# Paleogenomics/pss-bam

Hardware: AMD Instinct MI355X
Metric: aligned reads/s (whole node) + HBM GB/s fraction, 200M x 150bp BAM (higher is better)
Workload: dtype u64

## Files before the change

include/pssbam_hip.h:

```cpp
#ifndef PSSBAM_HIP_H
#define PSSBAM_HIP_H

#include <stddef.h>
#include <stdint.h>

#ifdef __cplusplus
extern "C" {
#endif

#define PSSBAM_ABI_VERSION 1
#define PSSBAM_MAX_KLEN 15
#define PSSBAM_MAX_READ_GROUPS 4096
#define PSSBAM_MAX_LENGTH_BINS 64
#define PSSBAM_MAX_CONTIG_SETS 4096
#define PSSBAM_MAX_HIST_LENGTH 65535
#define PSSBAM_MAX_BASE_QUALITY 93
#define PSSBAM_MAX_REGIONS (1 << 26)
#define PSSBAM_SITE_NONE 0
#define PSSBAM_SITE_CPG 1
#define PSSBAM_MAX_END_DEPTH 8

#define PSSBAM_OK 0
#define PSSBAM_EINVAL (-1)
#define PSSBAM_ENODEV (-2)
#define PSSBAM_EHIP (-3)
#define PSSBAM_ENOMEM (-4)
#define PSSBAM_ESTATE (-5)
#define PSSBAM_EFORMAT (-6)
#define PSSBAM_EBUSY (-7)

#define PSSBAM_TALLY_PSS 1u
#define PSSBAM_TALLY_KMER 2u

#define PSSBAM_KERNEL_AUTO 0
#define PSSBAM_KERNEL_SIMPLE 1
#define PSSBAM_KERNEL_TILED 2

typedef struct pssbam_pss_opts {
    int32_t region_len;
    uint64_t min_read_len;
    uint64_t max_read_len;
    int32_t min_mq;
    const char *up_ctx;
    const char *down_ctx;
    int32_t merged_only;
} pssbam_pss_opts;

typedef struct pssbam_kmer_opts {
    int32_t klen;
    int32_t min_mq;
    uint64_t min_read_len;
    uint64_t max_read_len;
    int32_t merged_only;
} pssbam_kmer_opts;

typedef struct pssbam_config {
    uint32_t abi_version;
    uint32_t tally_mask;
    pssbam_pss_opts pss;
    pssbam_kmer_opts kmer;
    const char *read_group;
    int32_t device;
    int32_t kernel;
} pssbam_config;

typedef struct pssbam_engine pssbam_engine;
struct genome;

enum {
    PSSBAM_ST_RECORDS = 0,
    PSSBAM_ST_RG_DROPPED = 1,
    PSSBAM_ST_PARSE_SKIP = 2,
    PSSBAM_ST_NO_CONTIG = 3,
    PSSBAM_ST_PSS_OK = 4,
    PSSBAM_ST_PSS_FILTERED = 5,
    PSSBAM_ST_KMER_OK = 6,
    PSSBAM_ST_KMER_FILTERED = 7,
    PSSBAM_ST_KMER_FAIL = 8,
    PSSBAM_ST_SLOW_PATH = 9,
    PSSBAM_ST_N = 16
};

const char *pssbam_last_error(void);
int pssbam_device_count(void);
int pssbam_warmup(int device);

int pssbam_engine_create(const pssbam_config *cfg, pssbam_engine **out);
void pssbam_engine_destroy(pssbam_engine *e);

int pssbam_engine_set_stream(pssbam_engine *e, void *hip_stream);

int pssbam_engine_set_genome(pssbam_engine *e, const struct genome *g);
int pssbam_engine_set_genome_async(pssbam_engine *e, const struct genome *g);
int pssbam_engine_genome_wait(pssbam_engine *e);

int pssbam_engine_set_genome_arrays(pssbam_engine *e, size_t n, const char *const *ids,
                                    const uint8_t *const *seqs, const uint64_t *lens,
                                    int seqs_on_device);

int pssbam_engine_set_references(pssbam_engine *e, int32_t n_ref, const char *const *names);

int pssbam_engine_submit(pssbam_engine *e, const void *records, uint64_t nbytes,
                         const uint32_t *offsets, uint32_t n_records);

int pssbam_engine_submit_async(pssbam_engine *e, const void *records, uint64_t nbytes,
                               const uint32_t *offsets, uint32_t n_records, uint64_t *ticket);
int pssbam_engine_wait_copied(pssbam_engine *e, uint64_t ticket);
int pssbam_engine_copy_done(pssbam_engine *e, uint64_t ticket);

int pssbam_engine_submit_device(pssbam_engine *e, const void *d_records, uint64_t nbytes,
                                const uint32_t *d_offsets, uint32_t n_records);

int pssbam_engine_sync(pssbam_engine *e);

int pssbam_engine_finish(pssbam_engine *e, unsigned long *fwd, unsigned long *rev, uint64_t *k5,
                         uint64_t *k3, uint64_t stats[PSSBAM_ST_N]);
int pssbam_engine_reset(pssbam_engine *e);

int pssbam_engine_set_read_groups(pssbam_engine *e, int32_t n, const char *const *ids);
int pssbam_engine_finish_groups(pssbam_engine *e, int32_t group, unsigned long *fwd, unsigned long *rev);

int pssbam_engine_finish_kmer_groups(pssbam_engine *e, int32_t group, uint64_t *k5, uint64_t *k3);

int pssbam_engine_set_length_bins(pssbam_engine *e, int32_t n_edges, const uint32_t *edges);

int pssbam_engine_set_contig_sets(pssbam_engine *e, int32_t n_sets, int64_t n_names, const char *const *names,
                                  const int32_t *set_of);

int pssbam_engine_set_min_base_quality(pssbam_engine *e, int32_t q);

int pssbam_engine_set_regions(pssbam_engine *e, int32_t n_names, const char *const *names, int64_t n_regions,
                              const int32_t *name_of, const uint32_t *starts, const uint32_t *ends);

int pssbam_engine_set_length_histogram(pssbam_engine *e, int32_t max_len);

int pssbam_engine_finish_length_histogram(pssbam_engine *e, uint64_t *fwd, uint64_t *rev);

int pssbam_engine_set_site_context(pssbam_engine *e, int32_t mode);

int pssbam_engine_finish_site_context(pssbam_engine *e, unsigned long *fwd_in, unsigned long *rev_in);

int pssbam_engine_set_end_condition(pssbam_engine *e, int32_t depth, int32_t cell5, int32_t cell3);

int pssbam_engine_finish_end_condition(pssbam_engine *e, unsigned long *fwd_c, unsigned long *rev_c, uint64_t reads[4]);

int pssbam_engine_counters_device(pssbam_engine *e, void **d_counters, size_t *n_u64);

int pssbam_engine_bind_counters(pssbam_engine *e, void *d_counters, size_t n_u64);

int pssbam_engine_genome_kmer_count(pssbam_engine *e, int klen, uint64_t *counts);

int pssbam_reduce_counters(pssbam_engine *const *engines, int n, int root);

int pssbam_host_register(void *ptr, size_t bytes);
int pssbam_host_unregister(void *ptr);

int pssbam_engine_timer_begin(pssbam_engine *e);
int pssbam_engine_timer_end(pssbam_engine *e, float *ms);
int pssbam_engine_kernel_time(pssbam_engine *e, double *total_ms, uint64_t *n_launches, int reset);

int pssbam_engine_phase_times(pssbam_engine *e, double *h2d_ms, uint64_t *h2d_bytes, double *kernel_ms,
                              uint64_t *n_launches);

typedef struct pssbam_bgzf_block {
    uint64_t in_off;
    uint32_t in_len;
    uint32_t isize;
    uint64_t out_off;
    uint32_t crc;
    uint32_t status;
} pssbam_bgzf_block;

int64_t pssbam_bgzf_scan(const void *bytes, uint64_t nbytes, pssbam_bgzf_block *blocks, uint64_t max_blocks,
                         uint64_t *consumed, uint64_t *inflated_bytes);

int pssbam_bgzf_inflate_device(void *hip_stream, const void *d_comp, uint64_t comp_bytes, pssbam_bgzf_block *d_blocks,
                               uint32_t n_blocks, void *d_out, int check_crc);

int pssbam_engine_submit_bgzf(pssbam_engine *e, const void *comp, uint64_t comp_bytes, const pssbam_bgzf_block *blocks,
                              uint32_t n_blocks, uint32_t first_record_offset, uint64_t *ticket);
int pssbam_engine_wait_bgzf_copied(pssbam_engine *e, uint64_t ticket);
int pssbam_engine_feed_open(pssbam_engine *e, int32_t n_ref, uint64_t genome_bytes_hint);
int pssbam_engine_feed_break(pssbam_engine *e);
int pssbam_engine_feed_handoff(pssbam_engine *from, pssbam_engine *to);
#define PSSBAM_FEED_BAD_BLOCK 1u
#define PSSBAM_FEED_RAGGED 2u
#define PSSBAM_FEED_BAD_RECORD 4u
#define PSSBAM_FEED_TRUNCATED 8u
int pssbam_engine_feed_status(pssbam_engine *e, uint32_t *flags, double *inflate_ms, uint64_t *inflated_bytes);
int pssbam_engine_hint_records(pssbam_engine *e, const void *records, uint64_t nbytes);
int pssbam_feed_reserve(int device);
int pssbam_feed_release(int device);

int pssbam_bgzf_inflate_host(int device, const void *bgzf, uint64_t nbytes, void *out, uint64_t out_cap, uint64_t *out_len,
                             uint32_t *n_blocks, uint32_t *first_bad_block, uint32_t *first_bad_status, double *kernel_ms,
                             int check_crc, int repeats);

int64_t pssbam_index_records(const void *bytes, uint64_t nbytes, uint32_t *offsets,
                             uint64_t max_records, uint64_t *consumed);

#ifdef __cplusplus
}
#endif
#endif
```

pss-bam_amd/__init__.py:

```python
from __future__ import annotations

import ctypes as C
import subprocess
from dataclasses import dataclass
from pathlib import Path

import numpy as np

PKG_DIR = Path(__file__).resolve().parent
ROOT = PKG_DIR.parent
LIB_HIP = PKG_DIR / "libpssbam_hip.so"
LIB_HOST = PKG_DIR / "libpssbam_host.so"
LIB_SYNTH = PKG_DIR / "libpssbam_synth.so"

TALLY_PSS, TALLY_KMER = 1, 2
KERNEL_AUTO, KERNEL_SIMPLE, KERNEL_TILED = 0, 1, 2
ST_NAMES = ["records", "rg_dropped", "parse_skip", "no_contig", "pss_ok", "pss_filtered", "kmer_ok",
            "kmer_filtered", "kmer_fail", "slow_path"]
ST_N = 16

HIP_SYMBOLS = [
    "pssbam_last_error", "pssbam_device_count", "pssbam_warmup", "pssbam_engine_create", "pssbam_engine_destroy",
    "pssbam_engine_set_stream", "pssbam_engine_set_genome", "pssbam_engine_set_genome_arrays",
    "pssbam_engine_set_references", "pssbam_engine_submit", "pssbam_engine_submit_async", "pssbam_engine_wait_copied",
    "pssbam_engine_copy_done", "pssbam_engine_phase_times", "pssbam_engine_submit_device", "pssbam_engine_sync",
    "pssbam_engine_finish", "pssbam_engine_reset", "pssbam_engine_counters_device", "pssbam_engine_bind_counters",
    "pssbam_reduce_counters", "pssbam_engine_genome_kmer_count", "pssbam_host_register", "pssbam_host_unregister", "pssbam_engine_timer_begin",
    "pssbam_engine_timer_end", "pssbam_engine_kernel_time", "pssbam_index_records", "pssbam_bgzf_scan",
    "pssbam_bgzf_inflate_device", "pssbam_bgzf_inflate_host", "pssbam_engine_submit_bgzf", "pssbam_engine_wait_bgzf_copied",
    "pssbam_engine_feed_status", "pssbam_engine_feed_break", "pssbam_engine_feed_handoff", "pssbam_feed_reserve", "pssbam_engine_hint_records",
    "pssbam_engine_set_genome_async", "pssbam_engine_genome_wait", "pssbam_engine_feed_open", "pssbam_feed_release",
    "pssbam_engine_set_read_groups", "pssbam_engine_finish_groups", "pssbam_engine_set_length_bins",
    "pssbam_engine_set_contig_sets", "pssbam_engine_finish_kmer_groups", "pssbam_engine_set_min_base_quality",
    "pssbam_engine_set_regions", "pssbam_engine_set_length_histogram", "pssbam_engine_finish_length_histogram",
    "pssbam_engine_set_site_context", "pssbam_engine_finish_site_context",
    "pssbam_engine_set_end_condition", "pssbam_engine_finish_end_condition",
]
MAX_READ_GROUPS = 4096
MAX_LENGTH_BINS = 64
MAX_CONTIG_SETS = 4096
MAX_BASE_QUALITY = 93
MAX_HIST_LENGTH = 65535
MAX_REGIONS = 1 << 26
SITE_NONE, SITE_CPG = 0, 1
SITE_MODES = {None: SITE_NONE, "none": SITE_NONE, "cpg": SITE_CPG}
MAX_END_DEPTH = 8
END_PRESETS = {"ss": (13, 13), "ds": (13, 2)}
EBUSY = -7


def build(verbose: bool = False) -> None:
    subprocess.run(["make", "-C", str(PKG_DIR), "all"], check=True,
                   stdout=None if verbose else subprocess.DEVNULL)


class PssbamError(RuntimeError):
    pass


class _PssOpts(C.Structure):
    _fields_ = [("region_len", C.c_int32), ("min_read_len", C.c_uint64), ("max_read_len", C.c_uint64),
                ("min_mq", C.c_int32), ("up_ctx", C.c_char_p), ("down_ctx", C.c_char_p),
                ("merged_only", C.c_int32)]


class _KmerOpts(C.Structure):
    _fields_ = [("klen", C.c_int32), ("min_mq", C.c_int32), ("min_read_len", C.c_uint64),
                ("max_read_len", C.c_uint64), ("merged_only", C.c_int32)]


class _Config(C.Structure):
    _fields_ = [("abi_version", C.c_uint32), ("tally_mask", C.c_uint32), ("pss", _PssOpts), ("kmer", _KmerOpts),
                ("read_group", C.c_char_p), ("device", C.c_int32), ("kernel", C.c_int32)]


_hip = None


def hip_lib() -> C.CDLL:
    global _hip
    if _hip is not None:
        return _hip
    if not LIB_HIP.exists():
        raise PssbamError(f"{LIB_HIP} is missing: run __graft_entry__.build() (hipcc --offload-arch=gfx950)")
    L = C.CDLL(str(LIB_HIP))
    L.pssbam_last_error.restype = C.c_char_p
    L.pssbam_engine_create.argtypes = [C.POINTER(_Config), C.POINTER(C.c_void_p)]
    L.pssbam_engine_destroy.argtypes = [C.c_void_p]
    L.pssbam_engine_destroy.restype = None
    L.pssbam_engine_set_stream.argtypes = [C.c_void_p, C.c_void_p]
    L.pssbam_engine_set_genome.argtypes = [C.c_void_p, C.c_void_p]
    L.pssbam_engine_set_genome_arrays.argtypes = [C.c_void_p, C.c_size_t, C.POINTER(C.c_char_p),
                                                  C.POINTER(C.c_void_p), C.POINTER(C.c_uint64), C.c_int]
    L.pssbam_engine_set_references.argtypes = [C.c_void_p, C.c_int32, C.POINTER(C.c_char_p)]
    L.pssbam_engine_submit.argtypes = [C.c_void_p, C.c_void_p, C.c_uint64, C.c_void_p, C.c_uint32]
    L.pssbam_engine_submit_async.argtypes = [C.c_void_p, C.c_void_p, C.c_uint64, C.c_void_p, C.c_uint32, C.POINTER(C.c_uint64)]
    L.pssbam_engine_wait_copied.argtypes = [C.c_void_p, C.c_uint64]
    L.pssbam_engine_copy_done.argtypes = [C.c_void_p, C.c_uint64]
    L.pssbam_engine_phase_times.argtypes = [C.c_void_p, C.POINTER(C.c_double), C.POINTER(C.c_uint64), C.POINTER(C.c_double),
                                            C.POINTER(C.c_uint64)]
    L.pssbam_engine_submit_device.argtypes = [C.c_void_p, C.c_void_p, C.c_uint64, C.c_void_p, C.c_uint32]
    L.pssbam_engine_sync.argtypes = [C.c_void_p]
    L.pssbam_engine_finish.argtypes = [C.c_void_p, C.c_void_p, C.c_void_p, C.c_void_p, C.c_void_p, C.c_void_p]
    L.pssbam_engine_reset.argtypes = [C.c_void_p]
    L.pssbam_engine_set_read_groups.argtypes = [C.c_void_p, C.c_int32, C.POINTER(C.c_char_p)]
    L.pssbam_engine_finish_groups.argtypes = [C.c_void_p, C.c_int32, C.c_void_p, C.c_void_p]
    L.pssbam_engine_finish_kmer_groups.argtypes = [C.c_void_p, C.c_int32, C.c_void_p, C.c_void_p]
    L.pssbam_engine_set_length_bins.argtypes = [C.c_void_p, C.c_int32, C.POINTER(C.c_uint32)]
    L.pssbam_engine_set_contig_sets.argtypes = [C.c_void_p, C.c_int32, C.c_int64, C.POINTER(C.c_char_p), C.POINTER(C.c_int32)]
    L.pssbam_engine_set_min_base_quality.argtypes = [C.c_void_p, C.c_int32]
    L.pssbam_engine_set_length_histogram.argtypes = [C.c_void_p, C.c_int32]
    L.pssbam_engine_finish_length_histogram.argtypes = [C.c_void_p, C.c_void_p, C.c_void_p]
    L.pssbam_engine_set_site_context.argtypes = [C.c_void_p, C.c_int32]
    L.pssbam_engine_finish_site_context.argtypes = [C.c_void_p, C.c_void_p, C.c_void_p]
    L.pssbam_engine_set_end_condition.argtypes = [C.c_void_p, C.c_int32, C.c_int32, C.c_int32]
    L.pssbam_engine_finish_end_condition.argtypes = [C.c_void_p, C.c_void_p, C.c_void_p, C.c_void_p]
    L.pssbam_engine_set_regions.argtypes = [C.c_void_p, C.c_int32, C.POINTER(C.c_char_p), C.c_int64, C.c_void_p, C.c_void_p, C.c_void_p]
    L.pssbam_engine_counters_device.argtypes = [C.c_void_p, C.POINTER(C.c_void_p), C.POINTER(C.c_size_t)]
    L.pssbam_engine_bind_counters.argtypes = [C.c_void_p, C.c_void_p, C.c_size_t]
    L.pssbam_engine_genome_kmer_count.argtypes = [C.c_void_p, C.c_int, C.c_void_p]
    L.pssbam_engine_timer_begin.argtypes = [C.c_void_p]
    L.pssbam_engine_timer_end.argtypes = [C.c_void_p, C.POINTER(C.c_float)]
    L.pssbam_engine_kernel_time.argtypes = [C.c_void_p, C.POINTER(C.c_double), C.POINTER(C.c_uint64), C.c_int]
    L.pssbam_index_records.restype = C.c_int64
    L.pssbam_index_records.argtypes = [C.c_void_p, C.c_uint64, C.c_void_p, C.c_uint64, C.POINTER(C.c_uint64)]
    _hip = L
    return L


def _chk(rc: int) -> None:
    if rc != 0:
        raise PssbamError(f"pssbam error {rc}: {hip_lib().pssbam_last_error().decode()}")


def bgzf_inflate(bgzf: np.ndarray, check_crc: bool = True, repeats: int = 1, want_output: bool = True) -> dict:
    L = hip_lib()
    L.pssbam_bgzf_inflate_host.argtypes = [C.c_int, C.c_void_p, C.c_uint64, C.c_void_p, C.c_uint64, C.POINTER(C.c_uint64),
                                           C.POINTER(C.c_uint32), C.POINTER(C.c_uint32), C.POINTER(C.c_uint32),
                                           C.POINTER(C.c_double), C.c_int, C.c_int]
    L.pssbam_bgzf_scan.restype = C.c_int64
    L.pssbam_bgzf_scan.argtypes = [C.c_void_p, C.c_uint64, C.c_void_p, C.c_uint64, C.POINTER(C.c_uint64), C.POINTER(C.c_uint64)]
    bgzf = np.ascontiguousarray(bgzf, dtype=np.uint8)
    consumed, total = C.c_uint64(), C.c_uint64()
    n = L.pssbam_bgzf_scan(bgzf.ctypes.data, bgzf.size, None, 0, C.byref(consumed), C.byref(total))
    if n < 0:
        _chk(int(n))
    out = np.empty(int(total.value) if want_output else 0, dtype=np.uint8)
    out_len, nb, bad_b, bad_s, ms = C.c_uint64(), C.c_uint32(), C.c_uint32(), C.c_uint32(), C.c_double()
    _chk(L.pssbam_bgzf_inflate_host(-1, bgzf.ctypes.data, bgzf.size, out.ctypes.data if want_output else None, out.size,
                                    C.byref(out_len), C.byref(nb), C.byref(bad_b), C.byref(bad_s), C.byref(ms),
                                    int(check_crc), repeats))
    return {"data": out, "inflated_bytes": int(out_len.value), "n_blocks": int(nb.value),
            "bad_block": None if bad_b.value == 0xFFFFFFFF else int(bad_b.value), "bad_status": int(bad_s.value),
            "kernel_ms": float(ms.value)}


def index_records(buf: np.ndarray) -> np.ndarray:
    L = hip_lib()
    n = L.pssbam_index_records(buf.ctypes.data, buf.size, None, 1 << 62, None)
    if n < 0:
        _chk(int(n))
    offs = np.empty(n + 1, dtype=np.uint32)
    consumed = C.c_uint64()
    n2 = L.pssbam_index_records(buf.ctypes.data, buf.size, offs.ctypes.data, n, C.byref(consumed))
    assert n2 == n
    return offs


@dataclass
class Tables:
    fwd: np.ndarray | None
    rev: np.ndarray | None
    k5: np.ndarray | None
    k3: np.ndarray | None
    stats: dict


class Engine:

    def __init__(self, pss: dict | None = None, kmer: dict | None = None, read_group: str | None = None,
                 kernel: int = KERNEL_AUTO, device: int = -1, read_groups: list[str] | None = None,
                 length_bins: list[int] | None = None, contig_sets=None, min_base_qual: int = 0,
                 length_hist: int = 0, site_context: str | None = None, end_condition: tuple[int, int, int] | None = None):
        L = hip_lib()
        cfg = _Config()
        cfg.abi_version = 1
        cfg.tally_mask = (TALLY_PSS if pss is not None else 0) | (TALLY_KMER if kmer is not None else 0)
        self._keep = []
        if pss is not None:
            up, dn = pss.get("up_ctx", "ACGT").encode(), pss.get("down_ctx", "ACGT").encode()
            self._keep += [up, dn]
            cfg.pss = _PssOpts(pss.get("region_len", 15), pss.get("min_read_len", 0),
                               pss.get("max_read_len", 250000000), pss.get("min_mq", 0), up, dn,
                               int(pss.get("merged_only", False)))
            self.region_len = cfg.pss.region_len
            self._len_range = (cfg.pss.min_read_len, cfg.pss.max_read_len)
        if kmer is not None:
            cfg.kmer = _KmerOpts(kmer.get("klen", 8), kmer.get("min_mq", 0), kmer.get("min_read_len", 0),
                                 kmer.get("max_read_len", 250000000), int(kmer.get("merged_only", False)))
            self.klen = cfg.kmer.klen
            if pss is None:
                self._len_range = (cfg.kmer.min_read_len, cfg.kmer.max_read_len)
        self.has_pss, self.has_kmer = pss is not None, kmer is not None
        if read_group is not None:
            rg = read_group.encode()
            self._keep.append(rg)
            cfg.read_group = rg
        cfg.device = device
        cfg.kernel = kernel
        h = C.c_void_p()
        _chk(L.pssbam_engine_create(C.byref(cfg), C.byref(h)))
        self._h = h
        self._L = L
        self.read_groups: list[str] = []
        self.length_bins: list[tuple[int, int]] = []
        self.contig_sets: list[str] = []
        self._min_base_qual = 0
        self._length_hist = 0
        self._site_context = SITE_NONE
        if min_base_qual:
            self.set_min_base_quality(min_base_qual)
        if length_hist:
            self.set_length_histogram(length_hist)
        if site_context is not None:
            self.set_site_context(site_context)
        self._end_condition = (0, 0, 0)
        if end_condition is not None:
            self.set_end_condition(*end_condition)
        if read_groups is not None:
            self.set_read_groups(read_groups)
        if length_bins is not None:
            self.set_length_bins(length_bins)
        if contig_sets is not None:
            self.set_contig_sets(contig_sets)

    def set_min_base_quality(self, q: int):
        _chk(self._L.pssbam_engine_set_min_base_quality(self._h, int(q)))
        self._min_base_qual = int(q)

    @property
    def min_base_qual(self) -> int:
        return self._min_base_qual

    def set_length_histogram(self, max_len: int):
        _chk(self._L.pssbam_engine_set_length_histogram(self._h, int(max_len)))
        self._length_hist = int(max_len)

    @property
    def length_hist(self) -> int:
        return self._length_hist

    def finish_length_hist(self) -> tuple[np.ndarray, np.ndarray]:
        fwd = np.zeros(self._length_hist + 2, dtype=np.uint64)
        rev = np.zeros_like(fwd)
        _chk(self._L.pssbam_engine_finish_length_histogram(self._h, fwd.ctypes.data, rev.ctypes.data))
        return fwd, rev

    def set_site_context(self, mode):
        if isinstance(mode, str) or mode is None:
            if mode not in SITE_MODES:
                raise ValueError(f"unknown site context {mode!r}")
            mode = SITE_MODES[mode]
        _chk(self._L.pssbam_engine_set_site_context(self._h, int(mode)))
        self._site_context = int(mode)

    @property
    def site_context(self) -> str | None:
        return "cpg" if self._site_context == SITE_CPG else None

    def finish_site_context(self) -> tuple[np.ndarray, np.ndarray]:
        fwd = np.zeros((self.region_len + 2, 16), dtype=np.uint64)
        rev = np.zeros_like(fwd)
        _chk(self._L.pssbam_engine_finish_site_context(self._h, fwd.ctypes.data, rev.ctypes.data))
        return fwd, rev

    def set_end_condition(self, depth: int, cell5: int = 13, cell3: int = 13):
        _chk(self._L.pssbam_engine_set_end_condition(self._h, int(depth), int(cell5), int(cell3)))
        self._end_condition = (int(depth), int(cell5), int(cell3)) if depth else (0, 0, 0)

    @property
    def end_condition(self) -> tuple[int, int, int] | None:
        return self._end_condition if self._end_condition[0] else None

    def finish_end_condition(self) -> tuple[np.ndarray, np.ndarray, np.ndarray]:
        fwd = np.zeros((self.region_len + 2, 16), dtype=np.uint64)
        rev = np.zeros_like(fwd)
        reads = np.zeros(4, dtype=np.uint64)
        _chk(self._L.pssbam_engine_finish_end_condition(self._h, fwd.ctypes.data, rev.ctypes.data, reads.ctypes.data))
        return fwd, rev, reads

    def set_regions(self, names, name_of, starts, ends):
        raw = [nm.encode() if isinstance(nm, str) else bytes(nm) for nm in names]
        arr = (C.c_char_p * max(len(raw), 1))(*raw)
        name_of = np.ascontiguousarray(name_of, dtype=np.int32)
        starts = np.ascontiguousarray(starts, dtype=np.uint32)
        ends = np.ascontiguousarray(ends, dtype=np.uint32)
        if not (name_of.size == starts.size == ends.size):
            raise ValueError("name_of, starts and ends must have one entry per interval")
        _chk(self._L.pssbam_engine_set_regions(self._h, len(raw), arr, name_of.size, name_of.ctypes.data, starts.ctypes.data,
                                               ends.ctypes.data))

    def set_contig_sets(self, sets):
        pairs = [(nm, lab) for lab, nms in sets.items() for nm in nms] if isinstance(sets, dict) else list(sets)
        labels: list[str] = []
        index: dict[str, int] = {}
        for _, lab in pairs:
            if lab not in index:
                index[lab] = len(labels)
                labels.append(lab)
        names = (C.c_char_p * max(len(pairs), 1))(*[nm.encode() if isinstance(nm, str) else bytes(nm) for nm, _ in pairs])
        set_of = (C.c_int32 * max(len(pairs), 1))(*[index[lab] for _, lab in pairs])
        _chk(self._L.pssbam_engine_set_contig_sets(self._h, len(labels), len(pairs), names, set_of))
        self.contig_sets = labels

    def finish_sets(self) -> dict:
        return self._finish_planes(enumerate(self.contig_sets))

    def set_length_bins(self, edges: list[int]):
        edges = [int(x) for x in edges]
        arr = (C.c_uint32 * max(len(edges), 1))(*[x & 0xFFFFFFFF for x in edges])
        _chk(self._L.pssbam_engine_set_length_bins(self._h, len(edges), arr))
        lo, hi = self._len_range
        starts, ends = [lo] + edges, [x - 1 for x in edges] + [hi]
        self.length_bins = list(zip(starts, ends))

    def set_read_groups(self, ids: list[str]):
        raw = [i.encode() if isinstance(i, str) else bytes(i) for i in ids]
        arr = (C.c_char_p * max(len(raw), 1))(*raw)
        _chk(self._L.pssbam_engine_set_read_groups(self._h, len(raw), arr))
        self.read_groups = [i.decode() if isinstance(i, bytes) else i for i in ids]

    def finish_groups(self) -> dict:
        return self._finish_planes([(-1, None)] + list(enumerate(self.read_groups)))

    def finish_bins(self) -> dict:
        return self._finish_planes(enumerate(self.length_bins))

    def _finish_planes(self, planes) -> dict:
        out = {}
        for g, key in planes:
            if not self.has_pss:
                k5 = np.zeros(4 ** self.klen, dtype=np.uint64)
                k3 = np.zeros_like(k5)
                _chk(self._L.pssbam_engine_finish_kmer_groups(self._h, g, k5.ctypes.data, k3.ctypes.data))
                if key not in out:
                    out[key] = Tables(None, None, k5, k3, {})
                continue
            fwd = np.zeros((self.region_len + 2, 16), dtype=np.uint64)
            rev = np.zeros_like(fwd)
            _chk(self._L.pssbam_engine_finish_groups(self._h, g, fwd.ctypes.data, rev.ctypes.data))
            if key not in out:
                out[key] = Tables(fwd, rev, None, None, {})
        return out

    def close(self):
        if getattr(self, "_h", None):
            self._L.pssbam_engine_destroy(self._h)
            self._h = None

    __del__ = close

    def set_stream(self, hip_stream: int):
        _chk(self._L.pssbam_engine_set_stream(self._h, C.c_void_p(hip_stream)))

    def set_genome_arrays(self, contigs: list[tuple[str, np.ndarray]]):
        n = len(contigs)
        arrs = [np.ascontiguousarray(a, dtype=np.uint8) for _, a in contigs]
        ids = (C.c_char_p * n)(*[c[0].encode() for c in contigs])
        seqs = (C.c_void_p * n)(*[a.ctypes.data for a in arrs])
        lens = (C.c_uint64 * n)(*[a.size for a in arrs])
        _chk(self._L.pssbam_engine_set_genome_arrays(self._h, n, ids, seqs, lens, 0))

    def set_genome_device(self, contigs: list[tuple[str, int, int]]):
        n = len(contigs)
        ids = (C.c_char_p * n)(*[c[0].encode() for c in contigs])
        seqs = (C.c_void_p * n)(*[c[1] for c in contigs])
        lens = (C.c_uint64 * n)(*[c[2] for c in contigs])
        _chk(self._L.pssbam_engine_set_genome_arrays(self._h, n, ids, seqs, lens, 1))

    def set_genome_struct(self, genome_ptr: int):
        _chk(self._L.pssbam_engine_set_genome(self._h, C.c_void_p(genome_ptr)))

    def set_references(self, names: list[str]):
        n = len(names)
        arr = (C.c_char_p * max(n, 1))(*[s.encode() for s in names])
        _chk(self._L.pssbam_engine_set_references(self._h, n, arr))

    def submit(self, records: np.ndarray, offsets: np.ndarray | None = None):
        records = np.ascontiguousarray(records, dtype=np.uint8)
        if offsets is None:
            offsets = index_records(records)
            if int(offsets[-1]) != records.size:
                raise PssbamError("record block ends in a partial record")
        offsets = np.ascontiguousarray(offsets, dtype=np.uint32)
        _chk(self._L.pssbam_engine_submit(self._h, records.ctypes.data, records.size, offsets.ctypes.data,
                                          offsets.size - 1))

    def submit_async(self, records: np.ndarray, offsets: np.ndarray) -> int:
        t = C.c_uint64()
        _chk(self._L.pssbam_engine_submit_async(self._h, records.ctypes.data, records.size, offsets.ctypes.data,
                                                offsets.size - 1, C.byref(t)))
        return int(t.value)

    def wait_copied(self, ticket: int):
        _chk(self._L.pssbam_engine_wait_copied(self._h, ticket))

    def copy_done(self, ticket: int) -> bool:
        rc = self._L.pssbam_engine_copy_done(self._h, ticket)
        if rc < 0:
            _chk(rc)
        return bool(rc)

    def phase_times(self) -> dict:
        a, b, c, d = C.c_double(), C.c_uint64(), C.c_double(), C.c_uint64()
        _chk(self._L.pssbam_engine_phase_times(self._h, C.byref(a), C.byref(b), C.byref(c), C.byref(d)))
        return {"h2d_ms": a.value, "h2d_bytes": b.value, "kernel_ms": c.value, "launches": d.value}

    def feed_open(self, n_ref: int, genome_bytes_hint: int = 0):
        self._L.pssbam_engine_feed_open.argtypes = [C.c_void_p, C.c_int32, C.c_uint64]
        _chk(self._L.pssbam_engine_feed_open(self._h, n_ref, genome_bytes_hint))

    def submit_bgzf(self, bgzf: np.ndarray, header_bytes: int = 0, max_batch_inflated: int = 1 << 30, on_busy=None) -> int:
        class _Blk(C.Structure):
            _fields_ = [("in_off", C.c_uint64), ("in_len", C.c_uint32), ("isize", C.c_uint32), ("out_off", C.c_uint64),
                        ("crc", C.c_uint32), ("status", C.c_uint32)]
        L = self._L
        L.pssbam_bgzf_scan.restype = C.c_int64
        L.pssbam_bgzf_scan.argtypes = [C.c_void_p, C.c_uint64, C.c_void_p, C.c_uint64, C.POINTER(C.c_uint64), C.POINTER(C.c_uint64)]
        L.pssbam_engine_submit_bgzf.argtypes = [C.c_void_p, C.c_void_p, C.c_uint64, C.c_void_p, C.c_uint32, C.c_uint32,
                                                C.POINTER(C.c_uint64)]
        L.pssbam_engine_wait_bgzf_copied.argtypes = [C.c_void_p, C.c_uint64]
        bgzf = np.ascontiguousarray(bgzf, dtype=np.uint8)
        consumed = C.c_uint64()
        n = L.pssbam_bgzf_scan(bgzf.ctypes.data, bgzf.size, None, 0, C.byref(consumed), None)
        if n < 0:
            _chk(int(n))
        if consumed.value != bgzf.size:
            raise PssbamError("input ends inside a BGZF block")
        blocks = (_Blk * max(int(n), 1))()
        L.pssbam_bgzf_scan(bgzf.ctypes.data, bgzf.size, blocks, n, None, None)
        i, skip = 0, header_bytes
        while i < n and skip >= blocks[i].isize and (skip > 0 or blocks[i].isize == 0):
            skip -= blocks[i].isize
            i += 1
        while i < n:
            j, base_in, base_out = i, blocks[i].in_off & ~3, blocks[i].out_off
            while j < n and blocks[j].out_off + blocks[j].isize - base_out <= max_batch_inflated:
                j += 1
            j = max(j, i + 1)
            grp = (_Blk * (j - i))()
            for k in range(i, j):
                grp[k - i] = blocks[k]
                grp[k - i].in_off -= base_in
                grp[k - i].out_off -= base_out
            end_in = blocks[j - 1].in_off + blocks[j - 1].in_len
            t = C.c_uint64()
            rc = L.pssbam_engine_submit_bgzf(self._h, bgzf.ctypes.data + base_in, end_in - base_in, grp, j - i, skip, C.byref(t))
            if rc == EBUSY and on_busy is not None:
                on_busy()
                rc = L.pssbam_engine_submit_bgzf(self._h, bgzf.ctypes.data + base_in, end_in - base_in, grp, j - i, skip, C.byref(t))
            _chk(rc)
            _chk(L.pssbam_engine_wait_bgzf_copied(self._h, t.value))
            skip = 0
            i = j
        return int(n)

    def feed_break(self):
        self._L.pssbam_engine_feed_break.argtypes = [C.c_void_p]
        _chk(self._L.pssbam_engine_feed_break(self._h))

    def feed_handoff(self, to: "Engine"):
        self._L.pssbam_engine_feed_handoff.argtypes = [C.c_void_p, C.c_void_p]
        _chk(self._L.pssbam_engine_feed_handoff(self._h, to._h))

    def feed_status(self) -> dict:
        L = self._L
        L.pssbam_engine_feed_status.argtypes = [C.c_void_p, C.POINTER(C.c_uint32), C.POINTER(C.c_double), C.POINTER(C.c_uint64)]
        f, ms, nb = C.c_uint32(), C.c_double(), C.c_uint64()
        _chk(L.pssbam_engine_feed_status(self._h, C.byref(f), C.byref(ms), C.byref(nb)))
        return {"flags": int(f.value), "inflate_ms": float(ms.value), "inflated_bytes": int(nb.value)}

    def submit_device(self, d_records: int, nbytes: int, d_offsets: int, n_records: int):
        _chk(self._L.pssbam_engine_submit_device(self._h, C.c_void_p(d_records), nbytes, C.c_void_p(d_offsets),
                                                 n_records))

    def sync(self):
        _chk(self._L.pssbam_engine_sync(self._h))

    def reset(self):
        _chk(self._L.pssbam_engine_reset(self._h))

    def finish(self) -> Tables:
        fwd = rev = k5 = k3 = None
        if self.has_pss:
            fwd = np.zeros((self.region_len + 2, 16), dtype=np.uint64)
            rev = np.zeros_like(fwd)
        if self.has_kmer:
            k5 = np.zeros(4 ** self.klen, dtype=np.uint64)
            k3 = np.zeros_like(k5)
        st = np.zeros(ST_N, dtype=np.uint64)
        p = lambda a: a.ctypes.data if a is not None else None
        _chk(self._L.pssbam_engine_finish(self._h, p(fwd), p(rev), p(k5), p(k3), st.ctypes.data))
        return Tables(fwd, rev, k5, k3, {n: int(st[i]) for i, n in enumerate(ST_NAMES)})

    def counters_device(self) -> tuple[int, int]:
        ptr, n = C.c_void_p(), C.c_size_t()
        _chk(self._L.pssbam_engine_counters_device(self._h, C.byref(ptr), C.byref(n)))
        return int(ptr.value), int(n.value)

    def bind_counters(self, d_ptr: int | None, n_u64: int = 0):
        _chk(self._L.pssbam_engine_bind_counters(self._h, C.c_void_p(d_ptr) if d_ptr else None, n_u64))

    def counter_layout(self) -> dict:
        rows = (self.region_len + 2) if self.has_pss else 0
        nb = 4 ** self.klen if self.has_kmer else 0
        lay = {"fwd": 0, "rev": rows * 16, "k5": 2 * rows * 16, "k3": 2 * rows * 16 + nb,
               "stats": 2 * rows * 16 + 2 * nb, "rows": rows, "bins": nb}
        base = lay["stats"] + ST_N
        if not self.has_pss:
            for name, tag, keys in (("groups", "id", self.read_groups), ("length_bins", "bin", self.length_bins),
                                    ("contig_sets", "label", self.contig_sets)):
                lay[name] = [{tag: key, "k5": base + k * 2 * nb, "k3": base + k * 2 * nb + nb} for k, key in enumerate(keys)]
            lay["n_u64"] = base + (len(self.read_groups) + len(self.length_bins) + len(self.contig_sets)) * 2 * nb
            return lay
        lay["groups"] = [{"id": g, "fwd": base + k * 2 * rows * 16, "rev": base + k * 2 * rows * 16 + rows * 16}
                         for k, g in enumerate(self.read_groups)]
        lay["length_bins"] = [{"bin": b, "fwd": base + k * 2 * rows * 16, "rev": base + k * 2 * rows * 16 + rows * 16}
                              for k, b in enumerate(self.length_bins)]
        lay["contig_sets"] = [{"label": s, "fwd": base + k * 2 * rows * 16, "rev": base + k * 2 * rows * 16 + rows * 16}
                              for k, s in enumerate(self.contig_sets)]
        lay["n_u64"] = base + (len(self.read_groups) + len(self.length_bins) + len(self.contig_sets)) * 2 * rows * 16
        if self._length_hist:
# ... 28 lines not shown
```

pss-bam_amd/csrc/engine.hip:

```cpp
#include "../../include/pssbam_hip.h"
#include "../../include/fasta-genome-io.h"

#include <hip/hip_runtime.h>

#include <algorithm>
#include <condition_variable>
#include <cstdarg>
#include <cstdio>
#include <cstdlib>
#include <cstring>
#include <ctime>
#include <map>
#include <string>
#include <thread>
#include <tuple>
#include <type_traits>
#include <unordered_map>
#include <atomic>
#include <memory>
#include <mutex>
#include <vector>

#include "tally_kernels.h"

// ... 85 lines not shown
    uint64_t flush_seq = 0;
};

struct DeferredTally {
    int slot;
    uint64_t sub_base, sub_len, offs_at;
    uint32_t n_bound, k;
    uint64_t sample_off;
    bool last_of_slot;
};

namespace {
struct PinEntry { size_t len; int refs; };
std::map<const void *, PinEntry> g_pins;
std::mutex g_pins_mu;
bool pin_acquire(const void *p, size_t len) {
    std::lock_guard<std::mutex> lk(g_pins_mu);
    auto it = g_pins.find(p);
    if (it != g_pins.end()) { it->second.refs++; return true; }
    if (hipHostRegister((void *)p, len, hipHostRegisterPortable) != hipSuccess) { (void)hipGetLastError(); return false; }
    g_pins[p] = PinEntry{len, 1};
    return true;
}
void pin_release(const void *p) {
    std::lock_guard<std::mutex> lk(g_pins_mu);
    auto it = g_pins.find(p);
    if (it == g_pins.end()) return;
    if (--it->second.refs == 0) { (void)hipHostUnregister((void *)p); g_pins.erase(it); }
}
}

struct KernelPrep { uint32_t lds = 0; int occ = 0; };

struct pssbam_engine {
    pssbam_config cfg{};
    std::string up_ctx, down_ctx, rg;
    bool has_rg = false;
    int device = 0;
    int n_cu = 0;
    hipStream_t stream = nullptr, copy_stream = nullptr, copy_stream2 = nullptr;
    hipStream_t inflate_stream[2] = {nullptr, nullptr};
    hipEvent_t feed_base_ev = nullptr;
    hipStream_t genome_stream = nullptr;
    std::thread late_thread;
    std::atomic<int> late_ready{0};
    std::mutex late_mu;
    hipStream_t late_copy1 = nullptr, late_copy2 = nullptr, late_genome = nullptr;
    bool late_adopted = false;
    hipEvent_t genome_ready = nullptr;
    bool genome_wait_pending = false;
    std::vector<const void *> genome_pins;
    std::vector<void *> retired;
    hipEvent_t copied2 = nullptr;
    bool own_stream = false;

    uint8_t *d_genome = nullptr;
    uint32_t *d_genome4 = nullptr;
    uint32_t acgt_ctx = 0;
    uint64_t genome_bytes = 0;
    std::vector<uint64_t> contig_start;
    std::vector<uint32_t> contig_len;
    std::vector<std::string> contig_ids;
    int32_t star_contig = -1;
    uint4 *d_ref_info = nullptr;
    uint4 *h_ref_info = nullptr;
    size_t h_ref_cap = 0;
    int32_t n_ref = 0;
    bool have_refs = false;
    uint8_t *d_rg = nullptr;
    PlaneSel planes = PLANES_NONE;
    uint32_t n_planes = 0, off_groups = 0, plane_words = 0;
    uint64_t kplane_words = 0;
    uint8_t *d_grp_ids = nullptr;
    uint32_t *d_grp_offs = nullptr, *d_grp_hash = nullptr;
    uint32_t grp_hash_mask = 0;
    std::vector<uint32_t> len_edges;
    std::unordered_map<std::string, uint32_t> ctg_plane;
    std::vector<std::string> ref_names;
    bool tallied = false;
    uint32_t min_bq = 0;
    uint32_t hist_max = 0, off_hist = 0;
    uint32_t site_mode = 0, off_site = 0;
    uint32_t end_depth = 0, end_cell5 = 0, end_cell3 = 0, off_end = 0;
    int env_hist_lds_bins = -1;
    std::unordered_map<std::string, std::vector<uint2>> regions;
    bool has_regions = false;
    uint32_t region_shift = 10;
    std::vector<uint4> ref_info_host;
    uint4 *d_region_info = nullptr;
    uint32_t *d_region_grid = nullptr;
    uint2 *d_region_iv = nullptr;
    unsigned long long *d_counters = nullptr;
    unsigned long long *d_counters_own = nullptr;
    size_t n_counters = 0;
    uint32_t rows = 0, off_rev = 0, off_k5 = 0, off_k3 = 0, off_stats = 0;
    uint64_t n_bins = 0;
    Slot slots[2];
    int next_slot = 0;
    uint64_t ticket_seq = 0;
    double h2d_ms = 0.0;
    uint64_t h2d_bytes = 0;
    std::vector<FeedAcc *> feed;
    int cur_feed = -1, spare_feed = -1;
    uint64_t flush_seq = 0;
    bool feed_opened = false;
    int32_t feed_n_ref = 0;
    uint64_t feed_mem_budget = 0;
    std::vector<DeferredTally> deferred;
    uint8_t *d_carry = nullptr;
    uint8_t *h_handoff = nullptr;
    hipEvent_t handoff_ev = nullptr;
    uint64_t feed_out_target = FEED_OUT_TARGET, feed_comp_cap = FEED_COMP_CAP;
    double feed_t_alloc = 0, feed_t_wait_busy = 0, feed_t_flush = 0;
    double feed_t0 = 0, feed_t_first_flush = -1;
    uint64_t feed_slots_allocated = 0, feed_deferred_launches = 0, feed_early_flushes = 0;
    uint64_t feed_blocks_launched = 0, feed_lanes_launched = 0;
    uint64_t feed_idle_min_blocks = 8192;
    uint64_t feed_block_target = 0;
    std::vector<std::pair<uint64_t, hipEvent_t>> feed_copies;
    std::vector<hipEvent_t> feed_event_pool;
    uint32_t *d_feed_flags = nullptr;
    uint64_t *d_feed_tail = nullptr;
    bool feed_fresh = true;
    uint32_t feed_skip = 0;
    double inflate_ms = 0.0;
    uint64_t inflated_bytes = 0;
    std::vector<std::pair<hipEvent_t, hipEvent_t>> inflate_events;
    hipEvent_t t_begin = nullptr, t_end = nullptr;
    std::vector<std::pair<hipEvent_t, hipEvent_t>> launch_events;
    std::vector<hipEvent_t> event_pool;
    double kernel_ms = 0.0;
    uint64_t kernel_launches = 0;
    int env_tile_reads = 0, env_grid_mult = 0, env_simple_blocks = 0, env_grid_wgs = 0, env_pieces = 0;
    int env_group_slots = 0;
    bool warned_ablate = false;
    bool compact_plan_once = false;
    std::unordered_map<const void *, KernelPrep> prep;
    bool use_compact = true;
    uint32_t *d_scratch = nullptr;
    size_t scratch_slots = 0;
    uint32_t dev_pieces = 0;
    uint64_t dev_pieces_avg = 0;
};

static void ctx_mask(const char *set, uint32_t (&m)[8]) {
    memset(m, 0, sizeof m);
    for (const unsigned char *p = (const unsigned char *)set;; p++) {
        const uint32_t st = enc_byte(*p);
        m[st >> 5] |= 1u << (st & 31);
        if (!*p) break;
    }
}

static int env_int(const char *name) {
    const char *v = getenv(name);
    return v ? atoi(v) : 0;
}

static void late_streams(pssbam_engine *e, bool wait) {
    std::lock_guard<std::mutex> lk(e->late_mu);
    if (e->late_adopted) return;
    if (!wait && !e->late_ready.load(std::memory_order_acquire)) return;
    if (e->late_thread.joinable()) e->late_thread.join();
    e->copy_stream = e->late_copy1;
    e->copy_stream2 = e->late_copy2;
    e->genome_stream = e->late_genome;
    e->late_adopted = true;
}

extern "C" int pssbam_engine_create(const pssbam_config *cfg, pssbam_engine **out) {
    if (!cfg || !out) return fail(PSSBAM_EINVAL, "null argument");
    *out = nullptr;
    if (cfg->abi_version != PSSBAM_ABI_VERSION)
        return fail(PSSBAM_EINVAL, "abi_version %u != %u", cfg->abi_version, PSSBAM_ABI_VERSION);
    if (!(cfg->tally_mask & (PSSBAM_TALLY_PSS | PSSBAM_TALLY_KMER)) ||
        (cfg->tally_mask & ~(PSSBAM_TALLY_PSS | PSSBAM_TALLY_KMER)))
        return fail(PSSBAM_EINVAL, "tally_mask must be a non-empty subset of PSS|KMER");
    if ((cfg->tally_mask & PSSBAM_TALLY_PSS)) {
        if (cfg->pss.region_len < 0 || cfg->pss.region_len > 1000000)
            return fail(PSSBAM_EINVAL, "region_len %d out of range", cfg->pss.region_len);
        if (!cfg->pss.up_ctx || !cfg->pss.down_ctx) return fail(PSSBAM_EINVAL, "up_ctx/down_ctx must be set");
    }
    if ((cfg->tally_mask & PSSBAM_TALLY_KMER) && (cfg->kmer.klen < 1 || cfg->kmer.klen > PSSBAM_MAX_KLEN))
        return fail(PSSBAM_EINVAL, "klen %d outside the device range 1..%d", cfg->kmer.klen, PSSBAM_MAX_KLEN);

    int n_dev = 0;
    if (hipGetDeviceCount(&n_dev) != hipSuccess || n_dev == 0)
        return fail(PSSBAM_ENODEV, "no HIP device available (this engine has no CPU path)");
    int dev = cfg->device;
    if (dev < 0) HIP_TRY(hipGetDevice(&dev));
    if (dev >= n_dev) return fail(PSSBAM_ENODEV, "device %d does not exist (%d present)", dev, n_dev);
    if (!device_is_gfx950(dev) && !getenv("PSSBAM_ALLOW_OTHER_ARCH"))
        return fail(PSSBAM_ENODEV, "device %d is not gfx950", dev);
    HIP_TRY(hipSetDevice(dev));

    pssbam_engine *e = new pssbam_engine();
    std::unique_ptr<pssbam_engine, void (*)(pssbam_engine *)> guard(e, pssbam_engine_destroy);
    e->cfg = *cfg;
    e->device = dev;
    if (cfg->tally_mask & PSSBAM_TALLY_PSS) {
        e->up_ctx = cfg->pss.up_ctx;
        e->down_ctx = cfg->pss.down_ctx;
    }
    if (cfg->read_group) {
        e->rg = cfg->read_group;
        e->has_rg = true;
    }
    e->cfg.pss.up_ctx = e->cfg.pss.down_ctx = e->cfg.read_group = nullptr;
    const bool tstat = getenv("PSSBAM_STATS") != nullptr;
    const double tc0 = tstat ? feed_now() : 0.0;
    hipDeviceProp_t pr;
    HIP_TRY(hipGetDeviceProperties(&pr, dev));
    e->n_cu = pr.multiProcessorCount;
    const double tc1 = tstat ? feed_now() : 0.0;
    HIP_TRY(hipStreamCreateWithFlags(&e->stream, hipStreamNonBlocking));
    if (getenv("PSSBAM_STREAMS_UP_FRONT")) {
        HIP_TRY(hipStreamCreateWithFlags(&e->copy_stream, hipStreamNonBlocking));
        HIP_TRY(hipStreamCreateWithFlags(&e->copy_stream2, hipStreamNonBlocking));
        HIP_TRY(hipStreamCreateWithFlags(&e->genome_stream, hipStreamNonBlocking));
        e->late_adopted = true;
    } else {
        e->late_thread = std::thread([e, dev]() {
            if (hipSetDevice(dev) == hipSuccess) {
                if (hipStreamCreateWithFlags(&e->late_copy1, hipStreamNonBlocking) != hipSuccess) e->late_copy1 = nullptr;
                if (hipStreamCreateWithFlags(&e->late_copy2, hipStreamNonBlocking) != hipSuccess) e->late_copy2 = nullptr;
                if (hipStreamCreateWithFlags(&e->late_genome, hipStreamNonBlocking) != hipSuccess) e->late_genome = nullptr;
            }
            (void)hipGetLastError();
            e->late_ready.store(1, std::memory_order_release);
        });
    }
    HIP_TRY(hipEventCreateWithFlags(&e->genome_ready, hipEventDisableTiming));
    HIP_TRY(hipEventCreateWithFlags(&e->copied2, hipEventDisableTiming));
    e->own_stream = true;
    HIP_TRY(hipEventCreate(&e->t_begin));
    HIP_TRY(hipEventCreate(&e->t_end));
    const double tc2 = tstat ? feed_now() : 0.0;

    e->rows = (cfg->tally_mask & PSSBAM_TALLY_PSS) ? (uint32_t)cfg->pss.region_len + 2u : 0u;
    e->n_bins = (cfg->tally_mask & PSSBAM_TALLY_KMER) ? (1ull << (2 * cfg->kmer.klen)) : 0ull;
    e->off_rev = e->rows * 16u;
    e->off_k5 = 2u * e->rows * 16u;
    e->off_k3 = (uint32_t)(e->off_k5 + e->n_bins);
    e->off_stats = (uint32_t)(e->off_k3 + e->n_bins);
    e->n_counters = (size_t)e->off_stats + PSSBAM_ST_N;
    e->plane_words = 2u * e->rows * 16u;
    e->off_groups = (uint32_t)e->n_counters;
    e->kplane_words = cfg->tally_mask == PSSBAM_TALLY_KMER ? 2ull * e->n_bins : 0ull;
    HIP_TRY(hipMalloc(&e->d_counters_own, e->n_counters * sizeof(unsigned long long)));
    e->d_counters = e->d_counters_own;
    HIP_TRY(hipMemsetAsync(e->d_counters, 0, e->n_counters * sizeof(unsigned long long), e->stream));
    if (e->has_rg) {
        HIP_TRY(hipMalloc(&e->d_rg, e->rg.size() + 16));
        HIP_TRY(hipMemcpy(e->d_rg, e->rg.data(), e->rg.size(), hipMemcpyHostToDevice));
    }
    for (Slot &s : e->slots) {
        HIP_TRY(hipEventCreate(&s.copy_begin));
        HIP_TRY(hipEventCreate(&s.copied));
        HIP_TRY(hipEventCreateWithFlags(&s.consumed, hipEventDisableTiming));
    }
    e->scratch_slots = (size_t)e->n_cu * 8;
    HIP_TRY(hipMalloc(&e->d_scratch, e->scratch_slots * SCRATCH_WORDS * sizeof(uint32_t)));
    e->env_tile_reads = env_int("PSSBAM_TILE_READS");
    e->env_grid_mult = env_int("PSSBAM_GRID_MULT");
    e->env_simple_blocks = env_int("PSSBAM_SIMPLE_BLOCKS");
    e->env_grid_wgs = env_int("PSSBAM_GRID_WGS");
    e->env_pieces = env_int("PSSBAM_PIECES");
    e->env_group_slots = env_int("PSSBAM_GROUP_SLOTS");
    if (getenv("PSSBAM_HIST_LDS_BINS")) e->env_hist_lds_bins = std::max(env_int("PSSBAM_HIST_LDS_BINS"), 0);
    if (const int g = env_int("PSSBAM_REGION_GRID_SHIFT")) e->region_shift = (uint32_t)std::min(std::max(g, 2), 20);
    if (getenv("PSSBAM_COMPACT")) e->use_compact = env_int("PSSBAM_COMPACT") != 0;
    if (getenv("PSSBAM_COMPACT_PLAN_ONCE")) e->compact_plan_once = env_int("PSSBAM_COMPACT_PLAN_ONCE") != 0;
    if (tstat)
        fprintf(stderr, "[pssbam] engine on device %d: device properties %.3f, its stream + events %.3f, counters + scratch (first allocations, first "
                        "enqueue) %.3f s\n", dev, tc1 - tc0, tc2 - tc1, feed_now() - tc2);
    *out = guard.release();
    return PSSBAM_OK;
}

extern "C" void pssbam_engine_destroy(pssbam_engine *e) {
    if (!e) return;
    (void)hipSetDevice(e->device);
    late_streams(e, true);
    for (hipStream_t is : e->inflate_stream)
        if (is) (void)hipStreamSynchronize(is);
    if (e->stream) (void)hipStreamSynchronize(e->stream);
    if (e->copy_stream) (void)hipStreamSynchronize(e->copy_stream);
    if (e->copy_stream2) (void)hipStreamSynchronize(e->copy_stream2);
    for (Slot &s : e->slots) {
        if (s.d_recs) (void)hipFree(s.d_recs);
        if (s.d_offs) (void)hipFree(s.d_offs);
        if (s.copied) (void)hipEventDestroy(s.copied);
        if (s.copy_begin) (void)hipEventDestroy(s.copy_begin);
        if (s.consumed) (void)hipEventDestroy(s.consumed);
    }
    if (e->genome_stream) (void)hipStreamSynchronize(e->genome_stream);
    for (const void *p : e->genome_pins) pin_release(p);
    e->genome_pins.clear();
    for (FeedAcc *sp : e->feed) {
        FeedAcc &s = *sp;
        void *ptrs[] = {s.d_comp, s.d_blocks, s.d_a, s.d_e, s.d_last, s.d_nexta, s.d_n, s.d_counts, s.d_base, s.d_out, s.d_offs, s.d_nrecs, s.d_chain};
        for (void *q : ptrs)
            if (q) (void)hipFree(q);
        if (s.h_blocks) (void)hipHostFree(s.h_blocks);
        if (s.consumed) (void)hipEventDestroy(s.consumed);
        if (s.copies_done) (void)hipEventDestroy(s.copies_done);
        if (s.copies_done2) (void)hipEventDestroy(s.copies_done2);
        if (s.inflated) (void)hipEventDestroy(s.inflated);
        if (s.inflate_done) (void)hipEventDestroy(s.inflate_done);
        delete sp;
    }
    e->feed.clear();
    if (e->d_carry) (void)hipFree(e->d_carry);
    if (e->h_handoff) (void)hipHostFree(e->h_handoff);
    if (e->handoff_ev) (void)hipEventDestroy(e->handoff_ev);
    for (void *q : e->retired) (void)hipFree(q);
    if (e->d_feed_tail) (void)hipFree(e->d_feed_tail);
    for (auto &p : e->feed_copies) (void)hipEventDestroy(p.second);
    for (hipEvent_t ev : e->feed_event_pool) (void)hipEventDestroy(ev);
    if (e->d_feed_flags) (void)hipFree(e->d_feed_flags);
    for (auto &p : e->inflate_events) { (void)hipEventDestroy(p.first); (void)hipEventDestroy(p.second); }
    for (auto &p : e->launch_events) { (void)hipEventDestroy(p.first); (void)hipEventDestroy(p.second); }
    for (hipEvent_t ev : e->event_pool) (void)hipEventDestroy(ev);
    if (e->t_begin) (void)hipEventDestroy(e->t_begin);
    if (e->t_end) (void)hipEventDestroy(e->t_end);
    if (e->d_scratch) (void)hipFree(e->d_scratch);
    if (e->d_genome) (void)hipFree(e->d_genome);
    if (e->d_genome4) (void)hipFree(e->d_genome4);
    if (e->d_ref_info) (void)hipFree(e->d_ref_info);
    if (e->h_ref_info) (void)hipHostFree(e->h_ref_info);
    if (e->d_rg) (void)hipFree(e->d_rg);
    for (void *q : {(void *)e->d_region_info, (void *)e->d_region_grid, (void *)e->d_region_iv})
        if (q) (void)hipFree(q);
    if (e->d_grp_ids) (void)hipFree(e->d_grp_ids);
    if (e->d_grp_offs) (void)hipFree(e->d_grp_offs);
    if (e->d_grp_hash) (void)hipFree(e->d_grp_hash);
    if (e->d_counters_own) (void)hipFree(e->d_counters_own);
    if (e->own_stream && e->stream) (void)hipStreamDestroy(e->stream);
    if (e->copy_stream) (void)hipStreamDestroy(e->copy_stream);
    if (e->copy_stream2) (void)hipStreamDestroy(e->copy_stream2);
    for (hipStream_t is : e->inflate_stream)
        if (is) (void)hipStreamDestroy(is);
    if (e->feed_base_ev) (void)hipEventDestroy(e->feed_base_ev);
    if (e->genome_stream) (void)hipStreamDestroy(e->genome_stream);
    if (e->genome_ready) (void)hipEventDestroy(e->genome_ready);
    if (e->copied2) (void)hipEventDestroy(e->copied2);
    delete e;
}

extern "C" int pssbam_engine_set_stream(pssbam_engine *e, void *hip_stream) {
    if (!e) return fail(PSSBAM_EINVAL, "null engine");
    HIP_TRY(hipSetDevice(e->device));
    HIP_TRY(hipStreamSynchronize(e->stream));
    if (e->own_stream) HIP_TRY(hipStreamDestroy(e->stream));
    e->stream = (hipStream_t)hip_stream;
    e->own_stream = false;
    return PSSBAM_OK;
}

static constexpr uint64_t CONTIG_ALIGN = 256, CONTIG_PAD = 256;

static hipEvent_t take_event(pssbam_engine *e);
static int feed_resume(pssbam_engine *e);

static int genome_settle(pssbam_engine *e) {
    if (e->genome_pins.empty()) return PSSBAM_OK;
    HIP_TRY(hipSetDevice(e->device));
    HIP_TRY(hipEventSynchronize(e->genome_ready));
    for (const void *p : e->genome_pins) pin_release(p);
    e->genome_pins.clear();
    return PSSBAM_OK;
}

static int genome_upload(pssbam_engine *e, size_t n, const char *const *ids, const uint8_t *const *seqs, const uint64_t *lens,
                         int seqs_on_device) {
    if (!e || (n && (!ids || !seqs || !lens))) return fail(PSSBAM_EINVAL, "null argument");
    HIP_TRY(hipSetDevice(e->device));
    int rc = genome_settle(e);
    if (rc) return rc;
    std::vector<size_t> order(n);
    for (size_t i = 0; i < n; i++) order[i] = i;
    std::stable_sort(order.begin(), order.end(), [&](size_t a, size_t b) { return strcmp(ids[a], ids[b]) < 0; });
    std::vector<uint64_t> start(n + 1, 0);
    std::vector<uint32_t> len(n + 1, 0);
    uint64_t total = CONTIG_PAD;
    for (size_t k = 0; k < n; k++) {
        if (lens[order[k]] > 0xFFFFFF00ull)
            return fail(PSSBAM_EINVAL, "contig %s has %llu bases; the engine addresses contigs below 4 Gi bases", ids[order[k]],
                        (unsigned long long)lens[order[k]]);
        start[k] = total;
        len[k] = (uint32_t)lens[order[k]];
        total += ((uint64_t)len[k] + CONTIG_PAD + CONTIG_ALIGN - 1) / CONTIG_ALIGN * CONTIG_ALIGN;
    }
    if (e->d_genome) {
        HIP_TRY(hipStreamSynchronize(e->stream));
        HIP_TRY(hipFree(e->d_genome));
        e->d_genome = nullptr;
        if (e->d_genome4) { HIP_TRY(hipFree(e->d_genome4)); e->d_genome4 = nullptr; }
    }
    HIP_TRY(hipMalloc(&e->d_genome, total));
    late_streams(e, true);
    if (!e->genome_stream) HIP_TRY(hipStreamCreateWithFlags(&e->genome_stream, hipStreamNonBlocking));
    hipStream_t gs = e->genome_stream;
    if (seqs_on_device) {
        hipEvent_t ev = take_event(e);
        if (!ev) return fail(PSSBAM_EHIP, "hipEventCreate failed");
        HIP_TRY(hipEventRecord(ev, e->stream));
        HIP_TRY(hipStreamWaitEvent(gs, ev, 0));
        e->event_pool.push_back(ev);
    }
    HIP_TRY(hipMemsetAsync(e->d_genome, 0, total, gs));
    const bool try_lock = !seqs_on_device && !getenv("PSSBAM_NO_PIN");
    for (size_t k = 0; k < n; k++) {
        if (!len[k]) continue;
        const void *src = seqs[order[k]];
        if (try_lock && len[k] >= (32u << 20) && pin_acquire(src, len[k])) e->genome_pins.push_back(src);
        HIP_TRY(hipMemcpyAsync(e->d_genome + start[k], src, len[k],
                               seqs_on_device ? hipMemcpyDeviceToDevice : hipMemcpyHostToDevice, gs));
    }
    hipLaunchKernelGGL(encode_genome_kernel, dim3(4096), dim3(256), 0, gs, e->d_genome, total / 16);
    HIP_TRY(hipGetLastError());
    {
        CtxSets sets;
        ctx_mask(e->up_ctx.c_str(), sets.up);
        ctx_mask(e->down_ctx.c_str(), sets.down);
        e->acgt_ctx = 0;
        for (uint32_t v = 0; v < 4; v++)
            e->acgt_ctx |= (((sets.up[0] >> v) & 1u) << (2 * v)) | (((sets.down[0] >> v) & 1u) << (2 * v + 1));
        const uint64_t n_out = total / 8, slack = 16;
        HIP_TRY(hipMalloc(&e->d_genome4, (n_out + slack) * sizeof(uint32_t)));
        HIP_TRY(hipMemsetAsync(e->d_genome4 + n_out, 0x44, slack * sizeof(uint32_t), gs));
        hipLaunchKernelGGL(pack_genome4_kernel, dim3(4096), dim3(256), 0, gs, e->d_genome, e->d_genome4, n_out, sets);
        HIP_TRY(hipGetLastError());
    }
    HIP_TRY(hipEventRecord(e->genome_ready, gs));
    e->genome_wait_pending = true;
    e->contig_start.assign(start.begin(), start.begin() + n);
    e->contig_len.assign(len.begin(), len.begin() + n);
    e->genome_bytes = total;
    e->contig_ids.clear();
    for (size_t k = 0; k < n; k++) e->contig_ids.emplace_back(ids[order[k]]);
    e->star_contig = -1;
    if (e->have_refs) e->have_refs = false;
    {
        auto it = std::lower_bound(e->contig_ids.begin(), e->contig_ids.end(), std::string("*"),
                                   [](const std::string &a, const std::string &b) { return strcmp(a.c_str(), b.c_str()) < 0; });
        if (it != e->contig_ids.end() && *it == "*") e->star_contig = (int32_t)(it - e->contig_ids.begin());
    }
    return PSSBAM_OK;
}

extern "C" int pssbam_engine_set_genome_arrays(pssbam_engine *e, size_t n, const char *const *ids,
                                               const uint8_t *const *seqs, const uint64_t *lens,
                                               int seqs_on_device) {
    int rc = genome_upload(e, n, ids, seqs, lens, seqs_on_device);
    if (rc) return rc;
    if (e->genome_stream) HIP_TRY(hipStreamSynchronize(e->genome_stream));
    return genome_settle(e);
}

static int genome_from_struct(pssbam_engine *e, const struct genome *g, bool wait) {
    if (!e || !g) return fail(PSSBAM_EINVAL, "null argument");
    std::vector<const char *> ids(g->n_seqs);
    std::vector<const uint8_t *> seqs(g->n_seqs);
    std::vector<uint64_t> lens(g->n_seqs);
    for (size_t i = 0; i < g->n_seqs; i++) {
        ids[i] = g->seqs[i]->id;
        seqs[i] = (const uint8_t *)g->seqs[i]->seq;
        lens[i] = g->seqs[i]->len;
    }
    return wait ? pssbam_engine_set_genome_arrays(e, g->n_seqs, ids.data(), seqs.data(), lens.data(), 0)
                : genome_upload(e, g->n_seqs, ids.data(), seqs.data(), lens.data(), 0);
}

extern "C" int pssbam_engine_set_genome(pssbam_engine *e, const struct genome *g) { return genome_from_struct(e, g, true); }

extern "C" int pssbam_engine_set_genome_async(pssbam_engine *e, const struct genome *g) { return genome_from_struct(e, g, false); }

extern "C" int pssbam_engine_genome_wait(pssbam_engine *e) {
    if (!e) return fail(PSSBAM_EINVAL, "null engine");
    HIP_TRY(hipSetDevice(e->device));
    if (e->genome_stream) HIP_TRY(hipStreamSynchronize(e->genome_stream));
    return genome_settle(e);
}

static int pack_regions(pssbam_engine *e, bool in_use) {
    if (!e->has_regions) return PSSBAM_OK;
    const size_t n_ent = (size_t)e->n_ref + 1;
    const uint32_t g = e->region_shift;
    std::vector<uint4> desc(n_ent, make_uint4(0, 0, 0, 0));
    uint64_t n_iv = 0, n_grid = 0;
    std::vector<const std::vector<uint2> *> src(n_ent, nullptr);
    for (size_t i = 0; i < n_ent; i++) {
        const uint4 ri = e->ref_info_host[i];
        if (!ri.w) continue;
        const auto it = e->regions.find(i < (size_t)e->n_ref ? e->ref_names[i] : std::string("*"));
        if (it == e->regions.end()) continue;
        uint64_t cnt = 0;
        for (const uint2 &v : it->second) cnt += v.x < ri.z ? 1u : 0u;
        if (!cnt) continue;
        src[i] = &it->second;
        desc[i] = make_uint4(0, (uint32_t)cnt, 0, 0);
        n_iv += cnt;
        n_grid += ((uint64_t)ri.z >> g) + 2;
    }
    if (n_iv >= (1ull << 32) || n_grid >= (1ull << 32)) return fail(PSSBAM_ENOMEM, "the region table has too many intervals or grid words for 32-bit indices");
    const uint64_t bytes = n_ent * sizeof(uint4) + (n_iv + 1) * sizeof(uint2) + (n_grid + 2) * sizeof(uint32_t);
    HIP_TRY(hipSetDevice(e->device));
    if (in_use && e->d_region_info) HIP_TRY(hipStreamSynchronize(e->stream));
    for (void **q : {(void **)&e->d_region_info, (void **)&e->d_region_grid, (void **)&e->d_region_iv})
        if (*q) { HIP_TRY(hipFree(*q)); *q = nullptr; }
    size_t free_b = 0, total_b = 0;
    HIP_TRY(hipMemGetInfo(&free_b, &total_b));
    if (bytes > (uint64_t)free_b)
        return fail(PSSBAM_ENOMEM, "the region table (%llu intervals, grid shift %u) needs %llu bytes; the device has %llu free",
                    (unsigned long long)n_iv, g, (unsigned long long)bytes, (unsigned long long)free_b);
    std::vector<uint2> iv((size_t)n_iv + 1, make_uint2(0, 0));
    std::vector<uint32_t> grid((size_t)n_grid + 2, 0u);
    uint64_t at_iv = 0, at_grid = 0;
    for (size_t i = 0; i < n_ent; i++) {
        if (!src[i]) continue;
        const uint32_t len = e->ref_info_host[i].z, cnt = desc[i].y;
        desc[i].x = (uint32_t)at_iv;
        desc[i].z = (uint32_t)at_grid;
        uint2 *out = iv.data() + at_iv;
        for (uint32_t k = 0; k < cnt; k++) out[k] = make_uint2((*src[i])[k].x, std::min((*src[i])[k].y, len));
        const uint64_t n_bins = ((uint64_t)len >> g) + 1;
        uint32_t j = 0;
        for (uint64_t b = 0; b < n_bins; b++) {
            while (j < cnt && (uint64_t)out[j].y <= (b << g)) j++;
            grid[at_grid + b] = j;
        }
        grid[at_grid + n_bins] = cnt;
        at_iv += cnt;
        at_grid += n_bins + 1;
    }
    HIP_TRY(hipMalloc(&e->d_region_info, n_ent * sizeof(uint4)));
    HIP_TRY(hipMalloc(&e->d_region_iv, iv.size() * sizeof(uint2)));
    HIP_TRY(hipMalloc(&e->d_region_grid, grid.size() * sizeof(uint32_t)));
    HIP_TRY(hipMemcpy(e->d_region_info, desc.data(), n_ent * sizeof(uint4), hipMemcpyHostToDevice));
    HIP_TRY(hipMemcpy(e->d_region_iv, iv.data(), iv.size() * sizeof(uint2), hipMemcpyHostToDevice));
    HIP_TRY(hipMemcpy(e->d_region_grid, grid.data(), grid.size() * sizeof(uint32_t), hipMemcpyHostToDevice));
    return PSSBAM_OK;
}

extern "C" int pssbam_engine_set_regions(pssbam_engine *e, int32_t n_names, const char *const *names, int64_t n_regions,
                                         const int32_t *name_of, const uint32_t *starts, const uint32_t *ends) {
    if (!e) return fail(PSSBAM_EINVAL, "null engine");
    if (n_names < 0 || n_regions < 0 || n_regions > PSSBAM_MAX_REGIONS) return fail(PSSBAM_EINVAL, "region count outside 0..%d", PSSBAM_MAX_REGIONS);
    if ((n_names && !names) || (n_regions && (!name_of || !starts || !ends))) return fail(PSSBAM_EINVAL, "null region list");
    if (e->tallied) return fail(PSSBAM_ESTATE, "records have been tallied already: set the regions after create or reset, before the first tally");
    std::unordered_map<std::string, std::vector<uint2>> map;
    for (int32_t k = 0; k < n_names; k++) {
        if (!names[k]) return fail(PSSBAM_EINVAL, "region contig name %d is NULL", k);
        if (n_regions) map[names[k]];
    }
    for (int64_t i = 0; i < n_regions; i++) {
        if (name_of[i] < 0 || name_of[i] >= n_names) return fail(PSSBAM_EINVAL, "region %lld: contig index %d outside 0..%d", (long long)i, name_of[i], n_names - 1);
        if (starts[i] > ends[i])
            return fail(PSSBAM_EINVAL, "region %lld on %s: start %u lies behind end %u", (long long)i, names[name_of[i]], starts[i], ends[i]);
        if (starts[i] < ends[i]) map[names[name_of[i]]].push_back(make_uint2(starts[i], ends[i]));
    }
    for (auto &kv : map) {
        std::vector<uint2> &v = kv.second;
        std::sort(v.begin(), v.end(), [](const uint2 &a, const uint2 &b) { return a.x != b.x ? a.x < b.x : a.y < b.y; });
        size_t n = 0;
        for (const uint2 &r : v) {
            if (n && r.x <= v[n - 1].y) v[n - 1].y = std::max(v[n - 1].y, r.y);
            else v[n++] = r;
        }
        v.resize(n);
    }
    HIP_TRY(hipSetDevice(e->device));
    e->regions.swap(map);
    e->has_regions = n_regions > 0;
    if (!e->has_regions) {
        if (e->d_region_info) HIP_TRY(hipStreamSynchronize(e->stream));
        for (void **q : {(void **)&e->d_region_info, (void **)&e->d_region_grid, (void **)&e->d_region_iv})
            if (*q) { HIP_TRY(hipFree(*q)); *q = nullptr; }
        return PSSBAM_OK;
    }
    return e->have_refs ? pack_regions(e, true) : PSSBAM_OK;
}

extern "C" int pssbam_engine_set_references(pssbam_engine *e, int32_t n_ref, const char *const *names) {
    if (!e || n_ref < 0 || (n_ref && !names)) return fail(PSSBAM_EINVAL, "bad argument");
    if (!e->d_genome) return fail(PSSBAM_ESTATE, "set_genome must precede set_references");
    HIP_TRY(hipSetDevice(e->device));
    std::vector<uint4> info((size_t)n_ref + 1, make_uint4(0, 0, 0, 0));
    auto fill = [&](size_t slot, int32_t contig, const char *name) {
        if (contig < 0) return;
        const uint64_t gb = e->contig_start[(size_t)contig];
        uint32_t plane = 0;
        if (!e->ctg_plane.empty()) {
            const auto it = e->ctg_plane.find(name);
            if (it != e->ctg_plane.end()) plane = it->second;
        }
        info[slot] = make_uint4((uint32_t)gb, (uint32_t)(gb >> 32), e->contig_len[(size_t)contig], 1u | plane << 1);
    };
    for (int32_t i = 0; i < n_ref; i++) {
        size_t lo = 0, hi = e->contig_ids.size();
        while (lo < hi) {
            const size_t mid = (lo + hi) / 2;
            const int c = strcmp(names[i], e->contig_ids[mid].c_str());
            if (c == 0) { fill((size_t)i, (int32_t)mid, names[i]); break; }
            if (c < 0) hi = mid; else lo = mid + 1;
        }
    }
    fill((size_t)n_ref, e->star_contig, "*");
    e->ref_names.assign(names, names + n_ref);
    if (e->feed_opened && !e->deferred.empty() && n_ref != e->feed_n_ref)
        return fail(PSSBAM_ESTATE, "pssbam_engine_feed_open announced %d references, set_references brings %d", e->feed_n_ref, n_ref);
    if (e->d_ref_info) {
        if (e->have_refs) HIP_TRY(hipStreamSynchronize(e->stream));
        HIP_TRY(hipFree(e->d_ref_info));
        e->d_ref_info = nullptr;
    }
    HIP_TRY(hipMalloc(&e->d_ref_info, ((size_t)n_ref + 1) * sizeof(uint4)));
    if (e->h_ref_cap < (size_t)n_ref + 1) {
        if (e->h_ref_info) (void)hipHostFree(e->h_ref_info);
        e->h_ref_info = nullptr;
        e->h_ref_cap = (size_t)n_ref + 1 + 64;
        HIP_TRY(hipHostMalloc((void **)&e->h_ref_info, e->h_ref_cap * sizeof(uint4), hipHostMallocDefault));
    } else if (e->have_refs) HIP_TRY(hipStreamSynchronize(e->stream));
    memcpy(e->h_ref_info, info.data(), ((size_t)n_ref + 1) * sizeof(uint4));
    hipLaunchKernelGGL(copy_table_kernel, dim3(1), dim3(256), 0, e->stream, e->d_ref_info, (const uint4 *)e->h_ref_info, (uint32_t)n_ref + 1u);
    HIP_TRY(hipGetLastError());
    const bool replaced = e->have_refs;
    e->n_ref = n_ref;
    e->have_refs = true;
    e->ref_info_host.swap(info);
    if (const int rc = pack_regions(e, replaced)) return rc;
    return feed_resume(e);
}

static hipEvent_t take_event(pssbam_engine *e) {
// ... 1055 lines not shown
```

pss-bam_amd/csrc/tally_kernels.h:

```cpp
#pragma once

#include "record_decode.h"

namespace pssbam {

constexpr int TILED_THREADS = 256;
constexpr int TILED_WAVES = TILED_THREADS / 64;
constexpr int TILED_ROWS = 32;
constexpr int KMER_LDS_MAX_K = 4;
constexpr uint32_t STAGE_SLACK = 64;
constexpr uint32_t CODE_NONE = 32;
constexpr uint32_t TABLE_WORDS = 64 * 32;
constexpr uint32_t SCRATCH_KMER = 1024, SCRATCH_DELTA = 1536, SCRATCH_WORDS = 1552;
constexpr uint32_t SITE_WORDS = 16 * 32, SITE_SCRATCH_WORDS = SCRATCH_WORDS + SITE_WORDS;
constexpr uint32_t CODE_SITE = 64;
constexpr uint32_t END_SCRATCH_WORDS = SCRATCH_WORDS + 32 * 32;
constexpr uint32_t CODE_END = 64;
__host__ __device__ inline uint32_t end_lds_bytes(uint32_t rows) { return (32u * rows + 4u) * 4u; }
constexpr uint32_t REF_LDS_ENTRIES = 64;

struct LdsTableRowMajor {
    uint32_t *t;
    uint32_t rows;
    __device__ __forceinline__ void add(uint32_t table, uint32_t row, uint32_t cell) const {
// ... 1413 lines not shown
    __shared__ int32_t lds_delta[ST_USED];
    if (threadIdx.x < ST_USED) lds_delta[threadIdx.x] = 0;
    __syncthreads();
    const uint32_t stride = gridDim.x * blockDim.x;
    for (uint32_t r = blockIdx.x * blockDim.x + threadIdx.x; r < P.n_recs; r += stride) {
        const uint32_t o0 = P.offs[r], o1 = P.offs[r + 1];
        GlobalBytes src{P.recs + o0};
        const RecHdr h = decode_hdr(src, o1 - o0);
        const Plan pl = make_plan<false, true>(P, src, h);
        bool kfail = false;
        if (pl.fk5 || pl.fk3) kfail = tally_kmer_record_plane<false>(P, G, pl, record_plane<PLANES, true>(src, h, pl, G), nullptr);
        book_events(false, true, record_events(false, true, pl, kfail), lds_delta);
    }
    __syncthreads();
    flush_events(false, true, P, lds_delta);
}

constexpr uint32_t GKC_SPAN = 256;
template <bool LDS_BINS>
__global__ void __launch_bounds__(256) genome_kmer_kernel(const uint8_t *genome, uint64_t n, int K,
                                                          unsigned long long *bins) {
    __shared__ uint32_t lds_bins[LDS_BINS ? 4096 : 1];
    const uint32_t nb = 1u << (2 * K), mask = nb - 1u;
    if (LDS_BINS) {
        for (uint32_t i = threadIdx.x; i < nb; i += blockDim.x) lds_bins[i] = 0u;
        __syncthreads();
    }
    const uint64_t n_spans = (n + GKC_SPAN - 1) / GKC_SPAN;
    for (uint64_t sp = (uint64_t)blockIdx.x * blockDim.x + threadIdx.x; sp < n_spans; sp += (uint64_t)gridDim.x * blockDim.x) {
        const uint64_t p0 = sp * GKC_SPAN, p1 = min(n, p0 + GKC_SPAN);
        uint32_t code = 0u, run = 0u;
        for (uint64_t p = p0 >= (uint64_t)(K - 1) ? p0 - (uint64_t)(K - 1) : 0; p < p0; p++) {
            const uint32_t c = genome[p];
            run = c < 4u ? run + 1u : 0u;
            code = ((code << 2) | (c & 3u)) & mask;
        }
        for (uint64_t p = p0; p < p1; p += 4) {
            const uint32_t w = *(const uint32_t *)(genome + p);
#pragma unroll
            for (int b = 0; b < 4; b++) {
                if (p + b < p1) {
                    const uint32_t c = (w >> (8 * b)) & 0xFFu;
                    run = c < 4u ? run + 1u : 0u;
                    code = ((code << 2) | (c & 3u)) & mask;
                    if (run >= (uint32_t)K) {
                        if (LDS_BINS) atomicAdd(&lds_bins[code], 1u);
                        else atomicAdd(&bins[code], 1ull);
                    }
                }
            }
        }
    }
    if (LDS_BINS) {
        __syncthreads();
        for (uint32_t i = threadIdx.x; i < nb; i += blockDim.x)
            if (lds_bins[i]) atomicAdd(&bins[i], (unsigned long long)lds_bins[i]);
    }
}

constexpr uint32_t GKC4_SPAN = 256;
__global__ void __launch_bounds__(512) genome_kmer_packed_kernel(const uint32_t *g4, uint64_t n_pos, int K, uint32_t bin_lo,
                                                                 uint32_t n_bins, uint32_t rep_log2,
                                                                 unsigned long long *bins) {
    extern __shared__ uint32_t lds_hist[];
    const uint32_t rep = 1u << rep_log2;
    for (uint32_t i = threadIdx.x; i < (n_bins << rep_log2); i += blockDim.x) lds_hist[i] = 0u;
    __syncthreads();
    const uint32_t mask = (1u << (2 * K)) - 1u;
    const uint32_t copy = threadIdx.x & (rep - 1u);
    const uint64_t n_spans = (n_pos + GKC4_SPAN - 1) / GKC4_SPAN;
    for (uint64_t sp = (uint64_t)blockIdx.x * blockDim.x + threadIdx.x; sp < n_spans; sp += (uint64_t)gridDim.x * blockDim.x) {
        const uint64_t p0 = sp * GKC4_SPAN;
        const uint4 *src = (const uint4 *)(g4 + p0 / 8);
        uint32_t code = 0u, run = 0u;
        if (p0) {
            const uint32_t w = g4[p0 / 8 - 1];
#pragma unroll
            for (int b = 1; b < 8; b++) {
                const uint32_t c = (w >> (4 * b)) & 15u;
                run = c < 4u ? run + 1u : 0u;
                code = (code << 2) | (c & 3u);
            }
            run = min(run, (uint32_t)(K - 1));
        }
#pragma unroll 2
        for (int q = 0; q < (int)(GKC4_SPAN / 32); q++) {
            if (p0 + 32ull * q >= n_pos) break;
            const uint4 v = src[q];
            const uint32_t w4[4] = {v.x, v.y, v.z, v.w};
#pragma unroll
            for (int d = 0; d < 4; d++) {
#pragma unroll
                for (int b = 0; b < 8; b++) {
                    const uint32_t c = (w4[d] >> (4 * b)) & 15u;
                    run = c < 4u ? run + 1u : 0u;
                    code = ((code << 2) | (c & 3u)) & mask;
                    const uint32_t slot = code - bin_lo;
                    if (run >= (uint32_t)K && slot < n_bins && p0 + 32ull * q + 8u * d + b < n_pos)
                        atomicAdd(&lds_hist[(slot << rep_log2) + copy], 1u);
                }
            }
        }
    }
    __syncthreads();
    for (uint32_t i = threadIdx.x; i < n_bins; i += blockDim.x) {
        uint32_t sum = 0u;
        for (uint32_t r = 0; r < rep; r++) sum += lds_hist[(i << rep_log2) + r];
        if (sum) atomicAdd(&bins[bin_lo + i], (unsigned long long)sum);
    }
}

__global__ void copy_table_kernel(uint4 *dst, const uint4 *src, uint32_t n) {
    for (uint32_t i = threadIdx.x; i < n; i += blockDim.x) dst[i] = src[i];
}

__global__ void encode_genome_kernel(uint8_t *p, uint64_t n16) {
    const uint64_t stride = (uint64_t)gridDim.x * blockDim.x;
    uint4 *q = (uint4 *)p;
    for (uint64_t i = (uint64_t)blockIdx.x * blockDim.x + threadIdx.x; i < n16; i += stride) {
        uint4 v = q[i];
        uint32_t w[4] = {v.x, v.y, v.z, v.w};
#pragma unroll
        for (int k = 0; k < 4; k++) {
            uint32_t o = 0;
#pragma unroll
            for (int b = 0; b < 4; b++) {
                uint32_t c = (w[k] >> (8 * b)) & 0xFFu;
                if (c >= 'a' && c <= 'z') c -= 32u;
                o |= enc_byte(c) << (8 * b);
            }
            w[k] = o;
        }
        q[i] = make_uint4(w[0], w[1], w[2], w[3]);
    }
}

struct CtxSets { uint32_t up[8], down[8]; };
__global__ void pack_genome4_kernel(const uint8_t *g, uint32_t *out, uint64_t n_out, CtxSets sets) {
    const uint64_t stride = (uint64_t)gridDim.x * blockDim.x;
    const uint2 *src = (const uint2 *)g;
    for (uint64_t i = (uint64_t)blockIdx.x * blockDim.x + threadIdx.x; i < n_out; i += stride) {
        const uint2 v = src[i];
        uint32_t o = 0u;
#pragma unroll
        for (int b = 0; b < 8; b++) {
            const uint32_t c = ((b < 4 ? v.x : v.y) >> (8 * (b & 3))) & 0xFFu;
            const uint32_t nib = c < 4u ? c : 4u + (in_set(sets.up, c) ? 1u : 0u) + (in_set(sets.down, c) ? 2u : 0u);
            o |= nib << (4 * b);
        }
        out[i] = o;
    }
}

}
```

pss-bam_amd/host/fragkon_main.c:

```c
#include <ctype.h>
#include <stdio.h>
#include <stdlib.h>
#include <string.h>
#include <unistd.h>

#include "contig_sets.h"
#include "fasta-genome-io.h"
#include "frontend.h"
#include "length_bins.h"
#include "read_groups.h"
#include "regions.h"
#include "report.h"
#include "sam-parse.h"

int main(int argc, char *argv[])
{
    frontend_detach_start();
    int klen = 8, min_mq = 0, merged_only = 0, option;
    unsigned long min_read_len = 0, max_read_len = 250000000;
    char *fasta_fn = NULL, *bam_fn = NULL, *out_prefix = NULL;
    int by_group = 0;
    const char *len_edges = NULL, *ctg_map = NULL, *bed_fn = NULL;

    while ((option = getopt(argc, argv, ":F:B:k:l:L:q:mGS:C:o:T:")) != -1) {
        switch (option) {
        case 'F': fasta_fn = strdup(optarg); break;
        case 'B': bam_fn = strdup(optarg); break;
        case 'k': klen = atoi(optarg); break;
        case 'l': min_read_len = strtoul(optarg, NULL, 10); break;
        case 'L': max_read_len = strtoul(optarg, NULL, 10); break;
        case 'q': min_mq = atoi(optarg); break;
        case 'm': merged_only = 1; break;
        case 'G': by_group = 1; break;
        case 'S': len_edges = optarg; break;
        case 'C': ctg_map = optarg; break;
        case 'T': bed_fn = optarg; break;
        case 'o': out_prefix = strdup(optarg); break;
        case ':':
            fprintf(stderr, "Please enter required argument for option -%c.\n", optopt);
            exit(0);
        case '?':
            if (isprint(optopt)) fprintf(stderr, "Unknown option -%c.\n", optopt);
            else fprintf(stderr, "Unknown option character \\x%x.\n", optopt);
            break;
        default:
            fprintf(stderr, "Error parsing command-line options.\n");
            exit(0);
        }
    }
    for (int i = optind; i < argc; i++) fprintf(stderr, "Non-option argument %s\n", argv[i]);

    if (!fasta_fn || !bam_fn) {
        fputs("fragkon: Program for describing kmer-based genomic sequence\n"
              "contexts around the fragmentation points of aligned reads.\n"
              "-F <reference FASTA (required)>\n"
              "-B <input BAM (required)>\n"
              "-k <kmer length (default: 8)>\n"
              "-l <minimum length of read to report (default: 0)>\n"
              "-L <maximum length of read to report (default: 250000000)>\n"
              "-q <map quality filter of read to report (default: 0)>\n"
              "-m <only consider merged reads>\n",
              stderr);
        exit(1);
    }
    const int n_selectors = by_group + (len_edges != NULL) + (ctg_map != NULL);
    if (n_selectors > 1) {
        fprintf(stderr, "-G (tables per read group), -S (tables per length bin) and -C (tables per contig set) exclude each other.\n");
        exit(1);
    }
    if (n_selectors && !out_prefix) {
        fprintf(stderr, "-%c needs -o <output filename prefix> for the per-%s tables (<prefix>.<tag>.fragkon.txt).\n",
                by_group ? 'G' : len_edges ? 'S' : 'C', by_group ? "read-group" : len_edges ? "length-bin" : "contig-set");
        exit(1);
    }
    uint32_t edges[PSSBAM_MAX_LENGTH_BINS - 1];
    int n_edges = 0;
    if (len_edges) {
        char err[200];
        if ((n_edges = pss_parse_length_edges(len_edges, min_read_len, max_read_len, edges, err, sizeof err)) < 0) {
            fprintf(stderr, "%s\n", err);
            exit(1);
        }
    }
    pss_regions bed;
    memset(&bed, 0, sizeof bed);
    if (bed_fn) {
        char err[300];
        if (pss_read_bed(bed_fn, &bed, err, sizeof err)) {
            fprintf(stderr, "%s (%s)\n", err, bed_fn);
            exit(1);
        }
    }
    frontend_contig_map sets;
    memset(&sets, 0, sizeof sets);
    if (ctg_map) {
        FILE *mf = fopen(ctg_map, "rb");
        char *text = NULL;
        size_t len = 0, cap = 0;
        int read_ok = mf != NULL;
        while (read_ok) {
            if (len == cap) {
                char *t = (char *)realloc(text, cap = cap ? 2 * cap : 65536);
                if (!t) { read_ok = 0; break; }
                text = t;
            }
            const size_t got = fread(text + len, 1, cap - len, mf);
            len += got;
            if (got == 0) { read_ok = !ferror(mf); break; }
        }
        if (mf) fclose(mf);
        if (!read_ok) {
            fprintf(stderr, "-C: unable to read the map file %s.\n", ctg_map);
            exit(1);
        }
        char err[600];
        sets.n_names = pss_parse_contig_sets(text, len, &sets.names, &sets.set_of, &sets.labels, &sets.n_labels, err, sizeof err);
        free(text);
        if (sets.n_names < 0) {
            fprintf(stderr, "%s (%s)\n", err, ctg_map);
            exit(1);
        }
    }
    if (klen < 1 || klen > PSSBAM_MAX_KLEN) {
        fprintf(stderr, "k-mer length %d is outside the range this build tallies on the GPU (1..%d).\n", klen, PSSBAM_MAX_KLEN);
        exit(1);
    }

    fputs("# Entered command: ", stderr);
    for (int i = 0; i < argc; i++) fprintf(stderr, "%s ", argv[i]);
    fputc('\n', stderr);
    fprintf(stderr, "Input kmer length = %d.\n", klen);
    if (klen & 1)
        fprintf(stderr, "    *** k is odd - counting %d bases outside %d bases inside of alignment.\n", klen / 2,
                klen / 2 + 1);
    fprintf(stderr, "Reading genome sequence from: %s\n", fasta_fn);
    pssbam_config cfg;
    memset(&cfg, 0, sizeof cfg);
    cfg.abi_version = PSSBAM_ABI_VERSION;
    cfg.tally_mask = PSSBAM_TALLY_KMER;
    cfg.kmer.klen = klen;
    cfg.kmer.min_mq = min_mq;
    cfg.kmer.min_read_len = min_read_len;
    cfg.kmer.max_read_len = max_read_len;
    cfg.kmer.merged_only = merged_only;
    cfg.device = 0;
    cfg.kernel = PSSBAM_KERNEL_AUTO;

    frontend_group_by_rg = by_group;
    frontend_n_length_edges = n_edges;
    memcpy(frontend_length_edges, edges, (size_t)n_edges * sizeof *edges);
    if (ctg_map) frontend_contig_sets = &sets;
    if (bed_fn) frontend_regions = &bed;
    frontend_warmup_start(&cfg, bam_fn, fasta_fn);
    Genome *genome = init_genome(fasta_fn);
    if (!genome) {
        fprintf(stderr, "Error: Unable to load genome from %s.\n", fasta_fn);
        exit(1);
    }
    fprintf(stderr, "Finished loading genome.\nCounting kmer contexts for: %s\n", bam_fn);

    run_result res;
    frontend_fast_exit = getenv("PSSBAM_CLEAN_EXIT") == NULL;
    if (run_tally(&cfg, genome, bam_fn, env_gpu_count(), &res)) exit(1);
    fragkon_write_table(stdout, fasta_fn, bam_fn, klen, res.k5, res.k3);
    fflush(stdout);
    if (by_group && res.n_planes == 0)
        fprintf(stderr, "Warning: -G: the header of %s has no @RG line; only the table of all reads was written.\n", bam_fn);
    for (int k = 0; k < res.n_planes; k++) {
        const size_t bins = (size_t)1 << (2 * klen);
        unsigned long lo = 0, hi = 0;
        if (len_edges) pss_length_bin_bounds(edges, n_edges, k, min_read_len, max_read_len, &lo, &hi);
        const char *id = by_group ? res.group_ids[k] : ctg_map ? sets.labels[k] : NULL;
        const size_t tag_len = id ? pss_rg_file_tag(id, NULL, 0) : pss_length_bin_tag(lo, hi, NULL, 0);
        char *tag = (char *)malloc(tag_len + 1);
        if (!tag) { fprintf(stderr, "Error: out of memory\n"); exit(1); }
        if (id) pss_rg_file_tag(id, tag, tag_len + 1);
        else pss_length_bin_tag(lo, hi, tag, tag_len + 1);
        if (fragkon_write_plane(fasta_fn, bam_fn, out_prefix, tag, klen, res.plane_k5 + k * bins, res.plane_k3 + k * bins)) exit(1);
        free(tag);
    }
    if (getenv("PSSBAM_STATS")) {
        fprintf(stderr, "[pssbam] records=%llu kmer_ok=%llu kmer_filtered=%llu kmer_fail=%llu gpus=%d\n",
                (unsigned long long)res.stats[PSSBAM_ST_RECORDS], (unsigned long long)res.stats[PSSBAM_ST_KMER_OK],
                (unsigned long long)res.stats[PSSBAM_ST_KMER_FILTERED], (unsigned long long)res.stats[PSSBAM_ST_KMER_FAIL],
                res.n_gpus);
    }
    if (frontend_fast_exit) {
        fprintf(stderr, "Done.\n");
        front_end_exit(0);
    }
    run_result_free(&res);
    destroy_genome(genome);
    if (ctg_map) pss_free_contig_sets(sets.names, sets.n_names, sets.set_of, sets.labels, sets.n_labels);
    free(fasta_fn);
    free(bam_fn);
    free(out_prefix);
    fprintf(stderr, "Done.\n");
    return 0;
}
```

pss-bam_amd/host/frontend.c:

```c
#include "frontend.h"
#include "read_groups.h"

#include <errno.h>
#include <fcntl.h>
#include <pthread.h>
#include <signal.h>
#include <stdint.h>
#include <stdio.h>
#include <stdlib.h>
#include <string.h>
#include <sys/stat.h>
#include <sys/types.h>
#include <sys/wait.h>
#include <time.h>
#include <unistd.h>

#include "bam_reader.h"
#include "device_feed.h"
#include "sam_reader.h"

int frontend_fast_exit = 0;
int frontend_group_by_rg = 0;
int frontend_n_length_edges = 0;
int frontend_min_base_quality = 0;
int frontend_length_hist = 0;
int frontend_site_context = PSSBAM_SITE_NONE;
int frontend_end_depth = 0, frontend_end_cell5 = 0, frontend_end_cell3 = 0;
const pss_regions *frontend_regions = NULL;
uint32_t frontend_length_edges[PSSBAM_MAX_LENGTH_BINS - 1];
const frontend_contig_map *frontend_contig_sets = NULL;

static int send_contig_sets(pssbam_engine *e, const frontend_contig_map *m)
{
    return m ? pssbam_engine_set_contig_sets(e, m->n_labels, m->n_names, (const char *const *)m->names, m->set_of) : 0;
}

static int send_regions(pssbam_engine *e, const pss_regions *r)
{
    return r ? pssbam_engine_set_regions(e, r->n_names, (const char *const *)r->names, r->n, r->name_of, r->starts, r->ends) : 0;
}

static bam_reader *early_rd = NULL;
static char early_path[4096];
static int early_registered = 0, early_light = 0;
static pthread_t warmup_thread;
static int warmup_running = 0;

static struct early_feed {
    int want;
    pssbam_config cfg;
    char *up, *down, *rg;
    uint64_t fasta_bytes;
    pssbam_engine *eng[64];
    char **rg_ids;
    int n_rg;
    int min_bq;
    int hist;
    int site;
    int end_depth, end_cell5, end_cell3;
    const pss_regions *regions;
    int n_edges;
    uint32_t edges[PSSBAM_MAX_LENGTH_BINS - 1];
    const frontend_contig_map *sets;
    int n_gpus, engines_ok, engines_done, fed, feed_rc, genome_set, failed;
    device_feed_stats dfs;
    char err[600];
    pthread_mutex_t mu;
    pthread_cond_t cv;
    int posted, abandon;
    double t0, t_hip, t_engines, t_posted, t_upload_dur, t_genome_set, t_genome_set_dur, t_feed_end;
} EF = {.mu = PTHREAD_MUTEX_INITIALIZER, .cv = PTHREAD_COND_INITIALIZER};

static int early_gate(void *ctx, int block)
{
    (void)ctx;
    pthread_mutex_lock(&EF.mu);
    while (!EF.posted && !EF.abandon && block) pthread_cond_wait(&EF.cv, &EF.mu);
    const int abandon = EF.abandon, posted = EF.posted;
    pthread_mutex_unlock(&EF.mu);
    if (abandon) return -1;
    if (!posted) return 0;
    if (!EF.genome_set) {
        const double t = frontend_now_s();
        const bam_header *h = bam_reader_header(early_rd);
        for (int g = 0; g < EF.n_gpus; g++)
            if (pssbam_engine_set_references(EF.eng[g], h->n_ref, (const char *const *)h->ref_name)) {
                snprintf(EF.err, sizeof EF.err, "GPU engine: %s", pssbam_last_error());
                EF.failed = 1;
                return -1;
            }
        EF.genome_set = 1;
        EF.t_genome_set = frontend_now_s() - EF.t0;
        EF.t_genome_set_dur = frontend_now_s() - t;
    }
    return 1;
}

static void early_engines_done(void)
{
    pthread_mutex_lock(&EF.mu);
    EF.engines_done = 1;
    pthread_cond_broadcast(&EF.cv);
    pthread_mutex_unlock(&EF.mu);
}

static int feed_run(int n_gpus);

static void *pin_main(void *arg)
{
    (void)arg;
    device_feed_prefetch_pin();
    return NULL;
}

static void *reserve_main(void *arg)
{
    (void)pssbam_feed_reserve((int)(intptr_t)arg);
    return NULL;
}

typedef struct {
    pssbam_config cfg;
    int32_t n_ref;
    pssbam_engine **out;
    int rc, started;
    char err[400];
} engine_make_job;

static void *engine_make_main(void *arg)
{
    engine_make_job *j = (engine_make_job *)arg;
    if (pssbam_engine_create(&j->cfg, j->out) || pssbam_engine_feed_open(*j->out, j->n_ref, EF.fasta_bytes) ||
        (EF.min_bq > 0 && pssbam_engine_set_min_base_quality(*j->out, EF.min_bq)) ||
        (EF.hist > 0 && pssbam_engine_set_length_histogram(*j->out, EF.hist)) ||
        (EF.site != PSSBAM_SITE_NONE && pssbam_engine_set_site_context(*j->out, EF.site)) ||
        (EF.end_depth > 0 && pssbam_engine_set_end_condition(*j->out, EF.end_depth, EF.end_cell5, EF.end_cell3)) || send_regions(*j->out, EF.regions) ||
        (EF.n_rg > 0 && pssbam_engine_set_read_groups(*j->out, EF.n_rg, (const char *const *)EF.rg_ids)) ||
        (EF.n_edges > 0 && pssbam_engine_set_length_bins(*j->out, EF.n_edges, EF.edges)) || send_contig_sets(*j->out, EF.sets)) {
        j->rc = 1;
        snprintf(j->err, sizeof j->err, "%s", pssbam_last_error());
    }
    return NULL;
}

static void early_feed_main(void)
{
    const int n = env_gpu_count();
    EF.t_hip = frontend_now_s() - EF.t0;
    const int have = pssbam_device_count();
    if (!getenv("PSSBAM_OVERSUBSCRIBE"))
        for (int g = 0; g < n && g < (have > 0 ? have : 1); g++) {
            pthread_t th;
            if (pthread_create(&th, NULL, reserve_main, (void *)(intptr_t)g) == 0) pthread_detach(th);
        }
    pthread_t pin_th;
    const int pin_started = pthread_create(&pin_th, NULL, pin_main, NULL) == 0;
    const bam_header *h = bam_reader_header(early_rd);
    if (frontend_group_by_rg && (EF.n_rg = pss_parse_read_groups(h->text, h->l_text, &EF.rg_ids)) < 0) EF.n_rg = 0;
    engine_make_job job[64];
    pthread_t th[64];
    for (int g = 0; g < n; g++) {
        job[g].cfg = EF.cfg;
        job[g].cfg.device = have > 0 ? g % have : g;
        job[g].n_ref = h->n_ref;
        job[g].out = &EF.eng[g];
        job[g].rc = 0;
        job[g].started = g > 0 && pthread_create(&th[g], NULL, engine_make_main, &job[g]) == 0;
    }
    for (int g = 0; g < n; g++)
        if (!job[g].started) (void)engine_make_main(&job[g]);
    for (int g = 0; g < n; g++)
        if (job[g].started) pthread_join(th[g], NULL);
    for (int g = 0; g < n; g++) {
        if (job[g].rc) {
            snprintf(EF.err, sizeof EF.err, "GPU engine %d: %s", g, job[g].err);
            EF.failed = 1;
            EF.n_gpus = n;
            early_engines_done();
            if (pin_started) pthread_join(pin_th, NULL);
            return;
        }
        EF.n_gpus = g + 1;
    }
    EF.engines_ok = 1;
    EF.t_engines = frontend_now_s() - EF.t0;
    early_engines_done();
    {
        const uint8_t *r0;
        const uint32_t *o0;
        size_t nb0;
        int slot0 = -1;
        if (bam_reader_next_hold(early_rd, &r0, &o0, &nb0, &slot0) > 0)
// ... 153 lines not shown
        close(2);
    }
    if (frontend_fast_exit) _exit(status);
    exit(status);
}

double frontend_process_age_s(void)
{
    FILE *f = fopen("/proc/self/stat", "r");
    if (!f) return -1.0;
    char buf[2048];
    const size_t n = fread(buf, 1, sizeof buf - 1, f);
    fclose(f);
    buf[n] = 0;
    const char *p = strrchr(buf, ')');
    if (!p) return -1.0;
    unsigned long long start = 0;
    int field = 2;
    for (p++; *p && field < 22; p++)
        if (*p == ' ') field++;
    if (field != 22 || sscanf(p, "%llu", &start) != 1) return -1.0;
    struct timespec ts;
    if (clock_gettime(CLOCK_BOOTTIME, &ts) != 0) return -1.0;
    return ts.tv_sec + ts.tv_nsec * 1e-9 - (double)start / (double)sysconf(_SC_CLK_TCK);
}

double frontend_now_s(void)
{
    struct timespec ts;
    clock_gettime(CLOCK_MONOTONIC, &ts);
    return ts.tv_sec + ts.tv_nsec * 1e-9;
}
#define now_s frontend_now_s

int env_gpu_count(void)
{
    const char *v = getenv("PSSBAM_NGPU");
    int want = v ? atoi(v) : 1, have = pssbam_device_count();
    if (want < 1) want = 1;
    if (have < 1) have = 1;
    if (getenv("PSSBAM_OVERSUBSCRIBE")) return want > 64 ? 64 : want;
    return want > have ? have : want;
}

void run_result_free(run_result *res)
{
    pss_free_read_groups(res->group_ids, res->group_ids ? res->n_planes : 0);
    free(res->plane_fwd);
    free(res->plane_rev);
    free(res->plane_k5);
    free(res->plane_k3);
    free(res->hist_fwd);
    free(res->hist_rev);
    free(res->site_fwd);
    free(res->site_rev);
    free(res->end_fwd);
    free(res->end_rev);
    free(res->fwd);
    free(res->rev);
    free(res->k5);
    free(res->k3);
    memset(res, 0, sizeof *res);
}

static int send_read_groups(pssbam_engine **eng, int n_gpus, const char *text, size_t len, run_result *res)
{
    if ((res->n_planes = pss_parse_read_groups(text, len, &res->group_ids)) < 0) {
        res->n_planes = 0;
        fprintf(stderr, "Error: out of memory\n");
        return -1;
    }
    for (int g = 0; g < n_gpus && res->n_planes > 0; g++)
        if (pssbam_engine_set_read_groups(eng[g], res->n_planes, (const char *const *)res->group_ids)) {
            fprintf(stderr, "Error: GPU engine %d: %s\n", g, pssbam_last_error());
            return -1;
        }
    return 0;
}

static int cmp_str_ptr(const void *a, const void *b) { return strcmp(*(const char *const *)a, *(const char *const *)b); }

static void warn_unreached_sets(const frontend_contig_map *m, const Genome *genome, int32_t n_ref, const char *const *ref_names,
                                const char *aln_path)
{
    const char **refs = (const char **)malloc(((size_t)n_ref + 1) * sizeof *refs);
    char *reached = (char *)calloc((size_t)m->n_labels, 1);
    if (!refs || !reached) {
        free(refs);
        free(reached);
        return;
    }
    for (int32_t i = 0; i < n_ref; i++) refs[i] = ref_names[i];
    qsort(refs, (size_t)n_ref, sizeof *refs, cmp_str_ptr);
    for (int k = 0; k < m->n_names; k++) {
        const char *nm = m->names[k];
        if (reached[m->set_of[k]]) continue;
        const int in_input = strcmp(nm, "*") == 0 || bsearch(&nm, refs, (size_t)n_ref, sizeof *refs, cmp_str_ptr) != NULL;
        size_t lo = 0, hi = genome ? genome->n_seqs : 0;
        int in_genome = 0;
        while (in_input && lo < hi && !in_genome) {
            const size_t mid = (lo + hi) / 2;
            const int c = strcmp(nm, genome->seqs[mid]->id);
            if (c == 0) in_genome = 1;
            else if (c < 0) hi = mid;
            else lo = mid + 1;
        }
        reached[m->set_of[k]] = (char)in_genome;
    }
    for (int s = 0; s < m->n_labels; s++)
        if (!reached[s])
            fprintf(stderr, "Warning: -C: no contig of label %s is both a reference of %s and in the FASTA; its tables are all zero.\n",
                    m->labels[s], aln_path);
    free(refs);
    free(reached);
}

int run_tally(const pssbam_config *cfg, Genome *genome, const char *aln_path, int n_gpus, run_result *res)
{
    pssbam_engine *eng[64] = {0};
    char err[512];
    int rc = -1, registered = 0;
    void *buf_base = NULL;
    size_t buf_bytes = 0;
    const double t0 = now_s();
    double t_mark = t0, t_open = 0, t_engine = 0, t_register = 0, t_read = 0, t_submit = 0, t_finish = 0;
    const int verbose = getenv("PSSBAM_STATS") != NULL;
    memset(res, 0, sizeof *res);
    if (n_gpus < 1) n_gpus = 1;
    if (n_gpus > 64) n_gpus = 64;

    const int is_bam = file_is_bam(aln_path);
    bam_reader *rd = NULL;
    sam_reader *sd = NULL;
    int32_t refs_sent = -1;
    if (is_bam < 0) {
        fprintf(stderr, "Error: Unable to open %s.\n", aln_path);
        return -1;
    }
    device_feed_stats dfs;
    memset(&dfs, 0, sizeof dfs);
    int fed_on_device = 0, adopted = 0, light = 0;
    int device_feed = is_bam && device_feed_enabled() && cfg->kernel != PSSBAM_KERNEL_SIMPLE;
    if (warmup_running) {
        const int mine = EF.want && is_bam && strcmp(early_path, aln_path) == 0 && same_config(cfg, &EF.cfg) && same_length_bins() && device_feed;
        if (EF.want) {
            int upload_ok = 0;
            if (mine) {
                pthread_mutex_lock(&EF.mu);
                while (!EF.engines_done) pthread_cond_wait(&EF.cv, &EF.mu);
                pthread_mutex_unlock(&EF.mu);
                upload_ok = EF.engines_ok;
                const double tu = now_s();
                for (int g = 0; g < EF.n_gpus && upload_ok; g++)
                    if (pssbam_engine_set_genome_async(EF.eng[g], genome)) {
                        snprintf(EF.err, sizeof EF.err, "GPU engine %d: %s", g, pssbam_last_error());
                        upload_ok = 0;
                    }
                EF.t_upload_dur = now_s() - tu;
            }
            pthread_mutex_lock(&EF.mu);
            if (mine && upload_ok) EF.posted = 1;
            else EF.abandon = 1;
            EF.t_posted = now_s() - EF.t0;
            pthread_cond_broadcast(&EF.cv);
            pthread_mutex_unlock(&EF.mu);
        }
        pthread_join(warmup_thread, NULL);
        warmup_running = 0;
        if (EF.want && mine && EF.engines_ok && !EF.failed && EF.posted) {
            adopted = 1;
            n_gpus = EF.n_gpus;
            for (int g = 0; g < n_gpus; g++) eng[g] = EF.eng[g];
        } else if (EF.want) {
            for (int g = 0; g < EF.n_gpus; g++)
                if (EF.eng[g]) pssbam_engine_destroy(EF.eng[g]);
            if (EF.failed && verbose) fprintf(stderr, "[pssbam] early feed not usable (%s): regular start\n", EF.err);
        }
        EF.want = 0;
    }
    if (is_bam && early_rd && strcmp(early_path, aln_path) == 0) {
        rd = early_rd;
        early_rd = NULL;
        light = early_light;
        if (early_registered) {
            bam_reader_buffer(rd, &buf_base, &buf_bytes);
            registered = 1;
        }
    } else if (is_bam && device_feed) {
        rd = bam_reader_open_slots(aln_path, 2, (size_t)8 << 20, 3, err, sizeof err);
        light = 1;
    } else if (is_bam) rd = bam_reader_open_slots(aln_path, 0, 0, feed_slots(n_gpus), err, sizeof err);
    else sd = sam_reader_open(aln_path, 0, err, sizeof err);
    if (is_bam && !rd && light) {
        light = 0;
        device_feed = 0;
        rd = bam_reader_open_slots(aln_path, 0, 0, feed_slots(n_gpus), err, sizeof err);
    }
    if (rd && light && !device_feed) {
        bam_reader_close(rd);
        light = 0;
        rd = bam_reader_open_slots(aln_path, 0, 0, feed_slots(n_gpus), err, sizeof err);
    }
    if (!rd && !sd) {
        fprintf(stderr, "Error: Unable to open %s: %s\n", aln_path, err);
        goto done;
    }
    t_open = now_s() - t_mark; t_mark = now_s();
    if (adopted) {
        if (EF.feed_rc || EF.failed) {
            if (EF.err[0]) fprintf(stderr, "Error: %s\n", EF.err);
            goto done;
        }
        if (!EF.genome_set) {
            const bam_header *h = bam_reader_header(rd);
            for (int g = 0; g < n_gpus; g++)
                if (pssbam_engine_set_references(eng[g], h->n_ref, (const char *const *)h->ref_name)) {
                    fprintf(stderr, "Error: GPU engine %d: %s\n", g, pssbam_last_error());
                    goto done;
                }
        }
        refs_sent = bam_reader_header(rd)->n_ref;
        dfs = EF.dfs;
        if (frontend_group_by_rg) {
            res->n_planes = EF.n_rg;
            res->group_ids = EF.rg_ids;
            EF.rg_ids = NULL;
            EF.n_rg = 0;
        }
        if (verbose)
            fprintf(stderr, "[pssbam] early feed (helper thread, seconds after start-up began): HIP runtime up %.3f, engines %.3f, genome upload "
                            "enqueued %.3f (took this thread %.3f), references set + put-off tallies launched %.3f (took %.3f), feed drained %.3f\n",
                    EF.t_hip, EF.t_engines, EF.t_posted, EF.t_upload_dur, EF.t_genome_set, EF.t_genome_set_dur, EF.t_feed_end);
    } else {
        for (int g = 0; g < n_gpus; g++) {
            pssbam_config c = *cfg;
            const int have = pssbam_device_count();
            c.device = have > 0 ? g % have : g;
            if (pssbam_engine_create(&c, &eng[g]) ||
                (frontend_min_base_quality > 0 && pssbam_engine_set_min_base_quality(eng[g], frontend_min_base_quality)) ||
                (frontend_length_hist > 0 && pssbam_engine_set_length_histogram(eng[g], frontend_length_hist)) ||
                (frontend_site_context != PSSBAM_SITE_NONE && pssbam_engine_set_site_context(eng[g], frontend_site_context)) ||
                (frontend_end_depth > 0 && pssbam_engine_set_end_condition(eng[g], frontend_end_depth, frontend_end_cell5, frontend_end_cell3)) ||
                send_regions(eng[g], frontend_regions) ||
                (frontend_n_length_edges > 0 && pssbam_engine_set_length_bins(eng[g], frontend_n_length_edges, frontend_length_edges)) ||
                send_contig_sets(eng[g], frontend_contig_sets)) {
                fprintf(stderr, "Error: GPU engine %d: %s\n", g, pssbam_last_error());
                goto done;
            }
        }
        for (int g = 0; g < n_gpus; g++)
            if (pssbam_engine_set_genome_async(eng[g], genome)) {
                fprintf(stderr, "Error: GPU engine %d: %s\n", g, pssbam_last_error());
                goto done;
            }
        if (frontend_group_by_rg && rd && send_read_groups(eng, n_gpus, bam_reader_header(rd)->text, bam_reader_header(rd)->l_text, res))
            goto done;
    }
    int groups_sent = !frontend_group_by_rg || rd != NULL;
    t_engine = now_s() - t_mark; t_mark = now_s();
    if (device_feed && rd && !adopted) {
        const bam_header *h = bam_reader_header(rd);
        for (int g = 0; g < n_gpus; g++)
            if (pssbam_engine_set_references(eng[g], h->n_ref, (const char *const *)h->ref_name)) {
                fprintf(stderr, "Error: GPU engine %d: %s\n", g, pssbam_last_error());
                goto done;
            }
        refs_sent = h->n_ref;
        {
            const uint8_t *r0;
            const uint32_t *o0;
            size_t nb0;
            int slot0 = -1;
            if (bam_reader_next_hold(rd, &r0, &o0, &nb0, &slot0) > 0)
                for (int g = 0; g < n_gpus; g++) (void)pssbam_engine_hint_records(eng[g], r0, nb0);
            if (slot0 >= 0) bam_reader_release(rd, slot0);
        }
        if (run_device_feed(eng, n_gpus, aln_path, bam_reader_header_bytes(rd), feed_run(n_gpus), verbose, &dfs, NULL)) goto done;
    }
    if (device_feed && rd) {
        if (dfs.fallback) {
            if (verbose) fprintf(stderr, "[pssbam] device feed not usable for this file: falling back to the host reader\n");
            for (int g = 0; g < n_gpus; g++)
                if (pssbam_engine_reset(eng[g])) { fprintf(stderr, "Error: GPU engine %d: %s\n", g, pssbam_last_error()); goto done; }
            bam_reader_close(rd);
            rd = bam_reader_open_slots(aln_path, 0, 0, feed_slots(n_gpus), err, sizeof err);
            light = 0;
            if (!rd) { fprintf(stderr, "Error: Unable to open %s: %s\n", aln_path, err); goto done; }
        } else fed_on_device = 1;
        t_submit = now_s() - t_mark; t_mark = now_s();
    }
    if (rd && !fed_on_device && !registered && !getenv("PSSBAM_NO_PIN")) {
        bam_reader_buffer(rd, &buf_base, &buf_bytes);
        registered = pssbam_host_register(buf_base, buf_bytes) == 0;
    }
    t_register = now_s() - t_mark;

    struct { int slot, g; uint64_t ticket; double t_issue, t_done; } fifo[64];
    int fifo_head = 0, fifo_len = 0;
    const int run = feed_run(n_gpus);
    const int max_inflight = rd ? (bam_reader_slots(rd) - 2 < 1 ? 1 : bam_reader_slots(rd) - 2 > 62 ? 62 : bam_reader_slots(rd) - 2) : 0;
    double overlap_s = 0.0, win_lo[64], win_hi[64];
    for (int g = 0; g < 64; g++) win_lo[g] = win_hi[g] = -1.0;
    uint64_t n_batches = 0;
#define RETIRE_OLDEST()                                                                                        \
    do {                                                                                                       \
        const int k = fifo_head;                                                                               \
        if (pssbam_engine_wait_copied(eng[fifo[k].g], fifo[k].ticket)) {                                       \
            fprintf(stderr, "Error: GPU engine: %s\n", pssbam_last_error());                                   \
            goto done;                                                                                         \
        }                                                                                                      \
        if (fifo[k].t_done < 0) fifo[k].t_done = now_s();                                                      \
        bam_reader_release(rd, fifo[k].slot);                                                                  \
        if (verbose && n_gpus > 1) {                                                                           \
                                \
            for (int o = 0; o < n_gpus; o++) {                                                                 \
                if (o == fifo[k].g || win_hi[o] < 0) continue;                                                 \
                const double lo = fifo[k].t_issue > win_lo[o] ? fifo[k].t_issue : win_lo[o];                   \
                const double hi = fifo[k].t_done < win_hi[o] ? fifo[k].t_done : win_hi[o];                     \
                if (hi > lo) overlap_s += hi - lo;                                                             \
            }                                                                                                  \
            if (n_batches <= 24)                                                                               \
                fprintf(stderr, "[pssbam] copy window: engine %d  %.4f .. %.4f s\n", fifo[k].g, fifo[k].t_issue - t0, \
                        fifo[k].t_done - t0);                                                                  \
            win_lo[fifo[k].g] = fifo[k].t_issue;                                                               \
            win_hi[fifo[k].g] = fifo[k].t_done;                                                                \
        }                                                                                                      \
        fifo_head = (fifo_head + 1) % 64;                                                                      \
        fifo_len--;                                                                                            \
    } while (0)

    for (int turn = 0; !fed_on_device; turn++) {
        const uint8_t *recs;
        const uint32_t *offs;
        size_t nbytes;
        int slot = -1;
        t_mark = now_s();
        int64_t n = rd ? bam_reader_next_hold(rd, &recs, &offs, &nbytes, &slot) : sam_reader_next(sd, &recs, &offs, &nbytes);
        t_read += now_s() - t_mark; t_mark = now_s();
        if (n < 0) {
            fprintf(stderr, "Error: %s: %s\n", aln_path, rd ? bam_reader_error(rd) : sam_reader_error(sd));
            goto done;
        }
        if (!groups_sent) {
            size_t hl = 0;
            const char *ht = sam_reader_header_text(sd, &hl);
            if (send_read_groups(eng, n_gpus, ht, hl, res)) goto done;
            groups_sent = 1;
        }
        if (n == 0) break;
        n_batches++;
        const int32_t n_ref = rd ? bam_reader_header(rd)->n_ref : sam_reader_n_ref(sd);
        if (n_ref != refs_sent) {
            const char *const *names = rd ? (const char *const *)bam_reader_header(rd)->ref_name : sam_reader_ref_names(sd);
            for (int g = 0; g < n_gpus; g++)
                if (pssbam_engine_set_references(eng[g], n_ref, names)) {
                    fprintf(stderr, "Error: GPU engine %d: %s\n", g, pssbam_last_error());
                    goto done;
                }
            refs_sent = n_ref;
        }
        const int g = (turn / run) % n_gpus;
        if (rd) {
            uint64_t ticket = 0;
            const double t_issue = now_s();
            if (pssbam_engine_submit_async(eng[g], recs, nbytes, offs, (uint32_t)n, &ticket)) {
                fprintf(stderr, "Error: GPU engine: %s\n", pssbam_last_error());
                goto done;
            }
            const int k = (fifo_head + fifo_len) % 64;
            fifo[k].slot = slot; fifo[k].g = g; fifo[k].ticket = ticket; fifo[k].t_issue = t_issue; fifo[k].t_done = -1.0;
            fifo_len++;
            if (verbose && n_gpus > 1)
                for (int i = 0; i < fifo_len; i++) {
                    const int q = (fifo_head + i) % 64;
                    if (fifo[q].t_done < 0 && pssbam_engine_copy_done(eng[fifo[q].g], fifo[q].ticket) == 1) fifo[q].t_done = now_s();
                }
            while (fifo_len > max_inflight) RETIRE_OLDEST();
        } else if (pssbam_engine_submit(eng[g], recs, nbytes, offs, (uint32_t)n)) {
            fprintf(stderr, "Error: GPU engine: %s\n", pssbam_last_error());
            goto done;
        }
        t_submit += now_s() - t_mark;
    }
    while (fifo_len > 0) RETIRE_OLDEST();
#undef RETIRE_OLDEST
    if (verbose && n_gpus > 1 && !fed_on_device)
        fprintf(stderr, "[pssbam] feed: %llu batches in runs of %d over %d engines, up to %d copies in flight; copy windows of "
                        "different engines overlapped for %.3f s\n", (unsigned long long)n_batches, run, n_gpus, max_inflight, overlap_s);
    t_mark = now_s();
    if (refs_sent < 0) {
        const int32_t n_ref = rd ? bam_reader_header(rd)->n_ref : sam_reader_n_ref(sd);
        const char *const *names = rd ? (const char *const *)bam_reader_header(rd)->ref_name : sam_reader_ref_names(sd);
        for (int g = 0; g < n_gpus; g++) (void)pssbam_engine_set_references(eng[g], n_ref, names);
    }
    if (pssbam_reduce_counters(eng, n_gpus, 0)) {
        fprintf(stderr, "Error: counter reduce: %s\n", pssbam_last_error());
        goto done;
    }
    if (cfg->tally_mask & PSSBAM_TALLY_PSS) {
        size_t cells = (size_t)(cfg->pss.region_len + 2) * 16;
        res->fwd = (unsigned long *)calloc(cells, sizeof(unsigned long));
        res->rev = (unsigned long *)calloc(cells, sizeof(unsigned long));
    }
    if (cfg->tally_mask & PSSBAM_TALLY_KMER) {
// ... 108 lines not shown
```

pss-bam_amd/host/frontend.h:

```cpp
#ifndef PSSBAM_FRONTEND_H
#define PSSBAM_FRONTEND_H

#include <stdint.h>

#include "fasta-genome-io.h"
#include "pssbam_hip.h"
#include "regions.h"

typedef struct run_result {
    unsigned long *fwd, *rev;
    uint64_t *k5, *k3;
    uint64_t stats[PSSBAM_ST_N];
    double inflate_s, total_s;
    int n_gpus;
    int n_planes;
    char **group_ids;
    unsigned long *plane_fwd, *plane_rev;
    uint64_t *plane_k5, *plane_k3;
    int hist_max;
    uint64_t *hist_fwd, *hist_rev;
    unsigned long *site_fwd, *site_rev;
    unsigned long *end_fwd, *end_rev;
    uint64_t end_reads[4];
} run_result;

extern int frontend_group_by_rg;

extern int frontend_min_base_quality;

extern int frontend_length_hist;

extern int frontend_site_context;

extern int frontend_end_depth, frontend_end_cell5, frontend_end_cell3;

extern const pss_regions *frontend_regions;

extern int frontend_n_length_edges;
extern uint32_t frontend_length_edges[PSSBAM_MAX_LENGTH_BINS - 1];

typedef struct frontend_contig_map {
    int n_names, n_labels;
    char **names, **labels;
    int32_t *set_of;
} frontend_contig_map;
extern const frontend_contig_map *frontend_contig_sets;

int run_tally(const pssbam_config *cfg, Genome *genome, const char *aln_path, int n_gpus, run_result *res);

void frontend_warmup_start(const pssbam_config *cfg, const char *aln_path, const char *fasta_path);

void frontend_detach_start(void);
int frontend_detached(void);

extern int frontend_fast_exit;
void front_end_exit(int status);
void run_result_free(run_result *res);
double frontend_now_s(void);
double frontend_process_age_s(void);
int env_gpu_count(void);
#endif
```

pss-bam_amd/host/genome_load.c:

```c
#include "fasta-genome-io.h"
#include "inflate_fast.h"

#include <errno.h>
#include <fcntl.h>
#include <pthread.h>
#include <stdatomic.h>
#include <sys/mman.h>
#include <sys/stat.h>
#include <unistd.h>

static char *contig_alloc(size_t bytes)
{
    const size_t huge = (size_t)2 << 20;
    if (bytes >= 4 * huge) {
        const size_t rounded = (bytes + huge - 1) & ~(huge - 1);
        void *p = NULL;
        if (posix_memalign(&p, huge, rounded) == 0) {
#ifdef MADV_HUGEPAGE
            (void)madvise(p, rounded, MADV_HUGEPAGE);
#endif
            return (char *)p;
        }
    }
    return (char *)malloc(bytes);
}

enum { C_BASE = 0, C_SPACE = 1, C_GT = 2 };
static unsigned char g_class[256];
static unsigned char g_upper[256];
static int g_tables_ready = 0;

static void init_tables(void)
{
    if (g_tables_ready) return;
    for (int c = 0; c < 256; c++) {
        g_class[c] = isspace(c) ? C_SPACE : (c == '>' ? C_GT : C_BASE);
        g_upper[c] = (unsigned char)toupper(c);
    }
    g_tables_ready = 1;
}

int is_gz(const char *fn)
{
    size_t n = strlen(fn);
    if (n < 3) return 0;
    return fn[n - 3] == '.' && fn[n - 2] == 'g' && fn[n - 1] == 'z';
}

FILE *fileOpen(const char *name, char access_mode[])
{
    FILE *f = fopen(name, access_mode);
    if (f == NULL) {
        fprintf(stderr, "%s\n", name);
        perror("Cannot open file");
    }
    return f;
}

int chr_cmp(const void *v1, const void *v2)
{
    const Seq *a = *(Seq *const *)v1, *b = *(Seq *const *)v2;
    return strcmp(a->id, b->id);
}

Seq *find_seq(Genome *genome, const char id[])
{
    Seq **hit;
    strncpy(genome->dummy->id, id, MAX_ID_LEN);
    genome->dummy->id[MAX_ID_LEN] = '\0';
    if (strlen(id) > MAX_ID_LEN) return NULL;
    hit = (Seq **)bsearch(&genome->dummy, genome->seqs, genome->n_seqs, sizeof(Seq *), chr_cmp);
    return hit ? *hit : NULL;
}


typedef struct {
    int gz;
    gzFile zf;
    int fd;
} blk_src;

static long blk_read(blk_src *s, unsigned char *buf, size_t cap)
{
    if (s->gz) return (long)gzread(s->zf, buf, (unsigned)cap);
    for (;;) {
        ssize_t n = read(s->fd, buf, cap);
        if (n < 0 && errno == EINTR) continue;
        return (long)n;
    }
}

typedef struct {
    Seq *cur;
    size_t cap;
    int state;
    size_t id_len;
    int bad;
} parse_state;

static void finish_contig(Genome *g, parse_state *ps)
{
    Seq *s = ps->cur;
    if (!s) return;
    s->seq[s->len] = '\0';
    if (ps->cap > s->len + 1) {
        char *shr = (char *)realloc(s->seq, s->len + 1);
        if (shr) s->seq = shr;
    }
    if (g->n_seqs < MAX_GENOME_SEQS) g->seqs[g->n_seqs++] = s;
    else destroy_seq(s);
    ps->cur = NULL;
}

static int begin_contig(parse_state *ps)
{
    Seq *s = (Seq *)malloc(sizeof(Seq));
    if (!s) return -1;
    ps->cap = 1 << 16;
    s->seq = (char *)malloc(ps->cap);
    if (!s->seq) { free(s); return -1; }
    s->len = 0;
    s->id[0] = '\0';
    ps->cur = s;
    ps->state = 1;
    ps->id_len = 0;
    return 0;
}

static int feed(Genome *g, parse_state *ps, const unsigned char *p, size_t n)
{
    size_t i = 0;
    while (i < n) {
        if (ps->state == 0) {
            Seq *s = ps->cur;
            if (!s) {
                if (p[i] != '>') { ps->bad = 1; return -1; }
                if (begin_contig(ps)) return -1;
                i++;
                continue;
            }
            while (i < n) {
                unsigned char c = p[i];
                unsigned char k = g_class[c];
                if (k == C_BASE) {
                    if (s->len + 2 > ps->cap) {
                        size_t want = ps->cap * 2;
                        char *nb;
                        if (want > (size_t)MAX_SEQ_LEN + 1) want = (size_t)MAX_SEQ_LEN + 1;
                        nb = (char *)realloc(s->seq, want);
                        if (!nb) return -1;
                        s->seq = nb;
                        ps->cap = want;
                    }
                    if (s->len == (size_t)MAX_SEQ_LEN) {
                        fprintf(stderr, "%s is truncated to %d\n", s->id, MAX_SEQ_LEN);
                        ps->state = 3;
                        break;
                    }
                    s->seq[s->len++] = (char)g_upper[c];
                    i++;
                } else if (k == C_SPACE) {
                    i++;
                } else {
                    break;
                }
            }
            if (i < n && ps->state == 0) {
                finish_contig(g, ps);
                if (begin_contig(ps)) return -1;
                i++;
            }
        } else if (ps->state == 1) {
            while (i < n && !g_class[p[i]]) {
                if (ps->id_len < MAX_ID_LEN) ps->cur->id[ps->id_len++] = (char)p[i];
                else ps->bad = 1;
                i++;
            }
            if (i < n) {
                if (p[i] == '>' ) {
                    if (ps->id_len < MAX_ID_LEN) ps->cur->id[ps->id_len++] = '>';
                    i++;
                    continue;
                }
                ps->cur->id[ps->id_len] = '\0';
                ps->state = 2;
            }
        } else if (ps->state == 2) {
            const unsigned char *nl = (const unsigned char *)memchr(p + i, '\n', n - i);
            if (!nl) { i = n; break; }
            i = (size_t)(nl - p) + 1;
            ps->state = 0;
        } else {
            const unsigned char *gt = (const unsigned char *)memchr(p + i, '>', n - i);
            if (!gt) { i = n; break; }
            i = (size_t)(gt - p);
            ps->state = 0;
        }
    }
    return 0;
}


typedef struct {
    size_t hdr;
    size_t body_a, body_b;
    size_t n_bases;
    char *dst;
    char id[MAX_ID_LEN + 1];
} fa_seg;

typedef struct {
    const unsigned char *data;
    size_t a, b;
    fa_seg *seg;
    size_t n_seg, cap_seg;
    int bad, open_header;
} fa_piece;

typedef struct {
    fa_piece *pc;
    size_t n_pc;
    size_t next;
    pthread_mutex_t mu;
    int pass;
} fa_job;

static fa_seg *piece_add_seg(fa_piece *pc)
{
    if (pc->n_seg == pc->cap_seg) {
        size_t cap = pc->cap_seg ? pc->cap_seg * 2 : 8;
        fa_seg *ns = (fa_seg *)realloc(pc->seg, cap * sizeof(fa_seg));
        if (!ns) return NULL;
        pc->seg = ns;
        pc->cap_seg = cap;
    }
    fa_seg *sg = &pc->seg[pc->n_seg++];
    memset(sg, 0, sizeof *sg);
    return sg;
}

static void piece_scan(fa_piece *pc)
{
    const unsigned char *p = pc->data;
    size_t i = pc->a;
    fa_seg *sg = piece_add_seg(pc);
    if (!sg) { pc->bad = 1; return; }
    sg->hdr = (size_t)-1;
    sg->body_a = i;
    while (i < pc->b) {
        size_t n = 0;
        while (i < pc->b) {
            const unsigned char k = g_class[p[i]];
            if (k == C_GT) break;
            n += k == C_BASE;
            i++;
        }
        sg->n_bases = n;
        sg->body_b = i;
        if (i == pc->b) break;
        sg = piece_add_seg(pc);
        if (!sg) { pc->bad = 1; return; }
        sg->hdr = i++;
        size_t id_len = 0;
        while (i < pc->b && !isspace(p[i])) {
            if (id_len < MAX_ID_LEN) sg->id[id_len++] = (char)p[i];
            else pc->bad = 1;
            i++;
        }
        sg->id[id_len] = '\0';
        const unsigned char *nl = i < pc->b ? (const unsigned char *)memchr(p + i, '\n', pc->b - i) : NULL;
        if (!nl) { pc->open_header = 1; sg->body_a = sg->body_b = pc->b; return; }
        i = (size_t)(nl - p) + 1;
        sg->body_a = sg->body_b = i;
    }
}

static void piece_copy(const fa_piece *pc)
{
    for (size_t k = 0; k < pc->n_seg; k++) {
        const fa_seg *sg = &pc->seg[k];
        char *d = sg->dst;
        if (!d) continue;
        for (size_t i = sg->body_a; i < sg->body_b; i++) {
            const unsigned char c = pc->data[i];
            if (g_class[c] == C_BASE) *d++ = (char)g_upper[c];
        }
    }
}

static void *fa_worker(void *arg)
{
    fa_job *job = (fa_job *)arg;
    for (;;) {
        pthread_mutex_lock(&job->mu);
        const size_t k = job->next++;
        pthread_mutex_unlock(&job->mu);
        if (k >= job->n_pc) break;
        if (job->pass == 0) piece_scan(&job->pc[k]);
        else piece_copy(&job->pc[k]);
    }
    return NULL;
}

static void fa_run(fa_job *job, int pass, int n_threads)
{
    pthread_t th[64];
    int started = 0;
    job->pass = pass;
    job->next = 0;
    for (int t = 0; t < n_threads - 1 && t < 64; t++)
        if (pthread_create(&th[started], NULL, fa_worker, job) == 0) started++;
    fa_worker(job);
    for (int t = 0; t < started; t++) pthread_join(th[t], NULL);
}

static int fasta_threads(void)
{
    int n_threads = 16;
    const char *ev = getenv("PSSBAM_FASTA_THREADS");
    long ncpu = sysconf(_SC_NPROCESSORS_ONLN);
    if (ev) n_threads = atoi(ev);
    if (ncpu > 0 && n_threads > ncpu) n_threads = (int)ncpu;
    return n_threads;
}

static int parse_parallel(const unsigned char *data, size_t size, const char fn[], int n_threads, Genome **out);

static int load_parallel(const char fn[], Genome **out)
{
    const int n_threads = fasta_threads();
    if (n_threads < 2) return 0;

    int fd = open(fn, O_RDONLY);
    struct stat st;
    if (fd < 0) return 0;
    if (fstat(fd, &st) != 0 || !S_ISREG(st.st_mode) || st.st_size < (off_t)(1 << 20)) { close(fd); return 0; }
    const size_t size = (size_t)st.st_size;
    const unsigned char *data = (const unsigned char *)mmap(NULL, size, PROT_READ, MAP_PRIVATE, fd, 0);
    close(fd);
    if (data == (const unsigned char *)MAP_FAILED) return 0;
    (void)madvise((void *)data, size, MADV_SEQUENTIAL);
    const int rc = parse_parallel(data, size, fn, n_threads, out);
    munmap((void *)data, size);
    return rc;
}

static int parse_parallel(const unsigned char *data, size_t size, const char fn[], int n_threads, Genome **out)
{
    int applicable = 1, bad = 0;
    Genome *genome = NULL;
    fa_job job;
    memset(&job, 0, sizeof job);
    pthread_mutex_init(&job.mu, NULL);
    size_t want = size / (4u * (size_t)n_threads);
    if (want > (8u << 20)) want = 8u << 20;
    if (want < (64u << 10)) want = 64u << 10;
    job.pc = (fa_piece *)calloc(size / want + 2, sizeof(fa_piece));
    if (!job.pc) { applicable = 0; goto out; }
    for (size_t a = 0; a < size;) {
        size_t b = a + want;
        if (b >= size) b = size;
        else {
            const unsigned char *nl = (const unsigned char *)memchr(data + b, '\n', size - b);
            b = nl ? (size_t)(nl - data) + 1 : size;
        }
        job.pc[job.n_pc].data = data;
        job.pc[job.n_pc].a = a;
        job.pc[job.n_pc].b = b;
        job.n_pc++;
        a = b;
    }
    if (data[0] != '>') bad = 1;
    if (!bad) fa_run(&job, 0, n_threads);

    genome = (Genome *)calloc(1, sizeof(Genome));
    if (!genome) { applicable = 0; goto out; }
    genome->seqs = (Seq **)malloc(sizeof(Seq *) * MAX_GENOME_SEQS);
    genome->dummy = (Seq *)calloc(1, sizeof(Seq));
    if (!genome->seqs || !genome->dummy) { applicable = 0; goto out; }
    genome->n_seqs = 0;
    for (int round = 0; round < 2 && !bad && applicable; round++) {
        Seq *cur = NULL;
        size_t idx = 0, fill = 0;
        for (size_t k = 0; k < job.n_pc && !bad; k++) {
            fa_piece *pc = &job.pc[k];
            if (round == 0 && (pc->bad || (pc->open_header))) { bad = 1; break; }
            for (size_t q = 0; q < pc->n_seg; q++) {
                fa_seg *sg = &pc->seg[q];
                if (sg->hdr != (size_t)-1) {
                    if (round == 0) {
                        if (genome->n_seqs >= MAX_GENOME_SEQS) { applicable = 0; break; }
                        cur = (Seq *)calloc(1, sizeof(Seq));
                        if (!cur) { applicable = 0; break; }
                        strcpy(cur->id, sg->id);
                        genome->seqs[genome->n_seqs++] = cur;
                    } else {
                        cur = genome->seqs[idx++];
                        fill = 0;
                    }
                }
                if (!cur) continue;
                if (round == 0) cur->len += sg->n_bases;
                else { sg->dst = cur->seq + fill; fill += sg->n_bases; }
            }
            if (!applicable) break;
        }
        if (round == 0 && !bad && applicable) {
            for (size_t c = 0; c < genome->n_seqs; c++) {
                Seq *sq = genome->seqs[c];
                if (sq->len > (size_t)MAX_SEQ_LEN) { applicable = 0; break; }
                sq->seq = contig_alloc(sq->len + 1);
                if (!sq->seq) { applicable = 0; break; }
                sq->seq[sq->len] = '\0';
            }
        }
    }
    if (!bad && applicable) fa_run(&job, 1, n_threads);

out:
    for (size_t k = 0; k < job.n_pc; k++) free(job.pc[k].seg);
    free(job.pc);
    pthread_mutex_destroy(&job.mu);
    if (!applicable) {
        if (genome) destroy_genome(genome);
        return 0;
    }
    if (bad) {
        fprintf(stderr, "%s: malformed FASTA (must start with '>', header lines end in newline, ids <= %d)\n",
                fn, MAX_ID_LEN);
        destroy_genome(genome);
        *out = NULL;
        return 1;
    }
    qsort(genome->seqs, genome->n_seqs, sizeof(Seq *), chr_cmp);
    *out = genome;
    return 1;
}

typedef struct { size_t in_off; uint32_t in_len, isize, crc; size_t out_off; } fa_bgzf_block;

typedef struct {
    const unsigned char *data;
    unsigned char *text;
    const fa_bgzf_block *blk;
    size_t n_blk, next;
    pthread_mutex_t mu;
    atomic_int bad;
} fa_bgzf_job;

static void *fa_bgzf_worker(void *arg)
{
    fa_bgzf_job *job = (fa_bgzf_job *)arg;
    pss_inflater *st = (pss_inflater *)malloc(sizeof *st);
    if (!st) { atomic_store(&job->bad, 1); return NULL; }
    for (;;) {
        pthread_mutex_lock(&job->mu);
        const size_t k0 = job->next;
        job->next += 64;
        pthread_mutex_unlock(&job->mu);
        if (k0 >= job->n_blk || atomic_load(&job->bad)) break;
        for (size_t k = k0; k < k0 + 64 && k < job->n_blk; k++) {
            const fa_bgzf_block *b = &job->blk[k];
            if (!b->isize) continue;
            if (pss_inflate_raw(st, job->data + b->in_off, b->in_len, job->text + b->out_off, b->isize) != 0 ||
                pss_crc32(0, job->text + b->out_off, b->isize) != b->crc) { atomic_store(&job->bad, 1); break; }
        }
    }
    free(st);
    return NULL;
}

static int load_bgzf_parallel(const char fn[], Genome **out)
{
    const int n_threads = fasta_threads();
    if (n_threads < 2) return 0;
    int fd = open(fn, O_RDONLY);
    struct stat sb;
    if (fd < 0) return 0;
    if (fstat(fd, &sb) != 0 || !S_ISREG(sb.st_mode) || sb.st_size < 28) { close(fd); return 0; }
    const size_t size = (size_t)sb.st_size;
    const unsigned char *data = (const unsigned char *)mmap(NULL, size, PROT_READ, MAP_PRIVATE, fd, 0);
    close(fd);
    if (data == (const unsigned char *)MAP_FAILED) return 0;
    int rc = 0;
    fa_bgzf_block *blk = NULL;
    size_t n_blk = 0, cap = 0, total = 0, o = 0;
    unsigned char *text = NULL;
    while (o < size) {
        if (size - o < 18 || data[o] != 0x1f || data[o + 1] != 0x8b || data[o + 2] != 8 || !(data[o + 3] & 4)) goto done;
        const size_t xlen = (size_t)data[o + 10] | ((size_t)data[o + 11] << 8);
        if (size - o < 12 + xlen + 8) goto done;
        size_t bsize = 0, x = o + 12;
        while (x + 4 <= o + 12 + xlen) {
            const size_t sl = (size_t)data[x + 2] | ((size_t)data[x + 3] << 8);
            if (data[x] == 'B' && data[x + 1] == 'C' && sl == 2 && x + 6 <= o + 12 + xlen) bsize = ((size_t)data[x + 4] | ((size_t)data[x + 5] << 8)) + 1;
            x += 4 + sl;
        }
        if (!bsize || bsize < 12 + xlen + 8 || bsize > size - o || (data[o + 3] & ~4)) goto done;
        if (n_blk == cap) {
            cap = cap ? cap * 2 : 4096;
            fa_bgzf_block *nb = (fa_bgzf_block *)realloc(blk, cap * sizeof *nb);
            if (!nb) goto done;
            blk = nb;
        }
        fa_bgzf_block *b = &blk[n_blk++];
        b->in_off = o + 12 + xlen;
        b->in_len = (uint32_t)(bsize - 12 - xlen - 8);
        memcpy(&b->crc, data + o + bsize - 8, 4);
        memcpy(&b->isize, data + o + bsize - 4, 4);
        if (b->isize > 65536u) goto done;
        b->out_off = total;
        total += b->isize;
        o += bsize;
    }
    if (total < ((size_t)1 << 20)) goto done;
    text = (unsigned char *)contig_alloc(total + 1);
    if (!text) goto done;
    {
        fa_bgzf_job job;
        memset(&job, 0, sizeof job);
        job.data = data;
        job.text = text;
        job.blk = blk;
        job.n_blk = n_blk;
        pthread_mutex_init(&job.mu, NULL);
        pthread_t th[64];
        int started = 0;
        for (int t = 0; t < n_threads - 1 && t < 64; t++)
            if (pthread_create(&th[started], NULL, fa_bgzf_worker, &job) == 0) started++;
        fa_bgzf_worker(&job);
        for (int t = 0; t < started; t++) pthread_join(th[t], NULL);
        pthread_mutex_destroy(&job.mu);
        if (atomic_load(&job.bad)) {
            fprintf(stderr, "%s: damaged BGZF block (inflate / CRC-32 check failed)\n", fn);
            *out = NULL;
            rc = 1;
            goto done;
        }
    }
    rc = parse_parallel(text, total, fn, n_threads, out);
done:
    free(text);
    free(blk);
    munmap((void *)data, size);
    return rc;
}

static int load_gzip_whole(const char fn[], Genome **out)
{
    const int n_threads = fasta_threads();
    if (n_threads < 2) return 0;
    struct stat sb;
    if (stat(fn, &sb) != 0 || !S_ISREG(sb.st_mode) || sb.st_size < 18) return 0;
    uint32_t isize = 0;
    {
        FILE *f = fopen(fn, "rb");
        if (!f) return 0;
        if (fseeko(f, -4, SEEK_END) != 0 || fread(&isize, 1, 4, f) != 4) isize = 0;
        fclose(f);
    }
    if (isize >= (1u << 20)) {
        int fd = open(fn, O_RDONLY);
        const size_t size = (size_t)sb.st_size;
        const unsigned char *data = fd >= 0 ? (const unsigned char *)mmap(NULL, size, PROT_READ, MAP_PRIVATE, fd, 0) : (const unsigned char *)MAP_FAILED;
        if (fd >= 0) close(fd);
        if (data != (const unsigned char *)MAP_FAILED) {
            size_t o = 10;
            int ok = size > 18 && data[0] == 0x1f && data[1] == 0x8b && data[2] == 8 && !(data[3] & 0xE0);
            const unsigned flg = ok ? data[3] : 0;
            if (ok && (flg & 4)) { ok = o + 2 <= size; if (ok) o += 2 + ((size_t)data[o] | ((size_t)data[o + 1] << 8)); }
            for (int fld = 0; ok && fld < 2; fld++)
                if (flg & (fld ? 16u : 8u)) {
                    while (o < size && data[o]) o++;
                    o++;
                }
            if (ok && (flg & 2)) o += 2;
            ok = ok && o + 8 < size;
            unsigned char *text = ok ? (unsigned char *)contig_alloc((size_t)isize + 1) : NULL;
            pss_inflater *st = text ? (pss_inflater *)malloc(sizeof *st) : NULL;
            int rc = 0, done = 0;
            if (st) {
                uint32_t crc;
                memcpy(&crc, data + size - 8, 4);
                if (pss_inflate_raw(st, data + o, size - 8 - o, text, isize) == 0 && pss_crc32(0, text, isize) == crc) {
                    rc = parse_parallel(text, isize, fn, n_threads, out);
                    done = 1;
                }
            }
            free(st);
            free(text);
            munmap((void *)data, size);
            if (done) return rc;
        }
    }
    gzFile zf = gzopen(fn, "rb");
    if (!zf) return 0;
    gzbuffer(zf, 1u << 20);
    size_t cap = (size_t)isize + 1, len = 0;
    if (cap < 5 * (size_t)sb.st_size) cap = 5 * (size_t)sb.st_size;
    if (cap < ((size_t)64 << 20)) cap = (size_t)64 << 20;
    unsigned char *text = (unsigned char *)contig_alloc(cap);
    int rc = 0, bad = 0;
    if (!text) { gzclose(zf); return 0; }
    for (;;) {
        if (len == cap) {
            const size_t ncap = cap + cap / 2;
            unsigned char *nt = (unsigned char *)contig_alloc(ncap);
            if (!nt) { bad = 1; break; }
            memcpy(nt, text, len);
            free(text);
            text = nt;
            cap = ncap;
        }
        const size_t want = cap - len < ((size_t)256 << 20) ? cap - len : ((size_t)256 << 20);
        const int got = gzread(zf, text + len, (unsigned)want);
        if (got < 0) { bad = 1; break; }
        if (got == 0) break;
        len += (size_t)got;
    }
    gzclose(zf);
    if (!bad && len >= ((size_t)1 << 20)) rc = parse_parallel(text, len, fn, n_threads, out);
    free(text);
    return rc;
}

Genome *init_genome(const char fn[])
{
    Genome *genome;
    blk_src src;
    parse_state ps;
    unsigned char *buf;
    const size_t BLK = 4u << 20;
    long got;

    init_tables();
    if (fn == NULL) return NULL;
    memset(&src, 0, sizeof src);
    src.gz = is_gz(fn);
    if (!src.gz && load_parallel(fn, &genome)) return genome;
    if (src.gz && load_bgzf_parallel(fn, &genome)) return genome;
    if (src.gz && load_gzip_whole(fn, &genome)) return genome;
    if (src.gz) {
        src.zf = gzopen(fn, "rb");
        if (!src.zf) {
            fprintf(stderr, "%s\n", fn);
            perror("Cannot open file");
            return NULL;
        }
        gzbuffer(src.zf, 1u << 20);
    } else {
        src.fd = open(fn, O_RDONLY);
        if (src.fd < 0) {
            fprintf(stderr, "%s\n", fn);
            perror("Cannot open file");
            return NULL;
        }
#ifdef POSIX_FADV_SEQUENTIAL
        (void)posix_fadvise(src.fd, 0, 0, POSIX_FADV_SEQUENTIAL);
#endif
    }
    genome = (Genome *)malloc(sizeof(Genome));
    genome->seqs = (Seq **)malloc(sizeof(Seq *) * MAX_GENOME_SEQS);
    genome->dummy = (Seq *)calloc(1, sizeof(Seq));
    genome->n_seqs = 0;
    buf = (unsigned char *)malloc(BLK);
    memset(&ps, 0, sizeof ps);
    while ((got = blk_read(&src, buf, BLK)) > 0) {
        if (feed(genome, &ps, buf, (size_t)got)) break;
    }
    if (ps.cur && (ps.state == 1 || ps.state == 2)) {
        ps.cur->id[ps.id_len < MAX_ID_LEN ? ps.id_len : MAX_ID_LEN] = '\0';
        ps.bad = 1;
    }
    finish_contig(genome, &ps);
    free(buf);
    if (src.gz) gzclose(src.zf); else close(src.fd);
    if (ps.bad) {
        fprintf(stderr, "%s: malformed FASTA (must start with '>', header lines end in newline, ids <= %d)\n",
                fn, MAX_ID_LEN);
        destroy_genome(genome);
        return NULL;
    }
    qsort(genome->seqs, genome->n_seqs, sizeof(Seq *), chr_cmp);
    return genome;
}


Fa_Src *init_fasta_src(const char fn[])
{
    Fa_Src *fs;
    if (fn == NULL) return NULL;
    if (strlen(fn) > MAX_FN_LEN) return NULL;
    fs = (Fa_Src *)calloc(1, sizeof(Fa_Src));
    if (!fs) return NULL;
    strcpy(fs->fn, fn);
    fs->seq_buffer = (char *)malloc((size_t)MAX_SEQ_LEN + 1);
    if (!fs->seq_buffer) { free(fs); return NULL; }
    fs->seq_buffer[0] = '\0';
    fs->is_gz = is_gz(fn);
    if (fs->is_gz) {
        fs->fagz = gzopen(fs->fn, "r");
        if (fs->fagz == NULL) { free(fs->seq_buffer); free(fs); return NULL; }
    } else {
        fs->fafp = fileOpen(fs->fn, "r");
        if (fs->fafp == NULL) { free(fs->seq_buffer); free(fs); return NULL; }
    }
    return fs;
}

int close_fasta_src(Fa_Src *fs)
{
    if (!fs) return 0;
    if (fs->is_gz) gzclose(fs->fagz); else fclose(fs->fafp);
    free(fs->seq_buffer);
    free(fs);
    return 0;
}

typedef int (*getc_fn)(void *h);
typedef void (*ungetc_fn)(int c, void *h);

static int read_record(getc_fn get, ungetc_fn unget, void *h, Seq *seq, char *seq_buffer)
{
    size_t i = 0;
    int c = get(h);
    init_tables();
    if (c == EOF) return -1;
    if (c != '>') return -2;
    c = get(h);
    while (c != EOF && !isspace(c)) {
        if (i < MAX_ID_LEN) seq->id[i++] = (char)c;
        c = get(h);
    }
    seq->id[i] = '\0';
    while (c != EOF && c != '\n') c = get(h);
    i = 0;
    if (c != EOF) c = get(h);
    while (c != '>' && c != EOF && i < (size_t)MAX_SEQ_LEN) {
        if (!g_class[c & 0xFF]) seq_buffer[i++] = (char)g_upper[c & 0xFF];
        c = get(h);
    }
    seq_buffer[i] = '\0';
    if (i == (size_t)MAX_SEQ_LEN) {
        fprintf(stderr, "%s is truncated to %d\n", seq->id, MAX_SEQ_LEN);
        while (c != '>' && c != EOF) c = get(h);
    }
    if (c != EOF) unget(c, h);
    seq->seq = (char *)malloc(i + 1);
    if (!seq->seq) return -3;
    memcpy(seq->seq, seq_buffer, i + 1);
    seq->len = i;
    return 0;
}

static int f_get(void *h) { return getc_unlocked((FILE *)h); }
static void f_unget(int c, void *h) { ungetc(c, (FILE *)h); }
static int z_get(void *h) { return gzgetc((gzFile)h); }
static void z_unget(int c, void *h) { gzungetc(c, (gzFile)h); }

int read_fasta(FILE *fafp, Seq *seq, char *seq_buffer)
{
    return read_record(f_get, f_unget, fafp, seq, seq_buffer);
}

int gzread_fasta(gzFile gzfp, Seq *seq, char *seq_buffer)
{
    return read_record(z_get, z_unget, gzfp, seq, seq_buffer);
}

Seq *get_next_fa(Fa_Src *fa_source, Genome *genome)
{
    Seq *seq;
    int status;
    if (!fa_source || !genome || genome->n_seqs >= MAX_GENOME_SEQS) return NULL;
    seq = (Seq *)malloc(sizeof(Seq));
    if (!seq) return NULL;
    status = fa_source->is_gz ? gzread_fasta(fa_source->fagz, seq, fa_source->seq_buffer)
                              : read_fasta(fa_source->fafp, seq, fa_source->seq_buffer);
    if (status) {
        free(seq);
        return NULL;
    }
    fa_source->n++;
    genome->seqs[genome->n_seqs++] = seq;
    return seq;
}

int destroy_seq(Seq *seq)
{
    if (!seq) return 0;
    free(seq->seq);
    free(seq);
    return 0;
}

int destroy_genome(Genome *genome)
{
    if (!genome) return 0;
    for (size_t i = 0; i < genome->n_seqs; i++) destroy_seq(genome->seqs[i]);
    free(genome->seqs);
    free(genome->dummy);
    free(genome);
    return 0;
}
```

pss-bam_amd/host/gkc_main.c:

```c
#include <stdio.h>
#include <stdlib.h>
#include <string.h>
#include <limits.h>
#include <unistd.h>

#include "fasta-genome-io.h"
#include "pssbam_hip.h"
#include "report.h"

#define K_DEF (4)

static void help(void)
{
    printf("genome-kmer-count -f <fasta genome file>\n");
    printf("                  -k <kmer size; default = %u>\n", K_DEF);
    printf("This program reports the number of observed number\n");
    printf("of all possible kmers of the given length in the\n");
    printf("input genome.\n");
    exit(0);
}

int main(int argc, char *argv[])
{
    int ich, k = K_DEF;
    char fa_in[MAX_FN_LEN + 1] = {'\0'};
    while ((ich = getopt(argc, argv, "f:k:")) != -1) {
        switch (ich) {
        case 'f': strncpy(fa_in, optarg, MAX_FN_LEN); break;
        case 'k': k = atoi(optarg); break;
        default: help();
        }
    }
    if (strlen(fa_in) == 0) help();
    if (k < 1 || k > PSSBAM_MAX_KLEN) {
        fprintf(stderr, "k-mer length %d is outside the range this build counts on the GPU (1..%d).\n", k, PSSBAM_MAX_KLEN);
        return 1;
    }
    Genome *genome = init_genome(fa_in);
    if (!genome) return 1;
    printf("Parsed input genome. Found %lu sequences.\n", genome->n_seqs);

    pssbam_config cfg;
    memset(&cfg, 0, sizeof cfg);
    cfg.abi_version = PSSBAM_ABI_VERSION;
    cfg.tally_mask = PSSBAM_TALLY_KMER;
    cfg.kmer.klen = k;
    cfg.kmer.max_read_len = 250000000;
    cfg.device = 0;
    pssbam_engine *eng = NULL;
    const size_t bins = (size_t)1 << (2 * k);
    uint64_t *counts = (uint64_t *)calloc(bins, sizeof(uint64_t));
    if (pssbam_engine_create(&cfg, &eng) || pssbam_engine_set_genome(eng, genome) ||
        pssbam_engine_genome_kmer_count(eng, k, counts)) {
        fprintf(stderr, "Error: GPU engine: %s\n", pssbam_last_error());
        return 1;
    }
    gkc_write_table(stdout, k, counts);
    pssbam_engine_destroy(eng);
    destroy_genome(genome);
    free(counts);
    return 0;
}
```

pss-bam_amd/host/pss_main.c:

```c
#include <ctype.h>
#include <stdio.h>
#include <stdlib.h>
#include <string.h>
#include <unistd.h>

#include "base_quality.h"
#include "contig_sets.h"
#include "fasta-genome-io.h"
#include "frontend.h"
#include "length_bins.h"
#include "length_hist.h"
#include "read_groups.h"
#include "regions.h"
#include "report.h"

int main(int argc, char *argv[])
{
    const double age_main = frontend_process_age_s();
    frontend_detach_start();
    const double t_main = frontend_now_s();
    int region_len = 15, min_mq = 0, merged_only = 0, by_group = 0, option;
    unsigned long min_read_len = 0, max_read_len = 250000000;
    const char *up_ctx = "ACGT", *down_ctx = "ACGT";
    char *fasta_fn = NULL, *bam_fn = NULL, *out_prefix = NULL, *read_group = NULL;
// ... 61 lines not shown
        exit(1);
    }
    uint32_t edges[PSSBAM_MAX_LENGTH_BINS - 1];
    int n_edges = 0;
    if (len_edges) {
        if (by_group) {
            fprintf(stderr, "-S (tables per length bin) and -G (tables per read group) exclude each other.\n");
            exit(1);
        }
        char err[200];
        if ((n_edges = pss_parse_length_edges(len_edges, min_read_len, max_read_len, edges, err, sizeof err)) < 0) {
            fprintf(stderr, "%s\n", err);
            exit(1);
        }
    }
    int min_bq = 0;
    if (min_bq_arg) {
        char err[200];
        if ((min_bq = pss_parse_min_base_quality(min_bq_arg, err, sizeof err)) < 0) {
            fprintf(stderr, "%s\n", err);
            exit(1);
        }
    }
    int hist_max = 0;
    if (hist_arg) {
        if (by_group || len_edges || ctg_map) {
            fprintf(stderr, "-H (fragment-length histogram) and %s exclude each other.\n",
                    by_group ? "-G (tables per read group)" : len_edges ? "-S (tables per length bin)" : "-C (tables per contig set)");
            exit(1);
        }
        char err[200];
        if ((hist_max = pss_parse_length_hist(hist_arg, err, sizeof err)) < 0) {
            fprintf(stderr, "%s\n", err);
            exit(1);
        }
    }
    if (site_arg) {
        if (strcmp(site_arg, "cpg") != 0) {
            fprintf(stderr, "-X (tables per site context): unknown context \"%s\"; the one context is cpg.\n", site_arg);
            exit(1);
        }
        if (by_group || len_edges || ctg_map || hist_arg) {
            fprintf(stderr, "-X (tables per site context) and %s exclude each other.\n",
                    by_group ? "-G (tables per read group)" : len_edges ? "-S (tables per length bin)"
                    : ctg_map ? "-C (tables per contig set)" : "-H (fragment-length histogram)");
            exit(1);
        }
    }
    int end_depth = 0, end_cell5 = 0, end_cell3 = 0;
    if (end_arg) {
        char err[200];
        if (pss_parse_end_condition(end_arg, &end_depth, &end_cell5, &end_cell3, err, sizeof err)) {
            fprintf(stderr, "%s\n", err);
            exit(1);
        }
        if (by_group || len_edges || ctg_map || hist_arg || site_arg) {
            fprintf(stderr, "-E (tables conditional on the other end) and %s exclude each other.\n",
                    by_group ? "-G (tables per read group)" : len_edges ? "-S (tables per length bin)"
                    : ctg_map ? "-C (tables per contig set)" : hist_arg ? "-H (fragment-length histogram)" : "-X (tables per site context)");
            exit(1);
        }
        if (region_len > 30 || end_depth > region_len) {
            fprintf(stderr, "-E (tables conditional on the other end) needs its depth <= -r <= 30 (both ends' marks are taken from the one pass "
                            "over 32 table rows), not -r %d with depth %d.\n", region_len, end_depth);
            exit(1);
        }
    }
    pss_regions bed;
    memset(&bed, 0, sizeof bed);
    if (bed_fn) {
        char err[300];
        if (pss_read_bed(bed_fn, &bed, err, sizeof err)) {
            fprintf(stderr, "%s (%s)\n", err, bed_fn);
            exit(1);
        }
    }
    frontend_contig_map sets;
    memset(&sets, 0, sizeof sets);
    if (ctg_map) {
        if (by_group || len_edges) {
            fprintf(stderr, "-C (tables per contig set) and %s exclude each other.\n",
                    by_group ? "-G (tables per read group)" : "-S (tables per length bin)");
            exit(1);
        }
        FILE *mf = fopen(ctg_map, "rb");
        char *text = NULL;
        size_t len = 0, cap = 0;
        int read_ok = mf != NULL;
        while (read_ok) {
            if (len == cap) {
                char *t = (char *)realloc(text, cap = cap ? 2 * cap : 65536);
                if (!t) { read_ok = 0; break; }
                text = t;
            }
            const size_t got = fread(text + len, 1, cap - len, mf);
            len += got;
            if (got == 0) { read_ok = !ferror(mf); break; }
        }
        if (mf) fclose(mf);
        if (!read_ok) {
            fprintf(stderr, "-C: unable to read the map file %s.\n", ctg_map);
            exit(1);
        }
        char err[600];
        sets.n_names = pss_parse_contig_sets(text, len, &sets.names, &sets.set_of, &sets.labels, &sets.n_labels, err, sizeof err);
        free(text);
        if (sets.n_names < 0) {
            fprintf(stderr, "%s (%s)\n", err, ctg_map);
            exit(1);
        }
    }

    fprintf(stderr, "Full command: %s -F %s -B %s -o %s -r %d -l %lu -L %lu -q %d", argv[0], fasta_fn, bam_fn,
            out_prefix, region_len, min_read_len, max_read_len, min_mq);
    if (read_group) fprintf(stderr, " -R %s", read_group);
    fprintf(stderr, " -U %s -D %s%s%s", up_ctx, down_ctx, merged_only ? " -m" : "", by_group ? " -G" : "");
    if (len_edges) fprintf(stderr, " -S %s", len_edges);
    if (ctg_map) fprintf(stderr, " -C %s", ctg_map);
    if (min_bq_arg) fprintf(stderr, " -Q %d", min_bq);
    if (hist_arg) fprintf(stderr, " -H %d", hist_max);
    if (site_arg) fprintf(stderr, " -X %s", site_arg);
    if (end_arg) fprintf(stderr, " -E %s", end_arg);
    fputc('\n', stderr);

    pssbam_config cfg;
    memset(&cfg, 0, sizeof cfg);
    cfg.abi_version = PSSBAM_ABI_VERSION;
    cfg.tally_mask = PSSBAM_TALLY_PSS;
    cfg.pss.region_len = region_len;
    cfg.pss.min_read_len = min_read_len;
    cfg.pss.max_read_len = max_read_len;
    cfg.pss.min_mq = min_mq;
    cfg.pss.up_ctx = up_ctx;
    cfg.pss.down_ctx = down_ctx;
    cfg.pss.merged_only = merged_only;
    cfg.read_group = read_group;
    cfg.device = 0;
    cfg.kernel = PSSBAM_KERNEL_AUTO;

    frontend_group_by_rg = by_group;
    frontend_n_length_edges = n_edges;
    memcpy(frontend_length_edges, edges, (size_t)n_edges * sizeof *edges);
    if (ctg_map) frontend_contig_sets = &sets;
    frontend_min_base_quality = min_bq;
    frontend_length_hist = hist_max;
    frontend_site_context = site_arg ? PSSBAM_SITE_CPG : PSSBAM_SITE_NONE;
    frontend_end_depth = end_depth;
    frontend_end_cell5 = end_cell5;
    frontend_end_cell3 = end_cell3;
    if (bed_fn) frontend_regions = &bed;
    fprintf(stderr, "Reading genome sequence from:\n%s\n", fasta_fn);
    frontend_warmup_start(&cfg, bam_fn, fasta_fn);
    const double t_fa = frontend_now_s();
    Genome *genome = init_genome(fasta_fn);
    if (getenv("PSSBAM_STATS")) fprintf(stderr, "[pssbam] genome: fasta load %.3f s\n", frontend_now_s() - t_fa);
    if (!genome) {
        fprintf(stderr, "Error: Unable to load genome from %s.\n", fasta_fn);
        exit(1);
    }
    fprintf(stderr, "Finished loading genome.\nCounting matches/mismatches from:\n%s\n", bam_fn);

    run_result res;
    frontend_fast_exit = getenv("PSSBAM_CLEAN_EXIT") == NULL;
    if (run_tally(&cfg, genome, bam_fn, env_gpu_count(), &res)) exit(1);

    double *fwd_rates = (double *)calloc((size_t)(region_len ? region_len : 1) * 12, sizeof(double));
    double *rev_rates = (double *)calloc((size_t)(region_len ? region_len : 1) * 12, sizeof(double));
    pss_sub_rates(region_len, res.fwd, fwd_rates);
    pss_sub_rates(region_len, res.rev, rev_rates);
    pss_write_counts(fasta_fn, bam_fn, out_prefix, region_len, res.fwd, res.rev);
    pss_write_rates(fasta_fn, bam_fn, out_prefix, region_len, fwd_rates, rev_rates);
    if (res.hist_fwd && pss_write_lengths(fasta_fn, bam_fn, out_prefix, res.hist_max, res.hist_fwd, res.hist_rev)) exit(1);
    if (res.site_fwd) {
        const size_t cells = (size_t)(region_len + 2) * 16;
        unsigned long *out_fwd = (unsigned long *)malloc(cells * sizeof *out_fwd), *out_rev = (unsigned long *)malloc(cells * sizeof *out_rev);
        if (!out_fwd || !out_rev) { fprintf(stderr, "Error: out of memory\n"); exit(1); }
        for (size_t i = 0; i < cells; i++) {
            out_fwd[i] = i < 32 ? res.fwd[i] : res.fwd[i] - res.site_fwd[i];
            out_rev[i] = i < 32 ? res.rev[i] : res.rev[i] - res.site_rev[i];
        }
        if (pss_write_labelled(fasta_fn, bam_fn, out_prefix, "cpg", region_len, res.site_fwd, res.site_rev) ||
            pss_write_labelled(fasta_fn, bam_fn, out_prefix, "noncpg", region_len, out_fwd, out_rev)) exit(1);
        free(out_fwd);
        free(out_rev);
    }
    if (res.end_fwd && (pss_write_labelled(fasta_fn, bam_fn, out_prefix, "cond", region_len, res.end_fwd, res.end_rev) ||
                        pss_write_end_reads(out_prefix, res.end_reads))) exit(1);
    if (by_group && res.n_planes == 0)
        fprintf(stderr, "Warning: -G: the header of %s has no @RG line; only the tables of all reads were written.\n", bam_fn);
    for (int k = 0; k < res.n_planes; k++) {
        const size_t cells = (size_t)(region_len + 2) * 16;
        unsigned long lo = 0, hi = 0;
        if (len_edges) pss_length_bin_bounds(edges, n_edges, k, min_read_len, max_read_len, &lo, &hi);
        const char *id = by_group ? res.group_ids[k] : ctg_map ? sets.labels[k] : NULL;
        const size_t tag_len = id ? pss_rg_file_tag(id, NULL, 0) : pss_length_bin_tag(lo, hi, NULL, 0);
        char *pprefix = (char *)malloc(strlen(out_prefix) + tag_len + 2);
        if (!pprefix) { fprintf(stderr, "Error: out of memory\n"); exit(1); }
        char *tag = pprefix + sprintf(pprefix, "%s.", out_prefix);
        if (id) pss_rg_file_tag(id, tag, tag_len + 1);
        else pss_length_bin_tag(lo, hi, tag, tag_len + 1);
        pss_sub_rates(region_len, res.plane_fwd + k * cells, fwd_rates);
        pss_sub_rates(region_len, res.plane_rev + k * cells, rev_rates);
        pss_write_counts(fasta_fn, bam_fn, pprefix, region_len, res.plane_fwd + k * cells, res.plane_rev + k * cells);
        pss_write_rates(fasta_fn, bam_fn, pprefix, region_len, fwd_rates, rev_rates);
        free(pprefix);
    }

    if (getenv("PSSBAM_STATS")) {
        static const char *nm[] = {"records", "rg_dropped", "parse_skip", "no_contig", "pss_ok", "pss_filtered"};
        for (int i = 0; i < 6; i++) fprintf(stderr, "[pssbam] %s=%llu\n", nm[i], (unsigned long long)res.stats[i]);
        fprintf(stderr, "[pssbam] slow_path=%llu%s\n", (unsigned long long)res.stats[PSSBAM_ST_SLOW_PATH],
                res.stats[PSSBAM_ST_SLOW_PATH] * 100 > res.stats[PSSBAM_ST_RECORDS]
                    ? "  (more than 1 % of the records were longer than the staged prefix and took the one-lane path: slower, same tables)" : "");
        fprintf(stderr, "[pssbam] gpus=%d inflate_s=%.3f total_s=%.3f\n", res.n_gpus, res.inflate_s, res.total_s);
        fprintf(stderr, "[pssbam] main() to reports written: %.3f s\n", frontend_now_s() - t_main);
        fprintf(stderr, "[pssbam] process creation to main(): %.2f s (exec + dynamic loading); main() to here %.3f s; exit: %s\n", age_main,
                frontend_now_s() - t_main, frontend_detached() ? "the caller is released now, this worker is torn down behind it" : "one process, teardown in the foreground");
    }
    if (frontend_fast_exit) {
        fprintf(stderr, "Done.\n");
        front_end_exit(0);
    }
    free(fwd_rates);
    free(rev_rates);
    run_result_free(&res);
    if (ctg_map) pss_free_contig_sets(sets.names, sets.n_names, sets.set_of, sets.labels, sets.n_labels);
    destroy_genome(genome);
    free(fasta_fn);
    free(bam_fn);
    free(out_prefix);
    free(read_group);
    fprintf(stderr, "Done.\n");
    return 0;
}
```

Before: 23.65 billion.

## Pack genome to 4 bits per base on host and expand on device

The host FASTA loader now produces a nibble-packed genome, using a per-engine nibble table that encodes ACGT and the context class. The engine uploads half as many bytes and rebuilds the byte genome on the device with a new expand kernel. This targets host-to-device transfer time of the reference during setup, at the cost of extra host packing work and more code paths. The packed path is the default unless PSSBAM_GENOME_BYTES is set.

```diff
diff --git a/include/pssbam_hip.h b/include/pssbam_hip.h
--- a/include/pssbam_hip.h
+++ b/include/pssbam_hip.h
@@ -97,6 +97,14 @@
 int pssbam_engine_set_genome_arrays(pssbam_engine *e, size_t n, const char *const *ids,
                                     const uint8_t *const *seqs, const uint64_t *lens,
                                     int seqs_on_device);
+
+int pssbam_genome_nibbles(const pssbam_config *cfg, uint8_t *nib);
+int pssbam_engine_genome_nibbles(pssbam_engine *e, uint8_t *nib);
+int pssbam_engine_set_genome_packed(pssbam_engine *e, size_t n, const char *const *ids, const uint8_t *const *packed,
+                                    const uint64_t *lens, const uint8_t *nib);
+int pssbam_engine_set_genome_packed_async(pssbam_engine *e, size_t n, const char *const *ids,
+                                          const uint8_t *const *packed, const uint64_t *lens, const uint8_t *nib);
+int pssbam_engine_genome_image(pssbam_engine *e, int which, void *dst, uint64_t cap, uint64_t *bytes);
 
 int pssbam_engine_set_references(pssbam_engine *e, int32_t n_ref, const char *const *names);
 
diff --git a/pss-bam_amd/__init__.py b/pss-bam_amd/__init__.py
--- a/pss-bam_amd/__init__.py
+++ b/pss-bam_amd/__init__.py
@@ -35,6 +35,8 @@
     "pssbam_engine_set_regions", "pssbam_engine_set_length_histogram", "pssbam_engine_finish_length_histogram",
     "pssbam_engine_set_site_context", "pssbam_engine_finish_site_context",
     "pssbam_engine_set_end_condition", "pssbam_engine_finish_end_condition",
+    "pssbam_genome_nibbles", "pssbam_engine_genome_nibbles", "pssbam_engine_set_genome_packed",
+    "pssbam_engine_set_genome_packed_async", "pssbam_engine_genome_image",
 ]
 MAX_READ_GROUPS = 4096
 MAX_LENGTH_BINS = 64
@@ -92,6 +94,11 @@
     L.pssbam_engine_set_genome.argtypes = [C.c_void_p, C.c_void_p]
     L.pssbam_engine_set_genome_arrays.argtypes = [C.c_void_p, C.c_size_t, C.POINTER(C.c_char_p),
                                                   C.POINTER(C.c_void_p), C.POINTER(C.c_uint64), C.c_int]
+    L.pssbam_genome_nibbles.argtypes = [C.POINTER(_Config), C.c_void_p]
+    L.pssbam_engine_genome_nibbles.argtypes = [C.c_void_p, C.c_void_p]
+    for fn in (L.pssbam_engine_set_genome_packed, L.pssbam_engine_set_genome_packed_async):
+        fn.argtypes = [C.c_void_p, C.c_size_t, C.POINTER(C.c_char_p), C.POINTER(C.c_void_p), C.POINTER(C.c_uint64), C.c_void_p]
+    L.pssbam_engine_genome_image.argtypes = [C.c_void_p, C.c_int, C.c_void_p, C.c_uint64, C.POINTER(C.c_uint64)]
     L.pssbam_engine_set_references.argtypes = [C.c_void_p, C.c_int32, C.POINTER(C.c_char_p)]
     L.pssbam_engine_submit.argtypes = [C.c_void_p, C.c_void_p, C.c_uint64, C.c_void_p, C.c_uint32]
     L.pssbam_engine_submit_async.argtypes = [C.c_void_p, C.c_void_p, C.c_uint64, C.c_void_p, C.c_uint32, C.POINTER(C.c_uint64)]
@@ -131,6 +138,18 @@
 def _chk(rc: int) -> None:
     if rc != 0:
         raise PssbamError(f"pssbam error {rc}: {hip_lib().pssbam_last_error().decode()}")
+
+
+def genome_nibbles(up_ctx: str | bytes | None = "ACGT", down_ctx: str | bytes | None = "ACGT") -> np.ndarray:
+    cfg = _Config()
+    cfg.abi_version = 1
+    cfg.tally_mask = TALLY_KMER if up_ctx is None else TALLY_PSS
+    if up_ctx is not None:
+        cfg.pss.up_ctx = up_ctx.encode() if isinstance(up_ctx, str) else bytes(up_ctx)
+        cfg.pss.down_ctx = down_ctx.encode() if isinstance(down_ctx, str) else bytes(down_ctx)
+    nib = np.zeros(256, dtype=np.uint8)
+    _chk(hip_lib().pssbam_genome_nibbles(C.byref(cfg), nib.ctypes.data))
+    return nib
 
 
 def bgzf_inflate(bgzf: np.ndarray, check_crc: bool = True, repeats: int = 1, want_output: bool = True) -> dict:
@@ -378,6 +397,28 @@
         lens = (C.c_uint64 * n)(*[c[2] for c in contigs])
         _chk(self._L.pssbam_engine_set_genome_arrays(self._h, n, ids, seqs, lens, 1))
 
+    def genome_nibbles(self) -> np.ndarray:
+        nib = np.zeros(256, dtype=np.uint8)
+        _chk(self._L.pssbam_engine_genome_nibbles(self._h, nib.ctypes.data))
+        return nib
+
+    def set_genome_packed(self, contigs: list[tuple[str, np.ndarray, int]], nib: np.ndarray):
+        n = len(contigs)
+        arrs = [np.ascontiguousarray(a, dtype=np.uint8) for _, a, _ in contigs]
+        nib = np.ascontiguousarray(nib, dtype=np.uint8)
+        assert nib.size == 256 and all(a.size >= (c[2] + 1) // 2 for a, c in zip(arrs, contigs))
+        ids = (C.c_char_p * n)(*[c[0].encode() for c in contigs])
+        seqs = (C.c_void_p * n)(*[a.ctypes.data for a in arrs])
+        lens = (C.c_uint64 * n)(*[c[2] for c in contigs])
+        _chk(self._L.pssbam_engine_set_genome_packed(self._h, n, ids, seqs, lens, nib.ctypes.data))
+
+    def genome_image(self, packed: bool) -> np.ndarray:
+        size = C.c_uint64()
+        _chk(self._L.pssbam_engine_genome_image(self._h, int(packed), None, 0, C.byref(size)))
+        out = np.zeros(size.value, dtype=np.uint8)
+        _chk(self._L.pssbam_engine_genome_image(self._h, int(packed), out.ctypes.data, out.size, C.byref(size)))
+        return out
+
     def set_genome_struct(self, genome_ptr: int):
         _chk(self._L.pssbam_engine_set_genome(self._h, C.c_void_p(genome_ptr)))
 
diff --git a/pss-bam_amd/csrc/engine.hip b/pss-bam_amd/csrc/engine.hip
--- a/pss-bam_amd/csrc/engine.hip
+++ b/pss-bam_amd/csrc/engine.hip
@@ -261,6 +261,18 @@
     }
 }
 
+static bool mask_has(const uint32_t (&m)[8], uint32_t b) { return (m[(b >> 5) & 7] >> (b & 31)) & 1u; }
+
+static void genome_nibbles(const char *up, const char *down, uint8_t nib[256]) {
+    uint32_t mu[8], md[8];
+    ctx_mask(up, mu);
+    ctx_mask(down, md);
+    for (uint32_t b = 0; b < 256; b++) {
+        const uint32_t c = enc_byte(b >= 'a' && b <= 'z' ? b - 32u : b);
+        nib[b] = (uint8_t)(c < 4u ? c : 4u + (mask_has(mu, c) ? 1u : 0u) + (mask_has(md, c) ? 2u : 0u));
+    }
+}
+
 static int env_int(const char *name) {
     const char *v = getenv(name);
     return v ? atoi(v) : 0;
@@ -482,8 +494,12 @@
 }
 
 static int genome_upload(pssbam_engine *e, size_t n, const char *const *ids, const uint8_t *const *seqs, const uint64_t *lens,
-                         int seqs_on_device) {
+                         int seqs_on_device, const uint8_t *nib = nullptr) {
     if (!e || (n && (!ids || !seqs || !lens))) return fail(PSSBAM_EINVAL, "null argument");
+    uint8_t own_nib[256];
+    genome_nibbles(e->up_ctx.c_str(), e->down_ctx.c_str(), own_nib);
+    if (nib && memcmp(nib, own_nib, sizeof own_nib))
+        return fail(PSSBAM_EINVAL, "the packed genome was made with a nibble table of other -U / -D sets than this engine's");
     HIP_TRY(hipSetDevice(e->device));
     int rc = genome_settle(e);
     if (rc) return rc;
@@ -518,30 +534,59 @@
         HIP_TRY(hipStreamWaitEvent(gs, ev, 0));
         e->event_pool.push_back(ev);
     }
-    HIP_TRY(hipMemsetAsync(e->d_genome, 0, total, gs));
+    CtxSets sets;
+    ctx_mask(e->up_ctx.c_str(), sets.up);
+    ctx_mask(e->down_ctx.c_str(), sets.down);
+    e->acgt_ctx = 0;
+    for (uint32_t v = 0; v < 4; v++)
+        e->acgt_ctx |= (((sets.up[0] >> v) & 1u) << (2 * v)) | (((sets.down[0] >> v) & 1u) << (2 * v + 1));
+    const uint64_t n_out = total / 8, slack = 16;
+    HIP_TRY(hipMalloc(&e->d_genome4, (n_out + slack) * sizeof(uint32_t)));
     const bool try_lock = !seqs_on_device && !getenv("PSSBAM_NO_PIN");
-    for (size_t k = 0; k < n; k++) {
-        if (!len[k]) continue;
-        const void *src = seqs[order[k]];
-        if (try_lock && len[k] >= (32u << 20) && pin_acquire(src, len[k])) e->genome_pins.push_back(src);
-        HIP_TRY(hipMemcpyAsync(e->d_genome + start[k], src, len[k],
-                               seqs_on_device ? hipMemcpyDeviceToDevice : hipMemcpyHostToDevice, gs));
-    }
-    hipLaunchKernelGGL(encode_genome_kernel, dim3(4096), dim3(256), 0, gs, e->d_genome, total / 16);
-    HIP_TRY(hipGetLastError());
-    {
-        CtxSets sets;
-        ctx_mask(e->up_ctx.c_str(), sets.up);
-        ctx_mask(e->down_ctx.c_str(), sets.down);
-        e->acgt_ctx = 0;
-        for (uint32_t v = 0; v < 4; v++)
-            e->acgt_ctx |= (((sets.up[0] >> v) & 1u) << (2 * v)) | (((sets.down[0] >> v) & 1u) << (2 * v + 1));
-        const uint64_t n_out = total / 8, slack = 16;
-        HIP_TRY(hipMalloc(&e->d_genome4, (n_out + slack) * sizeof(uint32_t)));
-        HIP_TRY(hipMemsetAsync(e->d_genome4 + n_out, 0x44, slack * sizeof(uint32_t), gs));
-        hipLaunchKernelGGL(pack_genome4_kernel, dim3(4096), dim3(256), 0, gs, e->d_genome, e->d_genome4, n_out, sets);
+    uint64_t sent = 0;
+    if (nib) {
+        const uint32_t nul = nib[0];
+        HIP_TRY(hipMemsetAsync(e->d_genome4, (int)(nul | (nul << 4)), (n_out + slack) * sizeof(uint32_t), gs));
+        for (size_t k = 0; k < n; k++) {
+            if (!len[k]) continue;
+            const void *src = seqs[order[k]];
+            const size_t bytes = ((size_t)len[k] + 1) / 2;
+            if (try_lock && bytes >= (16u << 20) && pin_acquire(src, bytes)) e->genome_pins.push_back(src);
+            HIP_TRY(hipMemcpyAsync((uint8_t *)e->d_genome4 + start[k] / 2, src, bytes, hipMemcpyHostToDevice, gs));
+            sent += bytes;
+        }
+        uint64_t rep = 0x03020100ull;
+        const uint32_t stored_nul = enc_byte(0u);
+        for (uint32_t cls = 4; cls < 8; cls++) {
+            uint32_t pick = 0;
+            for (uint32_t c = 4; c < 256 && !pick; c++)
+                if (4u + (mask_has(sets.up, c) ? 1u : 0u) + (mask_has(sets.down, c) ? 2u : 0u) == cls) pick = c;
+            if (cls == nul) pick = stored_nul;
+            rep |= (uint64_t)pick << (8 * cls);
+        }
+        hipLaunchKernelGGL(expand_genome4_kernel, dim3(4096), dim3(256), 0, gs, e->d_genome4, e->d_genome, total / 16, rep);
         HIP_TRY(hipGetLastError());
-    }
+    } else {
+        HIP_TRY(hipMemsetAsync(e->d_genome, 0, total, gs));
+        for (size_t k = 0; k < n; k++) {
+            if (!len[k]) continue;
+            const void *src = seqs[order[k]];
+            if (try_lock && len[k] >= (32u << 20) && pin_acquire(src, len[k])) e->genome_pins.push_back(src);
+            HIP_TRY(hipMemcpyAsync(e->d_genome + start[k], src, len[k],
+                                   seqs_on_device ? hipMemcpyDeviceToDevice : hipMemcpyHostToDevice, gs));
+            if (!seqs_on_device) sent += len[k];
+        }
+        hipLaunchKernelGGL(encode_genome_kernel, dim3(4096), dim3(256), 0, gs, e->d_genome, total / 16);
+        HIP_TRY(hipGetLastError());
+        {
+            HIP_TRY(hipMemsetAsync(e->d_genome4 + n_out, 0x44, slack * sizeof(uint32_t), gs));
+            hipLaunchKernelGGL(pack_genome4_kernel, dim3(4096), dim3(256), 0, gs, e->d_genome, e->d_genome4, n_out, sets);
+            HIP_TRY(hipGetLastError());
+        }
+    }
+    if (sent && getenv("PSSBAM_STATS"))
+        fprintf(stderr, "[pssbam] genome upload: %llu bytes over the link (%s), device %d\n", (unsigned long long)sent,
+                nib ? "4 bits per base" : "1 byte per base", e->device);
     HIP_TRY(hipEventRecord(e->genome_ready, gs));
     e->genome_wait_pending = true;
     e->contig_start.assign(start.begin(), start.begin() + n);
@@ -591,6 +636,45 @@
     HIP_TRY(hipSetDevice(e->device));
     if (e->genome_stream) HIP_TRY(hipStreamSynchronize(e->genome_stream));
     return genome_settle(e);
+}
+
+extern "C" int pssbam_engine_set_genome_packed_async(pssbam_engine *e, size_t n, const char *const *ids, const uint8_t *const *packed,
+                                                     const uint64_t *lens, const uint8_t *nib) {
+    if (!nib) return fail(PSSBAM_EINVAL, "null argument");
+    return genome_upload(e, n, ids, packed, lens, 0, nib);
+}
+
+extern "C" int pssbam_engine_set_genome_packed(pssbam_engine *e, size_t n, const char *const *ids, const uint8_t *const *packed,
+                                               const uint64_t *lens, const uint8_t *nib) {
+    int rc = pssbam_engine_set_genome_packed_async(e, n, ids, packed, lens, nib);
+    if (rc) return rc;
+    return pssbam_engine_genome_wait(e);
+}
+
+extern "C" int pssbam_genome_nibbles(const pssbam_config *cfg, uint8_t *nib) {
+    if (!cfg || !nib) return fail(PSSBAM_EINVAL, "null argument");
+    const bool pss = (cfg->tally_mask & PSSBAM_TALLY_PSS) != 0;
+    if (pss && (!cfg->pss.up_ctx || !cfg->pss.down_ctx)) return fail(PSSBAM_EINVAL, "up_ctx/down_ctx must be set");
+    genome_nibbles(pss ? cfg->pss.up_ctx : "", pss ? cfg->pss.down_ctx : "", nib);
+    return PSSBAM_OK;
+}
+
+extern "C" int pssbam_engine_genome_nibbles(pssbam_engine *e, uint8_t *nib) {
+    if (!e || !nib) return fail(PSSBAM_EINVAL, "null argument");
+    genome_nibbles(e->up_ctx.c_str(), e->down_ctx.c_str(), nib);
+    return PSSBAM_OK;
+}
+
+extern "C" int pssbam_engine_genome_image(pssbam_engine *e, int which, void *dst, uint64_t cap, uint64_t *bytes) {
+    if (!e || !bytes || (which != 0 && which != 1)) return fail(PSSBAM_EINVAL, "null or unknown argument");
+    if (!e->d_genome || !e->d_genome4) return fail(PSSBAM_ESTATE, "set_genome has not been called");
+    *bytes = which ? e->genome_bytes / 2 : e->genome_bytes;
+    if (!dst) return PSSBAM_OK;
+    if (cap < *bytes) return fail(PSSBAM_EINVAL, "the buffer holds %llu bytes, the image has %llu", (unsigned long long)cap, (unsigned long long)*bytes);
+    int rc = pssbam_engine_genome_wait(e);
+    if (rc) return rc;
+    HIP_TRY(hipMemcpy(dst, which ? (const void *)e->d_genome4 : (const void *)e->d_genome, *bytes, hipMemcpyDeviceToHost));
+    return PSSBAM_OK;
 }
 
 static int pack_regions(pssbam_engine *e, bool in_use) {
diff --git a/pss-bam_amd/csrc/tally_kernels.h b/pss-bam_amd/csrc/tally_kernels.h
--- a/pss-bam_amd/csrc/tally_kernels.h
+++ b/pss-bam_amd/csrc/tally_kernels.h
@@ -1589,4 +1589,23 @@
     }
 }
 
-}
+__global__ void expand_genome4_kernel(const uint32_t *g4, uint8_t *out, uint64_t n16, uint64_t rep) {
+    const uint64_t stride = (uint64_t)gridDim.x * blockDim.x;
+    const uint2 *src = (const uint2 *)g4;
+    uint4 *dst = (uint4 *)out;
+    for (uint64_t i = (uint64_t)blockIdx.x * blockDim.x + threadIdx.x; i < n16; i += stride) {
+        const uint2 v = src[i];
+        uint32_t w[4];
+#pragma unroll
+        for (int k = 0; k < 4; k++) {
+            const uint32_t half = ((k < 2 ? v.x : v.y) >> (16 * (k & 1))) & 0xFFFFu;
+            uint32_t o = 0u;
+#pragma unroll
+            for (int b = 0; b < 4; b++) o |= (uint32_t)((rep >> (8u * ((half >> (4 * b)) & 7u))) & 0xFFull) << (8 * b);
+            w[k] = o;
+        }
+        dst[i] = make_uint4(w[0], w[1], w[2], w[3]);
+    }
+}
+
+}
diff --git a/pss-bam_amd/host/fragkon_main.c b/pss-bam_amd/host/fragkon_main.c
--- a/pss-bam_amd/host/fragkon_main.c
+++ b/pss-bam_amd/host/fragkon_main.c
@@ -152,7 +152,7 @@
     if (ctg_map) frontend_contig_sets = &sets;
     if (bed_fn) frontend_regions = &bed;
     frontend_warmup_start(&cfg, bam_fn, fasta_fn);
-    Genome *genome = init_genome(fasta_fn);
+    Genome *genome = frontend_load_genome(&cfg, fasta_fn);
     if (!genome) {
         fprintf(stderr, "Error: Unable to load genome from %s.\n", fasta_fn);
         exit(1);
diff --git a/pss-bam_amd/host/frontend.c b/pss-bam_amd/host/frontend.c
--- a/pss-bam_amd/host/frontend.c
+++ b/pss-bam_amd/host/frontend.c
@@ -17,6 +17,7 @@
 
 #include "bam_reader.h"
 #include "device_feed.h"
+#include "genome_pack.h"
 #include "sam_reader.h"
 
 int frontend_fast_exit = 0;
@@ -38,6 +39,44 @@
 static int send_regions(pssbam_engine *e, const pss_regions *r)
 {
     return r ? pssbam_engine_set_regions(e, r->n_names, (const char *const *)r->names, r->n, r->name_of, r->starts, r->ends) : 0;
+}
+
+static struct {
+    const Genome *of;
+    GenomePacked *gp;
+    const char **ids;
+    uint64_t *lens;
+} packed_genome;
+
+Genome *frontend_load_genome(const pssbam_config *cfg, const char *fasta_fn)
+{
+    uint8_t nib[256];
+    const char *ev = getenv("PSSBAM_GENOME_BYTES");
+    if ((ev && atoi(ev)) || pssbam_genome_nibbles(cfg, nib)) return init_genome(fasta_fn);
+    GenomePacked *gp = NULL;
+    Genome *g = init_genome_packed(fasta_fn, nib, &gp);
+    if (!g) return NULL;
+    packed_genome.ids = (const char **)malloc((g->n_seqs ? g->n_seqs : 1) * sizeof(char *));
+    packed_genome.lens = (uint64_t *)malloc((g->n_seqs ? g->n_seqs : 1) * sizeof(uint64_t));
+    if (!packed_genome.ids || !packed_genome.lens) {
+        destroy_genome_packed(gp);
+        return g;
+    }
+    for (size_t i = 0; i < g->n_seqs; i++) {
+        packed_genome.ids[i] = g->seqs[i]->id;
+        packed_genome.lens[i] = g->seqs[i]->len;
+    }
+    packed_genome.of = g;
+    packed_genome.gp = gp;
+    return g;
+}
+
+static int send_genome(pssbam_engine *e, const Genome *genome)
+{
+    if (packed_genome.gp && packed_genome.of == genome)
+        return pssbam_engine_set_genome_packed_async(e, genome->n_seqs, packed_genome.ids, (const uint8_t *const *)packed_genome.gp->packed,
+                                                     packed_genome.lens, packed_genome.gp->nib);
+    return pssbam_engine_set_genome_async(e, genome);
 }
 
 static bam_reader *early_rd = NULL;
@@ -497,7 +536,7 @@
                 upload_ok = EF.engines_ok;
                 const double tu = now_s();
                 for (int g = 0; g < EF.n_gpus && upload_ok; g++)
-                    if (pssbam_engine_set_genome_async(EF.eng[g], genome)) {
+                    if (send_genome(EF.eng[g], genome)) {
                         snprintf(EF.err, sizeof EF.err, "GPU engine %d: %s", g, pssbam_last_error());
                         upload_ok = 0;
                     }
@@ -594,7 +633,7 @@
             }
         }
         for (int g = 0; g < n_gpus; g++)
-            if (pssbam_engine_set_genome_async(eng[g], genome)) {
+            if (send_genome(eng[g], genome)) {
                 fprintf(stderr, "Error: GPU engine %d: %s\n", g, pssbam_last_error());
                 goto done;
             }
diff --git a/pss-bam_amd/host/frontend.h b/pss-bam_amd/host/frontend.h
--- a/pss-bam_amd/host/frontend.h
+++ b/pss-bam_amd/host/frontend.h
@@ -46,6 +46,8 @@
 } frontend_contig_map;
 extern const frontend_contig_map *frontend_contig_sets;
 
+Genome *frontend_load_genome(const pssbam_config *cfg, const char *fasta_fn);
+
 int run_tally(const pssbam_config *cfg, Genome *genome, const char *aln_path, int n_gpus, run_result *res);
 
 void frontend_warmup_start(const pssbam_config *cfg, const char *aln_path, const char *fasta_path);
diff --git a/pss-bam_amd/host/genome4check_main.c b/pss-bam_amd/host/genome4check_main.c
--- /dev/null
+++ b/pss-bam_amd/host/genome4check_main.c
@@ -0,0 +1,43 @@
+#include <stdint.h>
+#include <stdio.h>
+#include <stdlib.h>
+#include <string.h>
+
+#include "fasta-genome-io.h"
+#include "genome_pack.h"
+
+int main(int argc, char **argv)
+{
+    const char *fa = NULL, *tab = NULL;
+    for (int i = 1; i < argc; i++) {
+        if (!strcmp(argv[i], "-f") && i + 1 < argc) fa = argv[++i];
+        else if (!strcmp(argv[i], "-t") && i + 1 < argc) tab = argv[++i];
+    }
+    if (!fa || !tab) {
+        fprintf(stderr, "usage: genome4check -f genome.fa[.gz] -t table.bin\n");
+        return 2;
+    }
+    uint8_t nib[256];
+    FILE *f = fopen(tab, "rb");
+    if (!f || fread(nib, 1, 256, f) != 256) { fprintf(stderr, "genome4check: %s does not hold 256 bytes\n", tab); return 1; }
+    fclose(f);
+    Genome *plain = init_genome(fa);
+    GenomePacked *gp = NULL;
+    Genome *g = init_genome_packed(fa, nib, &gp);
+    if (!plain || !g || !gp) { fprintf(stderr, "genome4check: cannot load %s\n", fa); return 1; }
+    if (plain->n_seqs != g->n_seqs || gp->n_seqs != g->n_seqs) { fprintf(stderr, "genome4check: contig counts differ\n"); return 1; }
+    for (size_t i = 0; i < g->n_seqs; i++) {
+        const Seq *a = plain->seqs[i], *b = g->seqs[i];
+        if (strcmp(a->id, b->id) || a->len != b->len || memcmp(a->seq, b->seq, a->len + 1)) {
+            fprintf(stderr, "genome4check: contig %zu differs between the two loads\n", i);
+            return 1;
+        }
+        printf("%s %zu ", b->id, b->len);
+        for (size_t k = 0; k < (b->len + 1) / 2; k++) printf("%02x", gp->packed[i][k]);
+        printf("\n");
+    }
+    destroy_genome(plain);
+    destroy_genome(g);
+    destroy_genome_packed(gp);
+    return 0;
+}
diff --git a/pss-bam_amd/host/genome_load.c b/pss-bam_amd/host/genome_load.c
--- a/pss-bam_amd/host/genome_load.c
+++ b/pss-bam_amd/host/genome_load.c
@@ -1,4 +1,5 @@
 #include "fasta-genome-io.h"
+#include "genome_pack.h"
 #include "inflate_fast.h"
 
 #include <errno.h>
@@ -8,6 +9,9 @@
 #include <sys/mman.h>
 #include <sys/stat.h>
 #include <unistd.h>
+#ifdef __SSE2__
+#include <emmintrin.h>
+#endif
 
 static char *contig_alloc(size_t bytes)
 {
@@ -38,6 +42,50 @@
         g_upper[c] = (unsigned char)toupper(c);
     }
     g_tables_ready = 1;
+}
+
+typedef struct {
+    const uint8_t *nib;
+    uint8_t **packed;
+    size_t n;
+} pack_ctx;
+
+static size_t packed_bytes(size_t len) { return len ? (len + 1) / 2 : 1; }
+
+static void pack_ctx_drop(pack_ctx *pk)
+{
+    if (!pk) return;
+    for (size_t i = 0; i < pk->n; i++) free(pk->packed[i]);
+    free(pk->packed);
+    pk->packed = NULL;
+    pk->n = 0;
+}
+
+static uint8_t *pack_contig(const Seq *s, const uint8_t *nib)
+{
+    uint8_t *out = (uint8_t *)malloc(packed_bytes(s->len));
+    const unsigned char *q = (const unsigned char *)s->seq;
+    if (!out) return NULL;
+    out[0] = (uint8_t)(nib[0] | (nib[0] << 4));
+    for (size_t p = 0; p < s->len; p += 2)
+        out[p >> 1] = (uint8_t)(nib[q[p]] | (nib[q[p + 1]] << 4));
+    return out;
+}
+
+static int sort_genome(Genome *g, pack_ctx *pk)
+{
+    typedef struct { Seq *s; uint8_t *p; } pair;
+    if (!pk) {
+        qsort(g->seqs, g->n_seqs, sizeof(Seq *), chr_cmp);
+        return 0;
+    }
+    pair *v = (pair *)malloc((g->n_seqs ? g->n_seqs : 1) * sizeof(pair));
+    if (!v) return -1;
+    for (size_t i = 0; i < g->n_seqs; i++) { v[i].s = g->seqs[i]; v[i].p = pk->packed[i]; }
+    qsort(v, g->n_seqs, sizeof(pair), chr_cmp);
+    for (size_t i = 0; i < g->n_seqs; i++) { g->seqs[i] = v[i].s; pk->packed[i] = v[i].p; }
+    free(v);
+    return 0;
 }
 
 int is_gz(const char *fn)
@@ -206,6 +254,8 @@
     size_t body_a, body_b;
     size_t n_bases;
     char *dst;
+    uint8_t *pk;
+    size_t pos;
     char id[MAX_ID_LEN + 1];
 } fa_seg;
 
@@ -223,6 +273,8 @@
     size_t next;
     pthread_mutex_t mu;
     int pass;
+    const uint8_t *nib;
+    const uint8_t *pair;
 } fa_job;
 
 static fa_seg *piece_add_seg(fa_piece *pc)
@@ -275,17 +327,97 @@
     }
 }
 
-static void piece_copy(const fa_piece *pc)
+typedef struct { uint8_t *pk; size_t pos; unsigned lo; int have_lo; } pack_cursor;
+
+static inline void pack_one(pack_cursor *pc, const uint8_t *nib, unsigned char c)
+{
+    if (pc->pos & 1) {
+        if (pc->have_lo) pc->pk[pc->pos >> 1] = (uint8_t)(pc->lo | ((unsigned)nib[c] << 4));
+        pc->have_lo = 0;
+    } else {
+        pc->lo = nib[c];
+        pc->have_lo = 1;
+    }
+    pc->pos++;
+}
+
+static inline void pack_run(pack_cursor *pc, const uint8_t *nib, const uint8_t *pair, const unsigned char *q, size_t n)
+{
+    size_t t = 0;
+    if (!n) return;
+    if (pc->pos & 1) pack_one(pc, nib, q[t++]);
+    uint8_t *out = pc->pk + (pc->pos >> 1);
+    const size_t pairs = (n - t) / 2;
+    for (size_t j = 0; j < pairs; j++) {
+        uint16_t w;
+        memcpy(&w, q + t + 2 * j, 2);
+        out[j] = pair[w];
+    }
+    t += 2 * pairs;
+    pc->pos += 2 * pairs;
+    if (t < n) pack_one(pc, nib, q[t]);
+}
+
+static void piece_copy(const fa_piece *pc, const uint8_t *nib, const uint8_t *pair)
 {
     for (size_t k = 0; k < pc->n_seg; k++) {
         const fa_seg *sg = &pc->seg[k];
         char *d = sg->dst;
         if (!d) continue;
-        for (size_t i = sg->body_a; i < sg->body_b; i++) {
-            const unsigned char c = pc->data[i];
-            if (g_class[c] == C_BASE) *d++ = (char)g_upper[c];
-        }
-    }
+        const int packing = nib && sg->pk;
+        const int acgt_is_0123 = packing && nib['A'] == 0 && nib['C'] == 1 && nib['G'] == 2 && nib['T'] == 3 &&
+                                 nib['a'] == 0 && nib['c'] == 1 && nib['g'] == 2 && nib['t'] == 3;
+        (void)acgt_is_0123;
+        pack_cursor cur = {sg->pk, sg->pos, 0, 0};
+        const unsigned char *p = pc->data;
+        size_t i = sg->body_a;
+        const size_t end = sg->body_b;
+        while (i < end) {
+            size_t stop = end;
+#ifdef __SSE2__
+            if (end - i >= 16) {
+                const __m128i v = _mm_loadu_si128((const __m128i *)(p + i));
+                const __m128i ws = _mm_sub_epi8(v, _mm_set1_epi8(9));
+                const __m128i other = _mm_or_si128(_mm_or_si128(_mm_cmpeq_epi8(v, _mm_set1_epi8(' ')), _mm_cmpeq_epi8(v, _mm_set1_epi8('>'))),
+                                                   _mm_cmpeq_epi8(_mm_min_epu8(ws, _mm_set1_epi8(4)), ws));
+                if (!_mm_movemask_epi8(other)) {
+                    const __m128i lc = _mm_sub_epi8(v, _mm_set1_epi8('a'));
+                    const __m128i is_lc = _mm_cmpeq_epi8(_mm_min_epu8(lc, _mm_set1_epi8(25)), lc);
+                    const __m128i up = _mm_sub_epi8(v, _mm_and_si128(is_lc, _mm_set1_epi8(32)));
+                    const __m128i acgt = _mm_or_si128(_mm_or_si128(_mm_cmpeq_epi8(up, _mm_set1_epi8('A')), _mm_cmpeq_epi8(up, _mm_set1_epi8('C'))),
+                                                      _mm_or_si128(_mm_cmpeq_epi8(up, _mm_set1_epi8('G')), _mm_cmpeq_epi8(up, _mm_set1_epi8('T'))));
+                    if (packing && acgt_is_0123 && !(cur.pos & 1) && _mm_movemask_epi8(acgt) == 0xFFFF) {
+                        const __m128i x = _mm_and_si128(_mm_srli_epi16(up, 1), _mm_set1_epi8(3));
+                        const __m128i code = _mm_xor_si128(x, _mm_and_si128(_mm_srli_epi16(x, 1), _mm_set1_epi8(1)));
+                        const __m128i two = _mm_or_si128(_mm_and_si128(code, _mm_set1_epi16(0x00FF)), _mm_slli_epi16(_mm_srli_epi16(code, 8), 4));
+                        _mm_storel_epi64((__m128i *)(cur.pk + (cur.pos >> 1)), _mm_packus_epi16(two, two));
+                        cur.pos += 16;
+                    } else if (packing) pack_run(&cur, nib, pair, p + i, 16);
+                    _mm_storeu_si128((__m128i *)d, up);
+                    d += 16;
+                    i += 16;
+                    continue;
+                }
+                stop = i + 16;
+            }
+#endif
+            for (; i < stop; i++) {
+                const unsigned char c = p[i];
+                if (g_class[c] != C_BASE) continue;
+                *d++ = (char)g_upper[c];
+                if (packing) pack_one(&cur, nib, c);
+            }
+        }
+    }
+}
+
+static void seg_fix_edges(const fa_seg *sg, const uint8_t *nib)
+{
+    if (!sg->pk || !sg->dst || !sg->n_bases) return;
+    const unsigned char *seq = (const unsigned char *)sg->dst - sg->pos;
+    const size_t s = sg->pos, t = s + sg->n_bases;
+    if (s & 1) sg->pk[s >> 1] = (uint8_t)(nib[seq[s - 1]] | (nib[seq[s]] << 4));
+    if (t & 1) sg->pk[t >> 1] = (uint8_t)(nib[seq[t - 1]] | (nib[seq[t]] << 4));
 }
 
 static void *fa_worker(void *arg)
@@ -297,7 +429,7 @@
         pthread_mutex_unlock(&job->mu);
         if (k >= job->n_pc) break;
         if (job->pass == 0) piece_scan(&job->pc[k]);
-        else piece_copy(&job->pc[k]);
+        else piece_copy(&job->pc[k], job->nib, job->pair);
     }
     return NULL;
 }
@@ -324,9 +456,9 @@
     return n_threads;
 }
 
-static int parse_parallel(const unsigned char *data, size_t size, const char fn[], int n_threads, Genome **out);
-
-static int load_parallel(const char fn[], Genome **out)
+static int parse_parallel(const unsigned char *data, size_t size, const char fn[], int n_threads, Genome **out, pack_ctx *pk);
+
+static int load_parallel(const char fn[], Genome **out, pack_ctx *pk)
 {
     const int n_threads = fasta_threads();
     if (n_threads < 2) return 0;
@@ -340,12 +472,12 @@
     close(fd);
     if (data == (const unsigned char *)MAP_FAILED) return 0;
     (void)madvise((void *)data, size, MADV_SEQUENTIAL);
-    const int rc = parse_parallel(data, size, fn, n_threads, out);
+    const int rc = parse_parallel(data, size, fn, n_threads, out, pk);
     munmap((void *)data, size);
     return rc;
 }
 
-static int parse_parallel(const unsigned char *data, size_t size, const char fn[], int n_threads, Genome **out)
+static int parse_parallel(const unsigned char *data, size_t size, const char fn[], int n_threads, Genome **out, pack_ctx *pk)
 {
     int applicable = 1, bad = 0;
     Genome *genome = NULL;
@@ -401,7 +533,12 @@
                 }
                 if (!cur) continue;
                 if (round == 0) cur->len += sg->n_bases;
-                else { sg->dst = cur->seq + fill; fill += sg->n_bases; }
+                else {
+                    sg->dst = cur->seq + fill;
+                    sg->pk = pk ? pk->packed[idx - 1] : NULL;
+                    sg->pos = fill;
+                    fill += sg->n_bases;
+                }
             }
             if (!applicable) break;
         }
@@ -413,9 +550,31 @@
                 if (!sq->seq) { applicable = 0; break; }
                 sq->seq[sq->len] = '\0';
             }
-        }
-    }
-    if (!bad && applicable) fa_run(&job, 1, n_threads);
+            if (pk && applicable) {
+                pk->packed = (uint8_t **)calloc(genome->n_seqs ? genome->n_seqs : 1, sizeof(uint8_t *));
+                if (!pk->packed) applicable = 0;
+                for (size_t c = 0; c < genome->n_seqs && applicable; c++) {
+                    pk->packed[c] = (uint8_t *)contig_alloc(packed_bytes(genome->seqs[c]->len));
+                    if (!pk->packed[c]) { applicable = 0; break; }
+                    pk->n = c + 1;
+                    if (!genome->seqs[c]->len) pk->packed[c][0] = (uint8_t)(pk->nib[0] | (pk->nib[0] << 4));
+                }
+            }
+        }
+    }
+    if (!bad && applicable) {
+        uint8_t *pair = pk ? (uint8_t *)malloc(65536) : NULL;
+        for (unsigned w = 0; pair && w < 65536; w++) pair[w] = (uint8_t)(pk->nib[w & 255] | (pk->nib[w >> 8] << 4));
+        job.nib = pair ? pk->nib : NULL;
+        job.pair = pair;
+        if (pk && !pair) applicable = 0;
+        else fa_run(&job, 1, n_threads);
+        free(pair);
+        if (pk && applicable)
+            for (size_t k = 0; k < job.n_pc; k++)
+                for (size_t q = 0; q < job.pc[k].n_seg; q++) seg_fix_edges(&job.pc[k].seg[q], pk->nib);
+        if (sort_genome(genome, pk)) applicable = 0;
+    }
 
 out:
     for (size_t k = 0; k < job.n_pc; k++) free(job.pc[k].seg);
@@ -423,16 +582,17 @@
     pthread_mutex_destroy(&job.mu);
     if (!applicable) {
         if (genome) destroy_genome(genome);
+        pack_ctx_drop(pk);
         return 0;
     }
     if (bad) {
         fprintf(stderr, "%s: malformed FASTA (must start with '>', header lines end in newline, ids <= %d)\n",
                 fn, MAX_ID_LEN);
         destroy_genome(genome);
+        pack_ctx_drop(pk);
         *out = NULL;
         return 1;
     }
-    qsort(genome->seqs, genome->n_seqs, sizeof(Seq *), chr_cmp);
     *out = genome;
     return 1;
 }
@@ -470,7 +630,7 @@
     return NULL;
 }
 
-static int load_bgzf_parallel(const char fn[], Genome **out)
+static int load_bgzf_parallel(const char fn[], Genome **out, pack_ctx *pk)
 {
     const int n_threads = fasta_threads();
     if (n_threads < 2) return 0;
@@ -538,7 +698,7 @@
             goto done;
         }
     }
-    rc = parse_parallel(text, total, fn, n_threads, out);
+    rc = parse_parallel(text, total, fn, n_threads, out, pk);
 done:
     free(text);
     free(blk);
@@ -546,7 +706,7 @@
     return rc;
 }
 
-static int load_gzip_whole(const char fn[], Genome **out)
+static int load_gzip_whole(const char fn[], Genome **out, pack_ctx *pk)
 {
     const int n_threads = fasta_threads();
     if (n_threads < 2) return 0;
@@ -583,7 +743,7 @@
                 uint32_t crc;
                 memcpy(&crc, data + size - 8, 4);
                 if (pss_inflate_raw(st, data + o, size - 8 - o, text, isize) == 0 && pss_crc32(0, text, isize) == crc) {
-                    rc = parse_parallel(text, isize, fn, n_threads, out);
+                    rc = parse_parallel(text, isize, fn, n_threads, out, pk);
                     done = 1;
                 }
             }
@@ -619,12 +779,12 @@
         len += (size_t)got;
     }
     gzclose(zf);
-    if (!bad && len >= ((size_t)1 << 20)) rc = parse_parallel(text, len, fn, n_threads, out);
+    if (!bad && len >= ((size_t)1 << 20)) rc = parse_parallel(text, len, fn, n_threads, out, pk);
     free(text);
     return rc;
 }
 
-Genome *init_genome(const char fn[])
+static Genome *load_genome(const char fn[], pack_ctx *pk)
 {
     Genome *genome;
     blk_src src;
@@ -637,9 +797,9 @@
     if (fn == NULL) return NULL;
     memset(&src, 0, sizeof src);
     src.gz = is_gz(fn);
-    if (!src.gz && load_parallel(fn, &genome)) return genome;
-    if (src.gz && load_bgzf_parallel(fn, &genome)) return genome;
-    if (src.gz && load_gzip_whole(fn, &genome)) return genome;
+    if (!src.gz && load_parallel(fn, &genome, pk)) return genome;
+    if (src.gz && load_bgzf_parallel(fn, &genome, pk)) return genome;
+    if (src.gz && load_gzip_whole(fn, &genome, pk)) return genome;
     if (src.gz) {
         src.zf = gzopen(fn, "rb");
         if (!src.zf) {
@@ -681,8 +841,55 @@
         destroy_genome(genome);
         return NULL;
     }
-    qsort(genome->seqs, genome->n_seqs, sizeof(Seq *), chr_cmp);
+    if (pk) {
+        pk->packed = (uint8_t **)calloc(genome->n_seqs ? genome->n_seqs : 1, sizeof(uint8_t *));
+        for (size_t i = 0; pk->packed && i < genome->n_seqs; i++) {
+            pk->packed[i] = pack_contig(genome->seqs[i], pk->nib);
+            if (!pk->packed[i]) break;
+            pk->n = i + 1;
+        }
+        if (!pk->packed || pk->n != genome->n_seqs || sort_genome(genome, pk)) {
+            pack_ctx_drop(pk);
+            destroy_genome(genome);
+            return NULL;
+        }
+        return genome;
+    }
+    sort_genome(genome, NULL);
     return genome;
+}
+
+Genome *init_genome(const char fn[]) { return load_genome(fn, NULL); }
+
+Genome *init_genome_packed(const char fn[], const uint8_t nib[256], GenomePacked **out)
+{
+    pack_ctx pk;
+    if (!out) return NULL;
+    *out = NULL;
+    if (!nib) return NULL;
+    GenomePacked *gp = (GenomePacked *)calloc(1, sizeof *gp);
+    if (!gp) return NULL;
+    memcpy(gp->nib, nib, 256);
+    memset(&pk, 0, sizeof pk);
+    pk.nib = gp->nib;
+    Genome *genome = load_genome(fn, &pk);
+    if (!genome) {
+        pack_ctx_drop(&pk);
+        free(gp);
+        return NULL;
+    }
+    gp->n_seqs = genome->n_seqs;
+    gp->packed = pk.packed;
+    *out = gp;
+    return genome;
+}
+
+void destroy_genome_packed(GenomePacked *gp)
+{
+    if (!gp) return;
+    for (size_t i = 0; i < gp->n_seqs; i++) free(gp->packed[i]);
+    free(gp->packed);
+    free(gp);
 }
 
 
diff --git a/pss-bam_amd/host/genome_pack.h b/pss-bam_amd/host/genome_pack.h
--- /dev/null
+++ b/pss-bam_amd/host/genome_pack.h
@@ -0,0 +1,25 @@
+#ifndef PSSBAM_GENOME_PACK_H
+#define PSSBAM_GENOME_PACK_H
+
+#include <stddef.h>
+#include <stdint.h>
+
+#include "fasta-genome-io.h"
+
+#ifdef __cplusplus
+extern "C" {
+#endif
+
+typedef struct genome_packed {
+    size_t n_seqs;
+    uint8_t **packed;
+    uint8_t nib[256];
+} GenomePacked;
+
+Genome *init_genome_packed(const char fn[], const uint8_t nib[256], GenomePacked **out);
+void destroy_genome_packed(GenomePacked *gp);
+
+#ifdef __cplusplus
+}
+#endif
+#endif
diff --git a/pss-bam_amd/host/gkc_main.c b/pss-bam_amd/host/gkc_main.c
--- a/pss-bam_amd/host/gkc_main.c
+++ b/pss-bam_amd/host/gkc_main.c
@@ -5,6 +5,7 @@
 #include <unistd.h>
 
 #include "fasta-genome-io.h"
+#include "genome_pack.h"
 #include "pssbam_hip.h"
 #include "report.h"
 
@@ -36,10 +37,6 @@
         fprintf(stderr, "k-mer length %d is outside the range this build counts on the GPU (1..%d).\n", k, PSSBAM_MAX_KLEN);
         return 1;
     }
-    Genome *genome = init_genome(fa_in);
-    if (!genome) return 1;
-    printf("Parsed input genome. Found %lu sequences.\n", genome->n_seqs);
-
     pssbam_config cfg;
     memset(&cfg, 0, sizeof cfg);
     cfg.abi_version = PSSBAM_ABI_VERSION;
@@ -47,10 +44,24 @@
     cfg.kmer.klen = k;
     cfg.kmer.max_read_len = 250000000;
     cfg.device = 0;
+    uint8_t nib[256];
+    GenomePacked *gp = NULL;
+    Genome *genome = pssbam_genome_nibbles(&cfg, nib) ? NULL : init_genome_packed(fa_in, nib, &gp);
+    if (!genome) return 1;
+    printf("Parsed input genome. Found %lu sequences.\n", genome->n_seqs);
+
     pssbam_engine *eng = NULL;
     const size_t bins = (size_t)1 << (2 * k);
     uint64_t *counts = (uint64_t *)calloc(bins, sizeof(uint64_t));
-    if (pssbam_engine_create(&cfg, &eng) || pssbam_engine_set_genome(eng, genome) ||
+    const char **ids = (const char **)malloc((genome->n_seqs ? genome->n_seqs : 1) * sizeof(char *));
+    uint64_t *lens = (uint64_t *)malloc((genome->n_seqs ? genome->n_seqs : 1) * sizeof(uint64_t));
+    if (!counts || !ids || !lens) return 1;
+    for (size_t i = 0; i < genome->n_seqs; i++) {
+        ids[i] = genome->seqs[i]->id;
+        lens[i] = genome->seqs[i]->len;
+    }
+    if (pssbam_engine_create(&cfg, &eng) ||
+        pssbam_engine_set_genome_packed(eng, genome->n_seqs, ids, (const uint8_t *const *)gp->packed, lens, gp->nib) ||
         pssbam_engine_genome_kmer_count(eng, k, counts)) {
         fprintf(stderr, "Error: GPU engine: %s\n", pssbam_last_error());
         return 1;
@@ -58,6 +69,9 @@
     gkc_write_table(stdout, k, counts);
     pssbam_engine_destroy(eng);
     destroy_genome(genome);
+    destroy_genome_packed(gp);
+    free(ids);
+    free(lens);
     free(counts);
     return 0;
 }
diff --git a/pss-bam_amd/host/pss_main.c b/pss-bam_amd/host/pss_main.c
--- a/pss-bam_amd/host/pss_main.c
+++ b/pss-bam_amd/host/pss_main.c
@@ -237,7 +237,7 @@
     fprintf(stderr, "Reading genome sequence from:\n%s\n", fasta_fn);
     frontend_warmup_start(&cfg, bam_fn, fasta_fn);
     const double t_fa = frontend_now_s();
-    Genome *genome = init_genome(fasta_fn);
+    Genome *genome = frontend_load_genome(&cfg, fasta_fn);
     if (getenv("PSSBAM_STATS")) fprintf(stderr, "[pssbam] genome: fasta load %.3f s\n", frontend_now_s() - t_fa);
     if (!genome) {
         fprintf(stderr, "Error: Unable to load genome from %s.\n", fasta_fn);
```

After: 23.65 billion, median of 3. Within noise of the previous version (+0.0%).
